# bjack205/rsLQR

Hardware: AMD Instinct MI355X
Metric: LQR solves/sec (nx=12,nu=4,N=256,batch=1024 per GPU) (higher is better)
Workload: dtype f64; 1 GPU; nx=12 nu=4 N=256 batch=1024 per GPU, fp64, factor+solve per step; parallelism=batch-sharded x1, no data-path collective, ranks_seen=1, flags=0, schedule=reduced-fused2

## Files before the change

### include/ndlqr_hip.h

```cpp
#ifndef NDLQR_HIP_H_
#define NDLQR_HIP_H_

#include <stddef.h>
#include <stdint.h>

#ifdef __cplusplus
extern "C" {
#endif

typedef struct NdlqrHipCtx NdlqrHipCtx;

int ndlqr_hip_device_count(void);
const char* ndlqr_hip_last_error(void);

NdlqrHipCtx* ndlqr_hip_create(int nstates, int ninputs, int nhorizon, int batch, int device);
#define NDLQR_CREATE_NO_PAD 1u
NdlqrHipCtx* ndlqr_hip_create_ex(int nstates, int ninputs, int nhorizon, int batch, int device, unsigned create_flags);
void ndlqr_hip_destroy(NdlqrHipCtx* ctx);
int ndlqr_hip_set_flags(NdlqrHipCtx* ctx, unsigned flags);
unsigned ndlqr_hip_get_flags(const NdlqrHipCtx* ctx);
int ndlqr_hip_set_stream(NdlqrHipCtx* ctx, void* hip_stream);
void* ndlqr_hip_get_stream(NdlqrHipCtx* ctx);

int ndlqr_hip_upload_inputs(NdlqrHipCtx* ctx, int p0, int count, const double* AB,
                            const double* QR, const double* rhs);
int ndlqr_hip_pack_flat_device(NdlqrHipCtx* ctx, const double* A, const double* B, const double* Q,
                               const double* R, const double* q, const double* r, const double* d,
                               const double* x0);
int ndlqr_hip_init_dense(NdlqrHipCtx* ctx, const double* A, const double* B, const double* Q, const double* H,
                         const double* R, const double* q, const double* r, const double* d, const double* x0);
int ndlqr_hip_cost_is_dense(const NdlqrHipCtx* ctx);
int ndlqr_hip_cost_phase_ms(NdlqrHipCtx* ctx, double* out3);
int ndlqr_hip_set_rhs_dense(NdlqrHipCtx* ctx, const double* q, const double* r, const double* d, const double* x0);
int ndlqr_hip_download_cost_reduction(NdlqrHipCtx* ctx, double* L, double* LR, double* G, double* At, double* Bt,
                                      double* qt, double* rt, double* dt, double* x0t);
int ndlqr_hip_init_constrained(NdlqrHipCtx* ctx, const double* A, const double* B, const double* Q, const double* H,
                               const double* R, const double* q, const double* r, const double* d, const double* x0, int p,
                               const double* C, const double* D, const double* lo, const double* hi, int shared);
int ndlqr_hip_is_constrained(const NdlqrHipCtx* ctx);
int ndlqr_hip_set_constraint_bounds(NdlqrHipCtx* ctx, const double* lo, const double* hi, int shared);
int ndlqr_hip_solve_constrained(NdlqrHipCtx* ctx, double rho, double alpha, double eps_abs, double eps_rel, int max_iter,
                                int check_every, int warm_start, int adapt_every, int* iters, int* status);
int ndlqr_hip_set_constraint_adaptation(NdlqrHipCtx* ctx, int every, double rho_min, double rho_max);
int ndlqr_hip_download_constraint_penalties(NdlqrHipCtx* ctx, double* rho);
int ndlqr_hip_set_constraint_infeasibility(NdlqrHipCtx* ctx, int every, double eps);
int ndlqr_hip_download_constraint_infeasibility_certificate(NdlqrHipCtx* ctx, double* dlam, double* dmu);
int ndlqr_hip_download_constraint_infeasibility_measures(NdlqrHipCtx* ctx, double* measures, int* iteration);
int ndlqr_hip_download_constraint_multipliers(NdlqrHipCtx* ctx, double* mu);
int ndlqr_hip_download_constraint_residuals(NdlqrHipCtx* ctx, double* resid);
int ndlqr_hip_download_constraint_reduction(NdlqrHipCtx* ctx, double* Qs, double* Hs, double* Rs, double* L, double* LR,
                                            double* G, double* At, double* Bt, double* qt, double* rt, double* dt, double* x0t,
                                            double* v, double* y);
int ndlqr_hip_solve_constrained_adjoint(NdlqrHipCtx* ctx, const double* g, double alpha, double eps_abs, double eps_rel,
                                        int max_iter, int check_every, int* iters, int* status);
int ndlqr_hip_constraint_gradients(NdlqrHipCtx* ctx, int summed, double* gC, double* gD, double* glo, double* ghi);
int ndlqr_hip_download_constraint_adjoint_multipliers(NdlqrHipCtx* ctx, double* nu);
int ndlqr_hip_download_constraint_adjoint_residuals(NdlqrHipCtx* ctx, double* resid);
int ndlqr_hip_download_constraint_codes(NdlqrHipCtx* ctx, unsigned char* codes, double* v);
int ndlqr_hip_device_pointers(NdlqrHipCtx* ctx, void** out5);

int ndlqr_hip_solve_async(NdlqrHipCtx* ctx);
int ndlqr_hip_synchronize(NdlqrHipCtx* ctx);
int ndlqr_hip_staged_io(NdlqrHipCtx* ctx, double** AB, double** QR, double** rhs, double** z);
int ndlqr_hip_solve_staged(NdlqrHipCtx* ctx);
int ndlqr_hip_set_pipeline_depth(NdlqrHipCtx* ctx, int depth);
int ndlqr_hip_pipeline_depth(const NdlqrHipCtx* ctx);
int ndlqr_hip_upload_rhs(NdlqrHipCtx* ctx, int p0, int count, const double* rhs);
int ndlqr_hip_solve_rhs_async(NdlqrHipCtx* ctx);
double ndlqr_hip_last_solve_ms(NdlqrHipCtx* ctx);
int ndlqr_hip_solve_adjoint(NdlqrHipCtx* ctx, const double* g);
int ndlqr_hip_download_adjoint(NdlqrHipCtx* ctx, double* w);
int ndlqr_hip_gradients(NdlqrHipCtx* ctx, unsigned sum_mask, double* gA, double* gB, double* gQ, double* gR, double* gq,
                        double* gr, double* gd, double* gx0);
int ndlqr_hip_refine(NdlqrHipCtx* ctx, int which, int max_steps, int* steps, double* eta_before, double* eta_after);
int ndlqr_hip_refine_phase_ms(NdlqrHipCtx* ctx, double* out3);
int ndlqr_hip_kkt_residual_vector(NdlqrHipCtx* ctx, double* r);
int ndlqr_hip_set_bounds(NdlqrHipCtx* ctx, int shared, const double* xlo, const double* xhi, const double* ulo,
                         const double* uhi);
int ndlqr_hip_solve_box(NdlqrHipCtx* ctx, double rho, double alpha, double eps_abs, double eps_rel, int max_iter,
                        int check_every, int warm_start, int* iters, int* status);
int ndlqr_hip_solve_box_ex(NdlqrHipCtx* ctx, double rho, double alpha, double eps_abs, double eps_rel, int max_iter,
                           int check_every, int warm_start, int* iters, int* status, int adapt_every, double rho_min,
                           double rho_max);
int ndlqr_hip_download_box_penalties(NdlqrHipCtx* ctx, double* rho);
int ndlqr_hip_download_box_residuals(NdlqrHipCtx* ctx, double* resid);
int ndlqr_hip_download_box_adjoint_residuals(NdlqrHipCtx* ctx, double* resid);
int ndlqr_hip_set_box_infeasibility(NdlqrHipCtx* ctx, int every, double eps);
int ndlqr_hip_download_infeasibility_certificate(NdlqrHipCtx* ctx, double* dlam, double* dmu_x, double* dmu_u);
int ndlqr_hip_download_infeasibility_measures(NdlqrHipCtx* ctx, double* measures, int* iteration);
int ndlqr_hip_set_box_acceleration(NdlqrHipCtx* ctx, int mem, double safeguard, double reg);
int ndlqr_hip_download_box_acceleration(NdlqrHipCtx* ctx, int* accepted, int* rejected, double* gamma, int* columns);
int ndlqr_hip_download_bound_multipliers(NdlqrHipCtx* ctx, double* mu_x, double* mu_u);
unsigned long long ndlqr_hip_factor_count(const NdlqrHipCtx* ctx);
int ndlqr_hip_solve_box_adjoint(NdlqrHipCtx* ctx, const double* g, double alpha, double eps_abs, double eps_rel, int max_iter,
                                int check_every, int* iters, int* status);
int ndlqr_hip_bound_gradients(NdlqrHipCtx* ctx, int summed, double* gxlo, double* gxhi, double* gulo, double* guhi);
int ndlqr_hip_polish_box(NdlqrHipCtx* ctx, double sigma, int max_steps, int max_rounds, int* steps, int* status);
int ndlqr_hip_solve_polished_adjoint(NdlqrHipCtx* ctx, const double* g, int max_steps, int* steps, int* status);
int ndlqr_hip_download_polish_codes(NdlqrHipCtx* ctx, unsigned char* codes);
int ndlqr_hip_solve_multi_rhs(NdlqrHipCtx* ctx, int nrhs, const double* q, const double* r, const double* d,
                              const double* x0, double* soln);
int ndlqr_hip_solve_multi_rhs_slices(NdlqrHipCtx* ctx, int nrhs, const double* q, const double* r, const double* d,
                                     const double* x0, int knot0, int nknots, unsigned blocks, double* out);

int ndlqr_hip_step_async(NdlqrHipCtx* ctx, const double* q, const double* r, const double* d, const double* x0,
                         double* soln);
int ndlqr_hip_synchronize_previous(NdlqrHipCtx* ctx);
int ndlqr_hip_set_step_selection(NdlqrHipCtx* ctx, int knot0, int nknots, unsigned blocks);
int ndlqr_hip_solve_slices_async(NdlqrHipCtx* ctx, int knot0, int nknots, unsigned blocks, double* out);
int ndlqr_hip_download_selection(NdlqrHipCtx* ctx, int knot0, int nknots, unsigned blocks, double* out);
int ndlqr_hip_time_shard_top_doubles(NdlqrHipCtx* ctx, int G);
int ndlqr_hip_time_shard_factor(NdlqrHipCtx* ctx, int g, int G);
int ndlqr_hip_time_shard_export(NdlqrHipCtx* ctx, int G, double* buf);
int ndlqr_hip_time_shard_import(NdlqrHipCtx* ctx, int G, const double* buf);
int ndlqr_hip_time_shard_finish(NdlqrHipCtx* ctx, int g, int G);
void* ndlqr_hip_host_alloc(size_t bytes);
void ndlqr_hip_host_free(void* p);
void* ndlqr_hip_device_alloc(size_t bytes);
void ndlqr_hip_device_free(void* p);
int ndlqr_hip_copy(void* dst, const void* src, size_t bytes);

int ndlqr_hip_download_solutions(NdlqrHipCtx* ctx, int p0, int count, double* soln);
int ndlqr_hip_download_rhs_blocks(NdlqrHipCtx* ctx, int p, double* z_full);
int ndlqr_hip_download_factors(NdlqrHipCtx* ctx, int p, double* fact);
int ndlqr_hip_factors_valid(const NdlqrHipCtx* ctx);
int ndlqr_hip_pack_solutions_device(NdlqrHipCtx* ctx, double* dst);
int ndlqr_hip_kkt_residual(NdlqrHipCtx* ctx, double* res, double* bnorm);
int ndlqr_hip_cholesky_failures(NdlqrHipCtx* ctx);
const char* ndlqr_hip_schedule(const NdlqrHipCtx* ctx);

int ndlqr_hip_profile_slots(NdlqrHipCtx* ctx);
int ndlqr_hip_profile_get(NdlqrHipCtx* ctx, int slot, char* name, int name_cap, double* total_ms,
                          int* launches);
int ndlqr_hip_profile_reset(NdlqrHipCtx* ctx);

int ndlqr_hip_gemm(int tA, int tB, int m, int n, int k, double alpha, const double* A, int lda,
                   const double* B, int ldb, double beta, double* C, int ldc);
int ndlqr_hip_potrf_lower(int n, double* A, int lda);
int ndlqr_hip_potrs_lower(int n, int nrhs, const double* L, int ldl, double* B, int ldb);
int ndlqr_hip_trsv_lower(int n, int nrhs, const double* L, int ldl, double* B, int ldb, int transposed);

#ifdef __cplusplus
}
#endif
#endif
```

### rslqr_amd/api.py

```python
import ctypes as C
import os
import re

import numpy as np

from . import build as _build

FLAG_STRICT_FP = 1
FLAG_GENERIC = 2
FLAG_PROFILE = 4
FLAG_KEEP_FACT = 8
FLAG_KEEP_RECORDS = 16
SOLN_LAMBDA, SOLN_STATE, SOLN_INPUT, SOLN_ONLY = 1, 2, 4, 8
GRAD_A, GRAD_B, GRAD_Q, GRAD_R, GRAD_q, GRAD_r, GRAD_d, GRAD_x0 = 1, 2, 4, 8, 16, 32, 64, 128
GRAD_NAMES = ("A", "B", "Q", "R", "q", "r", "d", "x0")

ERR_INVALID = -1
ERR_NO_DEVICE = -2
ERR_NOT_SPD = -3

dp = C.POINTER(C.c_double)


class Matrix(C.Structure):
# ... 132 lines not shown
    proto("ndlqr_NewLQRData", C.POINTER(LQRData), ci, ci)
    proto("ndlqr_FreeLQRData", ci, C.POINTER(LQRData))
    proto("ndlqr_InitializeLQRData", ci, C.POINTER(LQRData), dp, dp, dp, dp, cd, dp, dp, dp)
    proto("ndlqr_CopyLQRData", ci, C.POINTER(LQRData), C.POINTER(LQRData))
    proto("ndlqr_NewLQRProblem", pp, ci, ci, ci)
    proto("ndlqr_InitializeLQRProblem", ci, pp, dp, C.POINTER(C.POINTER(LQRData)))
    proto("ndlqr_FreeLQRProblem", ci, pp)
    proto("ndlqr_ReadLQRProblemJSONFile", pp, C.c_char_p)
    proto("ndlqr_ReadLQRDataJSONFile", C.POINTER(LQRData), C.c_char_p)
    proto("ReadMatrixJSONFile", Matrix, C.c_char_p, C.c_char_p)
    proto("FreeMatrix", ci, mp)
    proto("ReadFile", ci, C.c_char_p, C.POINTER(C.c_char_p), C.POINTER(ci))
    proto("ndlqr_NewSyntheticLQRProblem", pp, ci, ci, ci, cu64)
    proto("ndlqr_GenerateSyntheticFlat", ci, ci, ci, ci, cu64, dp, dp, dp, dp, dp, dp, dp, dp)
    proto("ndlqr_BuildTree", OrderedBinaryTree, ci)
    proto("ndlqr_FreeTree", ci, C.POINTER(OrderedBinaryTree))
    proto("ndlqr_GetIndexFromLeaf", ci, C.POINTER(OrderedBinaryTree), ci, ci)
    proto("ndlqr_GetIndexLevel", ci, C.POINTER(OrderedBinaryTree), ci)
    proto("ndlqr_GetIndexAtLevel", ci, C.POINTER(OrderedBinaryTree), ci, ci)
    proto("ndlqr_NewNdData", ndp, ci, ci, ci, ci)
    proto("ndlqr_FreeNdData", ci, ndp)
    proto("ndlqr_ResetNdData", None, ndp)
    proto("ndlqr_GetNdFactor", ci, ndp, ci, ci, C.POINTER(C.POINTER(NdFactor)))
    proto("ndlqr_NewCholeskyFactors", C.POINTER(NdLqrCholeskyFactors), ci, ci)
    proto("ndlqr_FreeCholeskyFactors", ci, C.POINTER(NdLqrCholeskyFactors))
    proto("ndlqr_GetSFactorization", ci, C.POINTER(NdLqrCholeskyFactors), ci, ci,
          C.POINTER(C.POINTER(CholeskyInfo)))
    proto("ndlqr_NewNdLqrSolver", sp, ci, ci, ci)
    proto("ndlqr_FreeNdLqrSolver", ci, sp)
    proto("ndlqr_InitializeWithLQRProblem", ci, pp, sp)
    proto("ndlqr_ResetSolver", None, sp)
    proto("ndlqr_GetNumVars", ci, sp)
    proto("ndlqr_SetNumThreads", ci, sp, ci)
    proto("ndlqr_GetNumThreads", ci, sp)
    proto("ndlqr_PrintSolveSummary", None, sp)
    proto("ndlqr_PrintSolveProfile", ci, sp)
    proto("ndlqr_GetProfile", NdLqrProfile, sp)
    proto("ndlqr_Solve", ci, sp)
    proto("ndlqr_GetSolution", Matrix, sp)
    proto("ndlqr_CopySolution", ci, sp, dp)
    proto("ndlqr_SyncFactorsToHost", ci, sp)
    proto("ndlqr_SetDeviceProfiling", ci, sp, ci)
    proto("ndlqr_SetDeviceFlags", ci, sp, C.c_uint)
    proto("ndlqr_SetFactorMirroring", ci, sp, ci)
    proto("ndlqr_SolveLeaf", ci, sp, ci)
    proto("ndlqr_SolveLeaves", ci, sp)
    proto("ndlqr_FactorInnerProduct", ci, ndp, ndp, ci, ci, ci)
    proto("ndlqr_SolveCholeskyFactor", ci, ndp, C.POINTER(CholeskyInfo), ci, ci, ci)
    proto("ndlqr_UpdateShurFactor", ci, ndp, ndp, ci, ci, ci, ci, C.c_bool)
    proto("ndlqr_ShouldCalcLambda", C.c_bool, C.POINTER(OrderedBinaryTree), ci, ci)
    proto("ndlqr_ComputeShurCompliment", ci, sp, ci, ci, ci)
    proto("MatrixMultiply", None, mp, mp, mp, C.c_bool, C.c_bool, cd, cd)
    proto("MatrixCholeskyFactorize", ci, mp)
    proto("MatrixCholeskySolve", ci, mp, mp)
    proto("MatrixSymmetricMultiply", None, mp, mp, mp, cd, cd)
    proto("MatrixAddition", ci, mp, mp, cd)
    proto("ndlqr_NewBatchSolver", vp, ci, ci, ci, ci, ci)
    proto("ndlqr_FreeBatchSolver", ci, vp)
    proto("ndlqr_BatchSetFlags", ci, vp, C.c_uint)
    proto("ndlqr_BatchGetFlags", C.c_uint, vp)
    proto("ndlqr_InitializeBatch", ci, vp, C.POINTER(pp), ci)
    proto("ndlqr_InitializeBatchFlat", ci, vp, dp, dp, dp, dp, dp, dp, dp, dp)
    proto("ndlqr_InitializeBatchSynthetic", ci, vp, cu64)
    proto("ndlqr_InitializeBatchFlatDense", ci, vp, dp, dp, dp, dp, dp, dp, dp, dp, dp)
    proto("ndlqr_BatchCostIsDense", ci, vp)
    proto("ndlqr_hip_download_cost_reduction", ci, vp, dp, dp, dp, dp, dp, dp, dp, dp, dp)
    proto("ndlqr_hip_cost_phase_ms", ci, vp, dp)
    proto("ndlqr_InitializeBatchFlatConstrained", ci, vp, dp, dp, dp, dp, dp, dp, dp, dp, dp, ci, dp, dp, dp, dp, C.c_uint)
    proto("ndlqr_BatchIsConstrained", ci, vp)
    proto("ndlqr_BatchSetConstraintBounds", ci, vp, dp, dp, C.c_uint)
    proto("ndlqr_SolveBatchLinConstrained", ci, vp, C.POINTER(NdLqrBoxSettingsFull), C.POINTER(ci), C.POINTER(ci))
    proto("ndlqr_BatchSetConstraintPenaltyAdaptation", ci, vp, ci, C.c_double, C.c_double)
    proto("ndlqr_CopyBatchConstraintPenalties", ci, vp, dp)
    proto("ndlqr_BatchSetConstraintInfeasibilityDetection", ci, vp, ci, cd)
    proto("ndlqr_CopyBatchConstraintInfeasibilityCertificate", ci, vp, dp, dp)
    proto("ndlqr_CopyBatchConstraintInfeasibilityMeasures", ci, vp, dp, C.POINTER(ci))
    proto("ndlqr_CopyBatchConstraintMultipliers", ci, vp, dp)
    proto("ndlqr_CopyBatchConstraintResiduals", ci, vp, dp)
    proto("ndlqr_hip_download_constraint_reduction", ci, vp, *([dp] * 14))
    proto("ndlqr_SolveBatchLinAdjoint", ci, vp, dp, C.POINTER(NdLqrBoxSettingsFull), C.POINTER(ci), C.POINTER(ci))
    proto("ndlqr_BatchConstraintGradients", ci, vp, dp, dp, dp, dp, C.c_uint)
    proto("ndlqr_CopyBatchConstraintAdjointMultipliers", ci, vp, dp)
    proto("ndlqr_CopyBatchConstraintAdjointResiduals", ci, vp, dp)
    proto("ndlqr_CopyBatchConstraintCodes", ci, vp, C.c_void_p)
    proto("ndlqr_hip_download_constraint_codes", ci, vp, C.c_void_p, dp)
    proto("ndlqr_InitializeBatchFlatDevice", ci, vp, vp, vp, vp, vp, vp, vp, vp, vp)
    proto("ndlqr_SolveBatch", ci, vp)
    proto("ndlqr_BatchSetRhsFlat", ci, vp, dp, dp, dp, dp)
    proto("ndlqr_SolveBatchRhsOnly", ci, vp)
    proto("ndlqr_SolveBatchMultiRhs", ci, vp, ci, dp, dp, dp, dp, dp)
    proto("ndlqr_SolveBatchMultiRhsSlices", ci, vp, ci, dp, dp, dp, dp, ci, ci, C.c_uint, dp)
    proto("ndlqr_SolveBatchAsync", ci, vp)
    proto("ndlqr_BatchStepAsync", ci, vp, dp, dp, dp, dp, dp)
    proto("ndlqr_BatchSynchronizePrevious", ci, vp)
    proto("ndlqr_BatchSetStepSelection", ci, vp, ci, ci, C.c_uint)
    proto("ndlqr_CopyBatchSolutionSlices", ci, vp, ci, ci, C.c_uint, dp)
    proto("ndlqr_SolveBatchSlicesAsync", ci, vp, ci, ci, C.c_uint, dp)
    proto("ndlqr_BatchTimeShardTopDoubles", ci, vp, ci)
    proto("ndlqr_BatchTimeShardFactor", ci, vp, ci, ci)
    proto("ndlqr_BatchTimeShardExportTop", ci, vp, ci, vp)
    proto("ndlqr_BatchTimeShardImportTop", ci, vp, ci, vp)
    proto("ndlqr_BatchTimeShardFinish", ci, vp, ci, ci)
    proto("ndlqr_HostAlloc", vp, C.c_size_t)
    proto("ndlqr_HostFree", None, vp)
    proto("ndlqr_DeviceAlloc", vp, C.c_size_t)
    proto("ndlqr_DeviceFree", None, vp)
    proto("ndlqr_DeviceCopy", ci, vp, vp, C.c_size_t)
    proto("ndlqr_BatchSynchronize", ci, vp)
    proto("ndlqr_BatchNumVars", ci, vp)
    proto("ndlqr_BatchSize", ci, vp)
    proto("ndlqr_CopyBatchSolution", ci, vp, ci, dp)
    proto("ndlqr_CopyBatchSolutions", ci, vp, dp)
    proto("ndlqr_CopyBatchSolutionsDevice", ci, vp, vp)
    proto("ndlqr_CopyBatchFactors", ci, vp, ci, dp)
    proto("ndlqr_BatchCholeskyFailures", ci, vp)
    proto("ndlqr_BatchKktResiduals", ci, vp, dp, dp)
    proto("ndlqr_BatchSolveTimeMs", cd, vp)
    proto("ndlqr_SolveBatchAdjoint", ci, vp, dp)
    proto("ndlqr_CopyBatchAdjoint", ci, vp, dp)
    proto("ndlqr_BatchGradients", ci, vp, C.c_uint, dp, dp, dp, dp, dp, dp, dp, dp)
    proto("ndlqr_RefineBatch", ci, vp, ci, C.POINTER(ci), dp, dp)
    proto("ndlqr_RefineBatchAdjoint", ci, vp, ci, C.POINTER(ci), dp, dp)
    proto("ndlqr_BatchKktResidualVector", ci, vp, dp)
    proto("ndlqr_hip_refine_phase_ms", ci, vp, dp)
    proto("ndlqr_BatchDeviceContext", vp, vp)
    proto("ndlqr_BatchSetBounds", ci, vp, C.c_uint, dp, dp, dp, dp)
    proto("ndlqr_SolveBatchBoxConstrained", ci, vp, C.POINTER(NdLqrBoxSettingsFull), C.POINTER(ci), C.POINTER(ci))
    proto("ndlqr_CopyBatchBoundMultipliers", ci, vp, dp, dp)
    proto("ndlqr_CopyBatchBoxPenalties", ci, vp, dp)
    proto("ndlqr_CopyBatchBoxResiduals", ci, vp, dp)
    proto("ndlqr_CopyBatchBoxAdjointResiduals", ci, vp, dp)
    proto("ndlqr_BatchSetInfeasibilityDetection", ci, vp, ci, cd)
    proto("ndlqr_CopyBatchInfeasibilityCertificate", ci, vp, dp, dp, dp)
    proto("ndlqr_CopyBatchInfeasibilityMeasures", ci, vp, dp, C.POINTER(ci))
    proto("ndlqr_BatchSetBoxAcceleration", ci, vp, ci, cd, cd)
    proto("ndlqr_CopyBatchBoxAcceleration", ci, vp, C.POINTER(ci), C.POINTER(ci), dp, C.POINTER(ci))
    proto("ndlqr_SolveBatchBoxAdjoint", ci, vp, dp, C.POINTER(NdLqrBoxSettingsFull), C.POINTER(ci), C.POINTER(ci))
    proto("ndlqr_BatchBoundGradients", ci, vp, C.c_uint, dp, dp, dp, dp)
    proto("ndlqr_PolishBatchBoxConstrained", ci, vp, C.POINTER(NdLqrPolishSettings), C.POINTER(ci), C.POINTER(ci))
    proto("ndlqr_hip_download_polish_codes", ci, vp, C.POINTER(C.c_ubyte))
    proto("ndlqr_SolveBatchPolishedAdjoint", ci, vp, dp, C.POINTER(NdLqrPolishSettings), C.POINTER(ci), C.POINTER(ci))
    proto("ndlqr_hip_factor_count", C.c_ulonglong, vp)
    proto("ndlqr_hip_set_stream", ci, vp, vp)
    proto("ndlqr_hip_get_stream", vp, vp)
    proto("ndlqr_hip_profile_slots", ci, vp)
    proto("ndlqr_hip_profile_get", ci, vp, ci, C.c_char_p, ci, dp, C.POINTER(ci))
    proto("ndlqr_hip_profile_reset", ci, vp)
    proto("ndlqr_hip_device_pointers", ci, vp, C.POINTER(vp))
    proto("ndlqr_hip_staged_io", ci, vp, C.POINTER(dp), C.POINTER(dp), C.POINTER(dp), C.POINTER(dp))
    proto("ndlqr_hip_download_rhs_blocks", ci, vp, ci, dp)
    proto("ndlqr_hip_upload_inputs", ci, vp, ci, ci, dp, dp, dp)
    proto("ndlqr_hip_factors_valid", ci, vp)
    proto("ndlqr_hip_schedule", C.c_char_p, vp)
    proto("ndlqr_hip_set_pipeline_depth", ci, vp, ci)
    proto("ndlqr_hip_pipeline_depth", ci, vp)
    proto("ndlqr_hip_pack_solutions_device", ci, vp, vp)
    proto("ndlqr_hip_gemm", ci, ci, ci, ci, ci, ci, cd, dp, ci, dp, ci, cd, dp, ci)
    proto("ndlqr_hip_potrf_lower", ci, ci, dp, ci)
    proto("ndlqr_hip_potrs_lower", ci, ci, ci, dp, ci, dp, ci)
    _LIB = L
    return L


def pinned_empty(shape):
    import weakref
    count = int(np.prod(shape))
    L = lib()
    ptr = L.ndlqr_HostAlloc(max(count, 1) * 8)
    if not ptr:
        raise MemoryError("ndlqr_HostAlloc(%d bytes) failed" % (count * 8))
    buf = (C.c_double * max(count, 1)).from_address(ptr)
    arr = np.ctypeslib.as_array(buf)[:count].reshape(shape)
    weakref.finalize(buf, L.ndlqr_HostFree, C.c_void_p(ptr))
    return arr


class DeviceArray:

    def __init__(self, shape):
        import weakref
        self.shape = tuple(int(s) for s in (shape if isinstance(shape, (tuple, list)) else (shape,)))
        self.size = int(np.prod(self.shape))
        L = lib()
        self.ptr = L.ndlqr_DeviceAlloc(max(self.size, 1) * 8)
        if not self.ptr:
            raise MemoryError("ndlqr_DeviceAlloc(%d bytes) failed" % (self.size * 8))
        weakref.finalize(self, L.ndlqr_DeviceFree, C.c_void_p(self.ptr))

    def set(self, arr):
        arr = np.ascontiguousarray(arr, dtype=np.float64)
        assert arr.size == self.size
        if lib().ndlqr_DeviceCopy(C.c_void_p(self.ptr), arr.ctypes.data_as(C.c_void_p), self.size * 8):
            raise RuntimeError("ndlqr_DeviceCopy failed")
        return self

    def get(self):
        out = np.empty(self.shape)
        if lib().ndlqr_DeviceCopy(out.ctypes.data_as(C.c_void_p), C.c_void_p(self.ptr), self.size * 8):
            raise RuntimeError("ndlqr_DeviceCopy failed")
        return out


def device_count():
    return lib().ndlqr_hip_device_count()


def _ptr(a):
    return a.ctypes.data_as(dp)


def _any_ptr(a, size):
    if hasattr(a, "ptr"):
        if a.size != size:
            raise ValueError("expected %d doubles, got %d" % (size, a.size))
        return C.cast(C.c_void_p(int(a.ptr)), dp)
    if not (isinstance(a, np.ndarray) and a.dtype == np.float64 and a.flags["C_CONTIGUOUS"] and a.size == size):
        raise ValueError("expected a C-contiguous float64 array of %d doubles" % size)
    return _ptr(a)


def generate_synthetic(n, m, N, seed):
    out = dict(A=np.zeros((N, n * n)), B=np.zeros((N, n * m)), Q=np.zeros((N, n)),
               R=np.zeros((N, m)), q=np.zeros((N, n)), r=np.zeros((N, m)), d=np.zeros((N, n)),
               x0=np.zeros(n))
    err = lib().ndlqr_GenerateSyntheticFlat(n, m, N, seed, *[_ptr(out[k]) for k in
                                                               ("A", "B", "Q", "R", "q", "r", "d", "x0")])
    if err:
        raise RuntimeError("ndlqr_GenerateSyntheticFlat failed: %d" % err)
    return out


class BatchSolver:

    def __init__(self, n, m, N, batch, device=-1, flags=0):
        self.L = lib()
        self.n, self.m, self.N, self.batch = n, m, N, batch
        self.h = self.L.ndlqr_NewBatchSolver(n, m, N, batch, device)
        if not self.h:
            raise RuntimeError("ndlqr_NewBatchSolver failed: %s" %
                               self.L.ndlqr_hip_last_error().decode())
        self.nvars = self.L.ndlqr_BatchNumVars(self.h)
        self._sel = None
        self._step_refs = []
        if flags:
            self.set_flags(flags)

    def close(self):
        if getattr(self, "h", None):
            self.L.ndlqr_FreeBatchSolver(self.h)
            self.h = None
        self._step_refs = []

    __del__ = close

    def set_flags(self, flags):
        self.L.ndlqr_BatchSetFlags(self.h, flags)

    @property
    def ctx(self):
        return self.L.ndlqr_BatchDeviceContext(self.h)

    def initialize_flat(self, A, B, Q, R, q, r, d, x0):
        n, m, N, bt = self.n, self.m, self.N, self.batch
        shapes = dict(A=(bt, N, n * n), B=(bt, N, n * m), Q=(bt, N, n), R=(bt, N, m),
                      q=(bt, N, n), r=(bt, N, m), d=(bt, N, n), x0=(bt, n))
        arrs = []
        for name, a in zip(("A", "B", "Q", "R", "q", "r", "d", "x0"), (A, B, Q, R, q, r, d, x0)):
            a = np.ascontiguousarray(a, dtype=np.float64)
            if a.size != int(np.prod(shapes[name])):
                raise ValueError("bad size for %s" % name)
            arrs.append(a)
        err = self.L.ndlqr_InitializeBatchFlat(self.h, *[_ptr(a) for a in arrs])
        if err:
            raise RuntimeError("ndlqr_InitializeBatchFlat failed: %d" % err)

    def initialize_flat_device(self, *device_ptrs):
        err = self.L.ndlqr_InitializeBatchFlatDevice(self.h, *[C.c_void_p(int(p)) for p in device_ptrs])
        if err:
            raise RuntimeError("ndlqr_InitializeBatchFlatDevice failed: %d" % err)

    def initialize_flat_dense(self, A, B, Q, H, R, q, r, d, x0):
        n, m, N, bt = self.n, self.m, self.N, self.batch
        sizes = dict(A=bt * N * n * n, B=bt * N * n * m, Q=bt * N * n * n, H=bt * N * n * m, R=bt * N * m * m,
                     q=bt * N * n, r=bt * N * m, d=bt * N * n, x0=bt * n)
        ptrs, keep = [], []
        for name, a in zip(("A", "B", "Q", "H", "R", "q", "r", "d", "x0"), (A, B, Q, H, R, q, r, d, x0)):
            if a is None:
                if name != "H":
                    raise ValueError("%s is missing (only H may be None)" % name)
                ptrs.append(None)
                continue
            if not hasattr(a, "ptr"):
                a = np.ascontiguousarray(a, dtype=np.float64)
                if a.size != sizes[name]:
                    raise ValueError("bad size for %s" % name)
                keep.append(a)
            ptrs.append(_any_ptr(a, sizes[name]))
        err = self.L.ndlqr_InitializeBatchFlatDense(self.h, *ptrs)
        if err:
            raise RuntimeError("ndlqr_InitializeBatchFlatDense failed: %d (%s)" % (err, self.L.ndlqr_hip_last_error().decode()))

    def cost_is_dense(self):
        return bool(self.L.ndlqr_BatchCostIsDense(self.h))

    def cost_phase_ms(self):
        out = np.zeros(3)
# ... 464 lines not shown

    def set_box_acceleration(self, mem=0, safeguard=0.0, reg=0.0):
        err = self.L.ndlqr_BatchSetBoxAcceleration(self.h, int(mem), float(safeguard), float(reg))
        if err:
            raise RuntimeError("ndlqr_BatchSetBoxAcceleration failed: %d (%s)" % (err, self.L.ndlqr_hip_last_error().decode()))
        self._accel_mem = int(mem)

    def box_acceleration(self):
        B, mem = self.batch, getattr(self, "_accel_mem", 0)
        ints = [np.zeros(B, dtype=np.int32) for _ in range(3)]
        gamma = np.zeros((B, max(mem, 1)))
        ip = [a.ctypes.data_as(C.POINTER(C.c_int)) for a in ints]
        err = self.L.ndlqr_CopyBatchBoxAcceleration(self.h, ip[0], ip[1], _ptr(gamma), ip[2])
        if err:
            raise RuntimeError("ndlqr_CopyBatchBoxAcceleration failed: %d (%s)"
                               % (err, self.L.ndlqr_hip_last_error().decode()))
        return ints[0], ints[1], gamma[:, :mem], ints[2]

    def box_penalties(self, rho=None):
        if rho is None:
            rho = np.zeros(self.batch)
        err = self.L.ndlqr_CopyBatchBoxPenalties(self.h, _any_ptr(rho, self.batch))
        if err:
            raise RuntimeError("ndlqr_CopyBatchBoxPenalties failed: %d (%s)" % (err, self.L.ndlqr_hip_last_error().decode()))
        return rho

    def _residuals(self, name, resid):
        if resid is None:
            resid = np.zeros((self.batch, 4))
        err = getattr(self.L, name)(self.h, _any_ptr(resid, 4 * self.batch))
        if err:
            raise RuntimeError("%s failed: %d (%s)" % (name, err, self.L.ndlqr_hip_last_error().decode()))
        return resid

    def box_residuals(self, resid=None):
        return self._residuals("ndlqr_CopyBatchBoxResiduals", resid)

    def box_adjoint_residuals(self, resid=None):
        return self._residuals("ndlqr_CopyBatchBoxAdjointResiduals", resid)

    def bound_multipliers(self, mu_x=None, mu_u=None):
        n, m, N, B = self.n, self.m, self.N, self.batch
        if mu_x is None:
            mu_x = np.zeros((B, N, n))
        if mu_u is None:
            mu_u = np.zeros((B, N, m))
        err = self.L.ndlqr_CopyBatchBoundMultipliers(self.h, _any_ptr(mu_x, B * N * n), _any_ptr(mu_u, B * N * m))
        if err:
            raise RuntimeError("ndlqr_CopyBatchBoundMultipliers failed: %d (%s)"
                               % (err, self.L.ndlqr_hip_last_error().decode()))
        return mu_x, mu_u

    def solve_box_adjoint(self, g, alpha=0.0, eps_abs=0.0, eps_rel=0.0, max_iter=0, check_every=0):
        if not hasattr(g, "ptr"):
            g = np.ascontiguousarray(g, dtype=np.float64)
        st = NdLqrBoxSettingsFull(0.0, alpha, eps_abs, eps_rel, int(max_iter), int(check_every), 0)
        iters = np.zeros(self.batch, dtype=np.int32)
        status = np.zeros(self.batch, dtype=np.int32)
        err = self.L.ndlqr_SolveBatchBoxAdjoint(self.h, _any_ptr(g, self.batch * self.nvars), C.byref(st),
                                                iters.ctypes.data_as(C.POINTER(C.c_int)),
                                                status.ctypes.data_as(C.POINTER(C.c_int)))
        if err:
            raise RuntimeError("ndlqr_SolveBatchBoxAdjoint failed: %d (%s)" % (err, self.L.ndlqr_hip_last_error().decode()))
        return iters, status

    def bound_gradients(self, summed=False, out=None):
        n, m, N, B = self.n, self.m, self.N, self.batch
        shape = {k: ((N, w) if summed else (B, N, w)) for k, w in (("xlo", n), ("xhi", n), ("ulo", m), ("uhi", m))}
        if out is None:
            out = {k: np.zeros(sh) for k, sh in shape.items()}
        unknown = set(out) - set(shape)
        if unknown:
            raise ValueError("unknown bound names: %s" % sorted(unknown))
        ptrs = [None if out.get(k) is None else _any_ptr(out[k], int(np.prod(shape[k]))) for k in ("xlo", "xhi", "ulo", "uhi")]
        err = self.L.ndlqr_BatchBoundGradients(self.h, BOUNDS_SHARED if summed else 0, *ptrs)
        if err:
            raise RuntimeError("ndlqr_BatchBoundGradients failed: %d (%s)" % (err, self.L.ndlqr_hip_last_error().decode()))
        return out

    def polish_box(self, sigma=0.0, max_steps=0, max_rounds=0, steps=None, status=None):
        st = NdLqrPolishSettings(sigma, int(max_steps), int(max_rounds))
        if steps is None:
            steps = np.zeros(self.batch, dtype=np.int32)
        if status is None:
            status = np.zeros(self.batch, dtype=np.int32)
        as_int = lambda a: C.cast(a.ptr, C.POINTER(C.c_int)) if hasattr(a, "ptr") else a.ctypes.data_as(C.POINTER(C.c_int))
        err = self.L.ndlqr_PolishBatchBoxConstrained(self.h, C.byref(st), as_int(steps), as_int(status))
        if err:
            raise RuntimeError("ndlqr_PolishBatchBoxConstrained failed: %d (%s)"
                               % (err, self.L.ndlqr_hip_last_error().decode()))
        return steps, status

    def solve_polished_adjoint(self, g, max_steps=0, steps=None, status=None):
        if not hasattr(g, "ptr"):
            g = np.ascontiguousarray(g, dtype=np.float64)
        st = NdLqrPolishSettings(0.0, int(max_steps), 0)
        if steps is None:
            steps = np.zeros(self.batch, dtype=np.int32)
        if status is None:
            status = np.zeros(self.batch, dtype=np.int32)
        as_int = lambda a: C.cast(a.ptr, C.POINTER(C.c_int)) if hasattr(a, "ptr") else a.ctypes.data_as(C.POINTER(C.c_int))
        err = self.L.ndlqr_SolveBatchPolishedAdjoint(self.h, _any_ptr(g, self.batch * self.nvars), C.byref(st), as_int(steps),
                                                     as_int(status))
        if err:
            raise RuntimeError("ndlqr_SolveBatchPolishedAdjoint failed: %d (%s)" % (err, self.L.ndlqr_hip_last_error().decode()))
        return steps, status

    def polish_codes(self):
        out = np.zeros((self.batch, self.N, self.n + self.m), dtype=np.uint8)
        err = self.L.ndlqr_hip_download_polish_codes(self.ctx, out.ctypes.data_as(C.POINTER(C.c_ubyte)))
        if err:
            raise RuntimeError("ndlqr_hip_download_polish_codes failed: %d (%s)" % (err, self.L.ndlqr_hip_last_error().decode()))
        return out

    def factor_count(self):
        return int(self.L.ndlqr_hip_factor_count(self.ctx))

    def solutions_to_device(self, device_ptr):
        got = self.L.ndlqr_CopyBatchSolutionsDevice(self.h, C.c_void_p(int(device_ptr)))
        if got != self.nvars:
            raise RuntimeError("ndlqr_CopyBatchSolutionsDevice failed: %d" % got)

    def upload_packed(self, AB, QR, rhs):
        err = self.L.ndlqr_hip_upload_inputs(self.ctx, 0, self.batch, _ptr(AB), _ptr(QR), _ptr(rhs))
        if err:
            raise RuntimeError("ndlqr_hip_upload_inputs failed: %d" % err)

    def factors(self, p):
        if self.N & (self.N - 1):
            raise RuntimeError("ndlqr_CopyBatchFactors: not available for a padded horizon (horizon %d is no power of two)"
                               % self.N)
        K = int(np.log2(self.N))
        out = np.zeros(self.N * K * (2 * self.n + self.m) * self.n)
        err = self.L.ndlqr_CopyBatchFactors(self.h, p, _ptr(out))
        if err:
            raise RuntimeError("ndlqr_CopyBatchFactors failed: %d" % err)
        return out

    def cholesky_failures(self):
        return self.L.ndlqr_BatchCholeskyFailures(self.h)

    def profile(self):
        out = {}
        for slot in range(self.L.ndlqr_hip_profile_slots(self.ctx)):
            name = C.create_string_buffer(64)
            ms, cnt = C.c_double(0), C.c_int(0)
            self.L.ndlqr_hip_profile_get(self.ctx, slot, name, 64, C.byref(ms), C.byref(cnt))
            out[name.value.decode()] = (ms.value, cnt.value)
        return out

    def schedule(self):
        return self.L.ndlqr_hip_schedule(self.ctx).decode()

    def set_pipeline_depth(self, depth):
        return self.L.ndlqr_hip_set_pipeline_depth(self.ctx, depth)

    def pipeline_depth(self):
        return self.L.ndlqr_hip_pipeline_depth(self.ctx)

    def profile_reset(self):
        self.L.ndlqr_hip_profile_reset(self.ctx)
```

### rslqr_amd/csrc/hip_context.hpp

```cpp
#pragma once
#include <hip/hip_runtime.h>

#include <cstdio>
#include <cstdlib>
#include <cstring>
#include <initializer_list>
#include <string>
#include <utility>
#include <vector>

#include "ndlqr.h"
#include "ndlqr_hip.h"

#include "kernels_common.hpp"

#pragma GCC visibility push(hidden)
int ndlqr_hip_fail(const char* what, hipError_t e);
struct NdlqrHipCtx;
int ndlqr_hip_ensure_F(NdlqrHipCtx* c);
#pragma GCC visibility pop
#define HIP_TRY(expr)                                                  \
  do {                                                                 \
    hipError_t e_ = (expr);                                            \
    if (e_ != hipSuccess) return ndlqr_hip_fail(#expr, e_);            \
  } while (0)

constexpr size_t kLdsMax = 160 * 1024;
constexpr size_t kLdsDefaultDynamic = 64 * 1024;
template <class Kernel>
static inline hipError_t allow_dynamic_lds(Kernel* kernel, size_t lds) {
  if (lds <= kLdsDefaultDynamic) return hipSuccess;
  return hipFuncSetAttribute(reinterpret_cast<const void*>(kernel), hipFuncAttributeMaxDynamicSharedMemorySize, (int)lds);
}


enum { SLOT_LEAF = 0, SLOT_SEP, SLOT_SCHUR, SLOT_BOUNDARY, SLOT_APPLY, SLOT_BOTTOM, SLOT_UPPER, SLOT_TOP, SLOT_COUNT };

struct PendingEvent {
  int slot;
  hipEvent_t start, stop;
};

enum class Family { None, Small, GenericReduced, GenericKnot };

struct KeptState {
  Family family = Family::None;
  bool time_shard = false;
  bool rec_complete = false;
  bool rec_compact = false;
  bool fact_valid = false;
  const char* schedule = "none";
  void forget_factorisation() { rec_complete = fact_valid = false; }
};

struct CapturedChain {
  hipGraphExec_t exec = nullptr;
  unsigned flags = 0;
  hipStream_t stream = nullptr;
  unsigned apply = 0;
  void reset() {
    if (exec) (void)hipGraphExecDestroy(exec);
    exec = nullptr;
  }
};

struct KnotSlice {
  int knot0 = 0, nknots = 0;
  unsigned blocks = 7u;
  bool valid(int N, unsigned allowed) const {
    return knot0 >= 0 && nknots > 0 && knot0 + nknots <= N && (blocks & 7u) && !(blocks & ~allowed);
  }
  size_t width(const ndlqr::Dims& u) const {
    return ((blocks & 1u) ? u.n : 0) + ((blocks & 2u) ? u.n : 0) + ((blocks & 4u) ? u.m : 0);
  }
  size_t doubles(const ndlqr::Dims& u) const { return nknots > 0 ? width(u) * nknots : (size_t)u.rows * u.N - u.m; }
};

#pragma GCC visibility push(hidden)

template <class T, bool PINNED>
class OwnedBuf {
  T* p_ = nullptr;
  size_t n_ = 0;

 public:
  OwnedBuf() = default;
  OwnedBuf(const OwnedBuf&) = delete;
  OwnedBuf& operator=(const OwnedBuf&) = delete;
  OwnedBuf(OwnedBuf&& o) noexcept : p_(o.p_), n_(o.n_) { o.p_ = nullptr; o.n_ = 0; }
  OwnedBuf& operator=(OwnedBuf&& o) noexcept { std::swap(p_, o.p_); std::swap(n_, o.n_); return *this; }
  ~OwnedBuf() { reset(); }
  T* get() const { return p_; }
  operator T*() const { return p_; }
  size_t count() const { return n_; }
  void reset() {
    if (p_) (void)(PINNED ? hipHostFree(p_) : hipFree(p_));
    p_ = nullptr; n_ = 0;
  }
  hipError_t ensure(size_t count) {
    if (p_) return hipSuccess;
    const hipError_t e = PINNED ? hipHostMalloc((void**)&p_, sizeof(T) * count, hipHostMallocDefault)
                                : hipMalloc((void**)&p_, sizeof(T) * count);
    if (e != hipSuccess) p_ = nullptr;
    else n_ = count;
    return e;
  }
  hipError_t ensure_zeroed(size_t count, hipStream_t st = nullptr) {
    if (p_) return hipSuccess;
    const hipError_t e = ensure(count);
    if (e != hipSuccess) return e;
    if (PINNED) { memset(p_, 0, sizeof(T) * count); return hipSuccess; }
    return hipMemsetAsync(p_, 0, sizeof(T) * count, st);
  }
  hipError_t grow(size_t count) {
    if (count <= n_) return hipSuccess;
    reset();
    return ensure(count);
  }
};
template <class T> using DevBuf = OwnedBuf<T, false>;
template <class T> using PinnedBuf = OwnedBuf<T, true>;

static inline size_t doubles_QR(const ndlqr::Dims& d) { return (size_t)d.batch * d.N * d.w; }
static inline size_t doubles_z(const ndlqr::Dims& d) { return (size_t)d.batch * d.N * d.rows; }
static inline size_t doubles_F(const ndlqr::Dims& d) { return (size_t)d.batch * d.K * d.N * d.fb; }
static inline hipError_t first_error(std::initializer_list<hipError_t> list) {
  for (const hipError_t e : list) if (e != hipSuccess) return e;
  return hipSuccess;
}

struct BufferSet {
  DevBuf<double> rec;
  DevBuf<double> red;
  DevBuf<double> ytop;
  DevBuf<double> z;
  DevBuf<double> rhs;
  DevBuf<double> xfer;
  DevBuf<int> tree_cnt;
  PinnedBuf<int> h_fail;
  hipStream_t stream = nullptr;
  hipEvent_t ev_start = nullptr, ev_stop = nullptr;
  unsigned long long rhs_gen[4] = {};
  CapturedChain graph;
  bool ready = false;
  hipError_t ensure_xfer(const ndlqr::Dims& u) { return xfer.ensure((size_t)u.batch * u.N * u.rows + (size_t)u.batch * u.n); }
};


struct DevKnobs {
  int rowbcast = -1;
  int tree = -1;
  int backsub_cols = -1;
  int fuse2 = -1;
  int pipeline = 2;
  bool no_top = false;
  int top_levels = 3;
  bool no_mfma = false;
  int sep_threads = 0;
  int mult_threads = 0;
  bool no_reduced_generic = false;
  bool no_pad = false;
  bool alt_priority_set = false;
  int alt_priority = 0;
};

struct AdjointState {
  DevBuf<double> rhs, z;
  DevBuf<double> save;
  unsigned long long gen = 0;
  hipError_t ensure_save(const ndlqr::Dims& d) { return save.ensure(2 * (size_t)d.batch * d.N * d.n); }
  hipError_t ensure(const ndlqr::Dims& d, hipStream_t st) {
    return first_error({rhs.ensure(doubles_z(d)), z.ensure_zeroed(doubles_z(d), st), ensure_save(d)});
  }
};

struct BoxState {
  DevBuf<double> lo, hi, v, y, z, qr_save, rhs[2], resid, rho;
  DevBuf<unsigned char> mask;
  DevBuf<int> status, iters, word;
  PinnedBuf<int> h_word;
  bool shared = false, have_bounds = false, have_vy = false;
  size_t bstride = 0;
  bool fact = false;
  bool rho_uniform = false;
  double rho_value = 0.0;
  unsigned flags = 0;
  KeptState kept;
  unsigned long long soln_gen = 0;
  hipError_t ensure(const ndlqr::Dims& d, hipStream_t st) {
    const size_t nz = doubles_z(d), nv = doubles_QR(d), nb = (size_t)d.batch;
    return first_error({mask.ensure_zeroed(nv, st), lo.ensure(nv), hi.ensure(nv), word.ensure(4), h_word.ensure(5),
                        z.ensure_zeroed(nz, st),
                        v.ensure(nv), y.ensure(nv), qr_save.ensure(nv), rhs[0].ensure(nz), rhs[1].ensure(nz),
                        resid.ensure(4 * nb), status.ensure(nb), iters.ensure(nb), rho.ensure(nb)});
  }
};

struct BoxInfeasState {
  DevBuf<double> z_prev, y_prev, rho_prev, cert_lam, cert_mu, measures;
  DevBuf<int> measured_at;
  int every = 0;
  double eps = 1e-4;
  unsigned long long gen = 0;
  hipError_t ensure(const ndlqr::Dims& d) {
    const size_t nv = doubles_QR(d);
    return first_error({z_prev.ensure(doubles_z(d)), y_prev.ensure(nv), rho_prev.ensure((size_t)d.batch),
                        cert_lam.ensure((size_t)d.batch * d.N * d.n), cert_mu.ensure(nv),
                        measures.ensure(4 * (size_t)d.batch), measured_at.ensure((size_t)d.batch)});
  }
};

struct BoxAccelState {
  DevBuf<double> ring_t, ring_g, pv, py, gram, gprev, gamma;
  DevBuf<int> meta;
  int mem = 0, mem_solved = 0;
  double safeguard = 1.0, reg = 1e-10;
  unsigned long long gen = 0;
  hipError_t ensure(const ndlqr::Dims& d) {
    const size_t nv = doubles_QR(d), nb = (size_t)d.batch;
    return first_error({ring_t.grow((size_t)(mem + 1) * nv), ring_g.grow((size_t)(mem + 1) * nv), pv.ensure(nv), py.ensure(nv),
                        gram.ensure(nb * 17 * 17), gprev.ensure(nb), gamma.ensure(nb * 16), meta.ensure(6 * nb)});
  }
};

struct BoxAdjointState {
  DevBuf<unsigned char> code;
  DevBuf<double> v, y, resid, rhs[2];
  DevBuf<int> status, iters, word;
  unsigned long long gen = 0;
  hipError_t ensure(const ndlqr::Dims& d) {
    const size_t nz = doubles_z(d), nv = doubles_QR(d), nb = (size_t)d.batch;
    return first_error({code.ensure(nv), v.ensure(nv), y.ensure(nv), rhs[0].ensure(nz), rhs[1].ensure(nz),
                        resid.ensure(4 * nb), status.ensure(nb), iters.ensure(nb), word.ensure(1)});
  }
};

constexpr int kRefineMaxSteps = 8;
struct RefineState {
  DevBuf<double> r, delta, eta;
  DevBuf<unsigned long long> norms;
  DevBuf<int> steps;
  double phase_ms[3] = {};
  static size_t norm_count(const ndlqr::Dims& d) { return 2 * (kRefineMaxSteps + 1) * (size_t)d.batch; }
  hipError_t ensure_r(const ndlqr::Dims& d) { return r.ensure(doubles_z(d)); }
  hipError_t ensure(const ndlqr::Dims& d, hipStream_t st) {
    return first_error({ensure_r(d), norms.ensure(norm_count(d)), steps.ensure((size_t)d.batch), eta.ensure(2 * (size_t)d.batch),
                        delta.ensure_zeroed(doubles_z(d), st)});
  }
};

constexpr int kPolishMaxSteps = 32;
struct PolishState {
  DevBuf<unsigned char> code;
  DevBuf<double> z, mu, bt, zc, muc, btc, z0, r, delta, sig;
  DevBuf<double> nu, abt, ones;
  DevBuf<int> astate, asteps, ahere;
  unsigned long long adj_gen = 0;
  DevBuf<unsigned long long> norms;
  DevBuf<int> state, steps, here, word;
  PinnedBuf<int> h_word;
  bool fact = false;
  unsigned flags = 0;
  KeptState kept;
  unsigned long long soln_gen = 0;
  static size_t norm_count(const ndlqr::Dims& d) { return 2 * (kPolishMaxSteps + 1) * (size_t)d.batch; }
  hipError_t ensure(const ndlqr::Dims& d, hipStream_t st) {
    const size_t nz = doubles_z(d), nv = doubles_QR(d), nb = (size_t)d.batch;
    return first_error({code.ensure(nv), z.ensure(nz), mu.ensure(nv), bt.ensure(nz), zc.ensure(nz), muc.ensure(nv),
                        btc.ensure(nz), z0.ensure(nz), r.ensure(nz),
                        delta.ensure_zeroed(nz, st),
                        sig.ensure(nb), norms.ensure(norm_count(d)), state.ensure(nb), steps.ensure(nb), here.ensure(nb),
                        word.ensure(2), h_word.ensure(2)});
  }
  hipError_t ensure_adjoint(const ndlqr::Dims& d) {
    const size_t nb = (size_t)d.batch;
    return first_error({nu.ensure(doubles_QR(d)), abt.ensure(doubles_z(d)), ones.ensure(nb), astate.ensure(nb), asteps.ensure(nb),
                        ahere.ensure(nb)});
  }
};

struct MultiRhsState {
  DevBuf<double> rhs, z, zsep, fsum, ytop, in, out;
  hipError_t ensure(const ndlqr::Dims& d, const ndlqr::Dims& u, size_t cap, hipStream_t st) {
    const size_t nz = cap * d.N * d.rows;
    if (rhs.count() >= nz) return hipSuccess;
    hipError_t e = first_error({rhs.grow(nz), z.grow(nz), zsep.grow(cap * d.N * d.n), fsum.grow(cap * (d.N / 8) * 2 * d.n),
                                ytop.grow(cap * (d.N / 8) * d.n), in.grow(cap * ((size_t)u.N * (2 * u.n + u.m) + u.n)),
                                out.grow(cap * ((size_t)u.rows * u.N - u.m))});
    if (e == hipSuccess) e = first_error({hipMemsetAsync(rhs, 0, sizeof(double) * nz, st), hipMemsetAsync(z, 0, sizeof(double) * nz, st)});
    if (e != hipSuccess)
      for (DevBuf<double>* b : {&rhs, &z, &zsep, &fsum, &ytop, &in, &out}) b->reset();
    return e;
  }
};

struct CostState {
  bool dense = false;
  unsigned long long mapped_gen = 0;
  DevBuf<double> rec, At, Bt, qt, rt, dt, x0t, ones, stage;
  bool mapped(unsigned long long gen) const { return mapped_gen != 0 && mapped_gen == gen; }
  double phase_ms[3] = {};
  static size_t record_doubles(const ndlqr::Dims& u) { return (size_t)u.n * u.n + (size_t)u.m * u.m + (size_t)u.m * u.n; }
  hipError_t ensure(const ndlqr::Dims& u) {
    const size_t kn = (size_t)u.batch * u.N;
    return first_error({rec.ensure(kn * record_doubles(u)), At.ensure(kn * u.n * u.n), Bt.ensure(kn * u.n * u.m),
                        qt.ensure(kn * u.n), rt.ensure(kn * u.m), dt.ensure(kn * u.n), x0t.ensure((size_t)u.batch * u.n),
// ... 176 lines not shown
```

### rslqr_amd/csrc/kernels_bottom_reduced.hpp

```cpp
#pragma once
#include "kernels_dpp.hpp"
#include "kernels_small.hpp"

namespace ndlqr {

typedef double acc4_t __attribute__((ext_vector_type(4)));

template <int NX>
struct McPitch {
  static constexpr int SP = 18, WP = 17;
};

template <int NX, class Hook>
__device__ __forceinline__ void factor_tail_mc(const int lane, const acc4_t& c, const double (&ra)[(NX + 3) / 4],
                                               const double (&rb)[(NX + 3) / 4], const double* Wm, acc4_t& X0,
                                               acc4_t& X1, Hook hook) {
  constexpr int KS = (NX + 3) / 4, WP = McPitch<NX>::WP;
  int lane_o = lane;
  asm volatile("" : "+v"(lane_o));
  const int li = lane_o & 15, lk = lane_o >> 4;
  double wt[KS], wa[KS], b0[KS];
#pragma unroll
  for (int q = 0; q < KS; ++q) {
    wt[q] = Wm[(4 * q + lk) * WP + li];
// ... 427 lines not shown
      if constexpr (TREE) {
        ts[it].x = __hip_atomic_load(sl + 2 * ec, __ATOMIC_RELAXED, __HIP_MEMORY_SCOPE_AGENT);
        ts[it].y = __hip_atomic_load(sl + 2 * ec + 1, __ATOMIC_RELAXED, __HIP_MEMORY_SCOPE_AGENT);
      } else {
        ts[it] = reinterpret_cast<const double2*>(sl)[ec];
      }
    }
#pragma unroll
    for (int it = 0; it < IA; ++it) { const int e = lane + 64 * it; ta[it] = abm[e < NA ? e : NA - 1]; }
#pragma unroll
    for (int it = 0; it < IQ; ++it) { const int e = lane + 64 * it; tq[it] = qr[e < NQ ? e : NQ - 1]; }
#pragma unroll
    for (int it = 0; it < IR; ++it) { const int e = lane + 64 * it; tr[it] = r0[e < NR ? e : NR - 1]; }
#pragma unroll
    for (int it = 0; it < (EXT ? 0 : IS); ++it) {
      const int e = lane + 64 * it, ec = e < NS ? e : NS - 1;
      reinterpret_cast<double2*>(lds.buf)[ec] = ts[it];
    }
#pragma unroll
    for (int it = 0; it < IA; ++it) {
      const int e = lane + 64 * it, ec = e < NA ? e : NA - 1, row = ec / W, c = ec - row * W;
      abs_[row * WP + c] = ta[it];
    }
#pragma unroll
    for (int it = 0; it < IQ; ++it) { const int e = lane + 64 * it, ec = e < NQ ? e : NQ - 1; rq[ec] = 1.0 / tq[it]; }
#pragma unroll
    for (int it = 0; it < IR; ++it) { const int e = lane + 64 * it, ec = e < NR ? e : NR - 1; zs[ec] = tr[it]; }
  }
  wave_lds_sync();
  constexpr int TRI = RedSlot<NX>::TRI;
  const double *DL = slot, *DR = slot + TRI, *CA = slot + 2 * TRI, *CB = slot + 2 * TRI + NN;
  const double *gL = slot + 2 * TRI + 2 * NN, *gR = slot + 2 * TRI + 2 * NN + NX;

  const acc4_t c0 = leaf_tile_mc<NX, NU, WP>(lane, false, abs_, rq, rq + W, zs, zs + NX + W, [&](int g) {
    const int i = lk + 4 * g, ic = i < NX ? i : NX - 1;
    const int tix = RedSlot<NX>::tri(ic, ri);
    const double dd = DL[tix] + DR[tix], gg = gL[ic] + gR[ic];
    return -(li == NX ? gg : dd);
  });
  double wcol[NX];
  {
    const int h = lane & 31;
    const bool is_a = h < NX, is_b = h > NX && h <= 2 * NX;
    const double* src = is_a ? CA + h : CB + (is_b ? h - NX - 1 : 0);
    const double sign = ((is_a && hasA) || (is_b && hasB)) ? -1.0 : 0.0;
#pragma unroll
    for (int k = 0; k < NX; ++k) wcol[k] = src[k * NX] * sign;
  }
  wave_lds_sync();
  SEG(9);

  acc4_t X0, X1, unused;
  if (chol_wy_mc<NX>(lane, c0, lds.buf, wcol, lstore_of<NX>(store_l, F, rec, d, b, l, s)) && lane == 0)
    flag_failure(info, d, b);
  SEG(31);
  tail_wy_mc<NX>(lane, lds.buf, X0, X1,
                 [&](const double (&R0)[KSN], const double (&R1)[KSN], const acc4_t& Z0, const acc4_t& Z1) {
                   acc4_t g00, g01, g11;
                   gram_mc<NX, true, true, false, true>(R0, R1, Z0, Z1, g00, g01, unused, g11);
                   const acc4_t zero = {0.0, 0.0, 0.0, 0.0};
                   if constexpr (TREE)
                     push_mc<NX>(lane, hasA, hasB, leftchild, sa, sb, g00, g01, g11, zero, zero, zero, AddAtomic(),
                                 StoreThrough());
                   else
                     push_mc<NX>(lane, hasA, hasB, leftchild, sa, sb, g00, g01, g11, zero, zero, zero, AddAtomic(),
                                 StorePlain());
                 });
  SEG(13);
  store_record_mc<NX>(rec + ((size_t)b * N + s) * (2 * NN + NX), lane, hasA, hasB, X0, X1);
#ifdef NDLQR_SEGTIME
  __builtin_amdgcn_s_waitcnt(0);
#endif
  SEG(12);
}

template <int NX, int NU>
__global__ __launch_bounds__(64) __attribute__((amdgpu_waves_per_eu(4))) void reduced_level_mc(
    Dims d, int l, const double* __restrict__ AB, const double* __restrict__ QR, const double* __restrict__ rhs,
    double* red, double* __restrict__ rec, double* F, int* __restrict__ info, const int store_l) {
  __shared__ ReducedLds<NX, NU, false> lds;
  reduced_separator_mc<NX, NU, false>(d, l, (blockIdx.x + d.xoff) * (2 << l), blockIdx.y, threadIdx.x, AB, QR, rhs, red, rec, F,
                                      info, store_l, lds);
}


template <int NX, int NU>
__device__ __forceinline__ void reduced_eliminate_pass_mc(const Dims& d, const int base, const int b, const int lane,
                                                          const acc4_t& c_leaf, const double* slot,
                                                          int* __restrict__ info, double* buf) {
  constexpr int NN = NX * NX, TRI = RedSlot<NX>::TRI;
  const int N = d.N, T = 8;
  const bool hasA = base > 0, hasB = base + T < N;
  const int li = lane & 15, lk = lane >> 4, ri = li < NX ? li : NX - 1;
  const double *DL = slot, *DR = slot + TRI, *CA = slot + 2 * TRI, *CB = slot + 2 * TRI + NN;
  const double *gL = slot + 2 * TRI + 2 * NN, *gR = slot + 2 * TRI + 2 * NN + NX;
  acc4_t c0;
#pragma unroll
  for (int g = 0; g < 4; ++g) {
    const int i = lk + 4 * g, ic = i < NX ? i : NX - 1;
    const int tix = RedSlot<NX>::tri(ic, ri);
    const double dd = DL[tix] + DR[tix], gg = gL[ic] + gR[ic];
    c0[g] = c_leaf[g] - (li == NX ? gg : dd);
  }
  double wcol[NX];
  {
    const int h = lane & 31;
    const bool is_a = h < NX, is_b = h > NX && h <= 2 * NX;
    const double* src = is_a ? CA + h : CB + (is_b ? h - NX - 1 : 0);
    const double sign = ((is_a && hasA) || (is_b && hasB)) ? -1.0 : 0.0;
#pragma unroll
    for (int k = 0; k < NX; ++k) wcol[k] = src[k * NX] * sign;
  }
  wave_lds_sync();
  if (chol_wy_mc<NX>(lane, c0, buf, wcol, nullptr) && lane == 0) flag_failure(info, d, b);
}
template <int NX, int NU>
__device__ __forceinline__ void reduced_eliminate_tail_mc(const Dims& d, const int base, const int b, const int lane,
                                                          const bool gram, double* red, double* __restrict__ rec,
                                                          const double* buf) {
  using P = McWyLayout<NX>;
  constexpr int NN = NX * NX, KS = P::KS;
  const int N = d.N, T = 8, s = base + 3;
  const bool hasA = base > 0, hasB = base + T < N, leftchild = (base & T) == 0;
  const int li = lane & 15, lk = lane >> 4;
  double y0[KS], y1[KS];
  acc4_t Z0 = {0.0, 0.0, 0.0, 0.0}, Z1 = {0.0, 0.0, 0.0, 0.0};
#pragma unroll
  for (int q = 0; q < KS; ++q) {
    y0[q] = buf[P::Y0 + (4 * q + lk) * P::YP + li];
    y1[q] = buf[P::Y1 + (4 * q + lk) * P::YP + li];
    Z0[q] = y0[q]; Z1[q] = y1[q];
  }
  if (gram) {
    const RedSlot<NX> sa = red_slot<NX>(red, d, b, hasA ? base - 1 : s);
    const RedSlot<NX> sb = red_slot<NX>(red, d, b, hasB ? base + T - 1 : s);
    acc4_t g00, g01, g11, unused;
    gram_mc<NX, true, true, false, true>(y0, y1, Z0, Z1, g00, g01, unused, g11);
    const acc4_t zero = {0.0, 0.0, 0.0, 0.0};
    push_mc<NX>(lane, hasA, hasB, leftchild, sa, sb, g00, g01, g11, zero, zero, zero, AddAtomic(), StorePlain());
  } else {
    double wt[KS];
#pragma unroll
    for (int q = 0; q < KS; ++q) wt[q] = buf[P::W + (4 * q + lk) * P::WP + li];
    acc4_t X0 = {0.0, 0.0, 0.0, 0.0}, X1 = {0.0, 0.0, 0.0, 0.0};
#pragma unroll
    for (int q = 0; q < KS; ++q) {
      X0 = __builtin_amdgcn_mfma_f64_16x16x4f64(wt[q], y0[q], X0, 0, 0, 0);
      X1 = __builtin_amdgcn_mfma_f64_16x16x4f64(wt[q], y1[q], X1, 0, 0, 0);
    }
    store_record_mc<NX>(rec + ((size_t)b * N + s) * (2 * NN + NX), lane, hasA, hasB, X0, X1);
  }
}

template <int NX, int NU, bool TREE, bool REDIRECT>
__device__ __forceinline__ void bottom_group_mc(const Dims& d, const int k0, const int b, const int lane,
                                                const double* __restrict__ AB, const double* __restrict__ QR,
                                                const double* __restrict__ rhs, double* red, double* __restrict__ rec,
                                                double* F, int* __restrict__ info, const int store_l, const int compact0,
                                                ReducedLds<NX, NU>& lds, double* slotA, double* slotB,
                                                const bool with_m = false, acc4_t* c_m = nullptr);
template <int NX, int NU>
__global__ __launch_bounds__(128) __attribute__((amdgpu_waves_per_eu(4))) void bottom8_reduced_mc(
    Dims d, const double* __restrict__ AB, const double* __restrict__ QR, const double* __restrict__ rhs, double* red,
    double* __restrict__ rec, int* __restrict__ info) {
  __shared__ ReducedLds<NX, NU> lds[2];
  __shared__ __attribute__((aligned(16))) double mslot[RedSlot<NX>::SIZE];
  const int wave = __builtin_amdgcn_readfirstlane(threadIdx.x >> 6), b = blockIdx.y;
  const int kw = (blockIdx.x + d.xoff) * 8;
  int lane = threadIdx.x & 63;
  for (int e = threadIdx.x; e < RedSlot<NX>::SIZE; e += 128) mslot[e] = 0.0;
  __syncthreads();
  acc4_t c_m = {0.0, 0.0, 0.0, 0.0};
  bottom_group_mc<NX, NU, false, true>(d, kw + 4 * wave, b, lane, AB, QR, rhs, red, rec, nullptr, info, 0, 1, lds[wave],
                                       wave == 1 ? mslot : nullptr, wave == 0 ? mslot : nullptr, wave == 0, &c_m);
  asm volatile("s_waitcnt vmcnt(0)" ::: "memory");
  __syncthreads();
  asm volatile("" : "+v"(lane));
  if (wave == 0) reduced_eliminate_pass_mc<NX, NU>(d, kw, b, lane, c_m, mslot, info, lds[0].buf);
  __syncthreads();
  reduced_eliminate_tail_mc<NX, NU>(d, kw, b, lane, wave == 0, red, rec, lds[0].buf);
}

template <int NX>
__device__ __forceinline__ void backsub_top_body(const Dims& d, const int b, const int t,
                                                 const double* __restrict__ recs, double* __restrict__ ytop,
                                                 double* ytop_lds, const int bp = -1, const double* zsep = nullptr);
template <int NX, int NU>
__global__ __launch_bounds__(256) __attribute__((amdgpu_waves_per_eu(4))) void reduced_top_mc(Dims d, const int l0, const double* __restrict__ AB,
                                                      const double* __restrict__ QR, const double* __restrict__ rhs,
                                                      double* red, double* __restrict__ rec, double* F,
                                                      int* __restrict__ info, const int store_l,
                                                      double* __restrict__ ytop) {
  __shared__ ReducedLds<NX, NU, false> lds[4];
  const int wave = __builtin_amdgcn_readfirstlane(threadIdx.x >> 6), b = blockIdx.x;
  for (int l = l0, s0 = 0; l < d.K;) {
    int lane = threadIdx.x & 63;
    asm volatile("" : "+v"(lane));
    const int cnt = d.N >> (l + 1);
    if (wave + s0 < cnt)
      reduced_separator_mc<NX, NU, true>(d, l, (wave + s0) * (2 << l), b, lane, AB, QR, rhs, red, rec, F, info, store_l,
                                         lds[wave]);
    s0 += 4;
    if (s0 < cnt) continue;
    s0 = 0;
    ++l;
    asm volatile("s_waitcnt vmcnt(0)" ::: "memory");
    __syncthreads();
  }
  if (ytop) backsub_top_body<NX>(d, b, threadIdx.x, rec, ytop, reinterpret_cast<double*>(&lds[0]), -1, nullptr);
}

template <int NX, int NU, bool TREE, bool REDIRECT>
__device__ __forceinline__ void bottom_group_mc(const Dims& d, const int k0, const int b, const int lane,
                                                const double* __restrict__ AB, const double* __restrict__ QR,
                                                const double* __restrict__ rhs, double* red, double* __restrict__ rec,
                                                double* F, int* __restrict__ info, const int store_l, const int compact0,
                                                ReducedLds<NX, NU>& lds, double* slotA, double* slotB,
                                                const bool with_m, acc4_t* c_m) {
  constexpr int W = NX + NU, ROWS = 2 * NX + NU, NN = NX * NX, KSN = (NX + 3) / 4;
  constexpr int REC = 2 * NN + NX;
  constexpr int WP = ReducedLds<NX, NU>::WP;
  double* abs_ = lds.buf;
  double* rq = lds.rq;
  double* rh = lds.rh;
  const int N = d.N;
  const int li = lane & 15, lk = lane >> 4;
  const int ri = li < NX ? li : NX - 1;
  const bool hasA = k0 > 0, hasB = k0 + 4 < N;
  SEG_INIT();

  {
    const double* abm = AB + ((size_t)b * N + k0) * NX * W;
    const double* q0 = QR + ((size_t)b * N + k0) * W;
    const double* r0 = rhs + ((size_t)b * N + k0) * ROWS;
    constexpr int NQ = 4 * W, IQ = (NQ + 63) / 64, NR = 4 * ROWS, IR = (NR + 63) / 64;
    double qv[IQ], rv[IR];
#pragma unroll
    for (int it = 0; it < IQ; ++it) { const int e = lane + 64 * it; qv[it] = q0[e < NQ ? e : NQ - 1]; }
#pragma unroll
    for (int it = 0; it < IR; ++it) { const int e = lane + 64 * it; rv[it] = r0[e < NR ? e : NR - 1]; }
    if constexpr (W % 2 == 0) {
      constexpr int NA = 4 * NX * W / 2, IA = (NA + 63) / 64;
      double2 t[IA];
#pragma unroll
      for (int it = 0; it < IA; ++it) {
        const int e = lane + 64 * it;
        t[it] = reinterpret_cast<const double2*>(abm)[e < NA ? e : NA - 1];
      }
#pragma unroll
      for (int it = 0; it < IA; ++it) {
        const int e = lane + 64 * it, ec = e < NA ? e : NA - 1, row = ec / (W / 2), c2 = ec - row * (W / 2);
        reinterpret_cast<double2*>(&abs_[row * WP])[c2] = t[it];
      }
    } else {
      constexpr int NA = 4 * NX * W, IA = (NA + 63) / 64;
      double t[IA];
#pragma unroll
      for (int it = 0; it < IA; ++it) { const int e = lane + 64 * it; t[it] = abm[e < NA ? e : NA - 1]; }
#pragma unroll
      for (int it = 0; it < IA; ++it) { const int e = lane + 64 * it; abs_[e < NA ? e : NA - 1] = t[it]; }
    }
#pragma unroll
    for (int it = 0; it < IQ; ++it) {
      const int e = lane + 64 * it, ec = e < NQ ? e : NQ - 1, kn = ec / W, c = ec - kn * W;
      rq[ec] = 1.0 / qv[it];
      if (e < NQ && !(qv[it] > 0.0) && !(k0 + kn == N - 1 && c >= NX)) flag_failure(info, d, b);
    }
#pragma unroll
    for (int it = 0; it < IR; ++it) { const int e = lane + 64 * it; rh[e < NR ? e : NR - 1] = rv[it]; }
  }
  wave_lds_sync();
  SEG(20);

  auto none = [](int) { return 0.0; };
  acc4_t c_s0;
  if (k0 == 0) c_s0 = leaf_tile_mc<NX, NU, WP>(lane, true, abs_, rq, rq + W, rh, rh + ROWS, none);
  else c_s0 = leaf_tile_mc<NX, NU, WP>(lane, false, abs_, rq, rq + W, rh, rh + ROWS, none);
  acc4_t c_t = leaf_tile_mc<NX, NU, WP>(lane, false, abs_ + NX * WP, rq + W, rq + 2 * W, rh + ROWS, rh + 2 * ROWS, none);
  acc4_t c_s2 = leaf_tile_mc<NX, NU, WP>(lane, false, abs_ + 2 * NX * WP, rq + 2 * W, rq + 3 * W, rh + 2 * ROWS,
                                         rh + 3 * ROWS, none);
  if constexpr (REDIRECT) {
    if (with_m) {
      const double* qn = QR + ((size_t)b * N + k0 + 4) * W;
      const double* rn = rhs + ((size_t)b * N + k0 + 4) * ROWS;
      const int e = lane < 3 * NX ? lane : 3 * NX - 1;
      const double raw = e < NX ? qn[e] : rn[e - NX];
      const double val = e < NX ? 1.0 / raw : raw;
      double nw[4], nl[4], nxv[4];
#pragma unroll
      for (int g = 0; g < 4; ++g) {
        const int i = lk + 4 * g, ic = i < NX ? i : NX - 1;
        nw[g] = __shfl(val, ic, 64); nl[g] = __shfl(val, NX + ic, 64); nxv[g] = __shfl(val, 2 * NX + ic, 64);
      }
      *c_m = leaf_tile_mc<NX, NU, WP, false>(lane, false, abs_ + 3 * NX * WP, rq + 3 * W, rq, rh + 3 * ROWS, rh, none);
#pragma unroll
      for (int g = 0; g < 4; ++g) {
        const int i = lk + 4 * g;
        (*c_m)[g] += li == NX ? -fma(nxv[g], nw[g], nl[g]) : (i == li ? nw[g] : 0.0);
      }
    }
  }
  acc4_t X0, X1, unused;
  double* myrec = rec + ((size_t)b * N + k0) * REC;
  acc4_t park_a, ca_t, park_b11, cb_t;
  auto hook_s0 = [&](const double (&R0)[KSN], const double (&R1)[KSN], const acc4_t& Z0, const acc4_t& Z1) {
    acc4_t g11;
    gram_mc<NX, true, false, true, true>(R0, R1, Z0, Z1, park_a, unused, ca_t, g11);
#pragma unroll
    for (int g = 0; g < 4; ++g) c_t[g] -= (li < NX) ? g11[g] : ca_t[g];
  };
  auto hook_s2 = [&](const double (&R0)[KSN], const double (&R1)[KSN], const acc4_t& Z0, const acc4_t& Z1) {
    acc4_t g00;
    gram_mc<NX, true, true, false, true>(R0, R1, Z0, Z1, g00, cb_t, unused, park_b11);
#pragma unroll
    for (int g = 0; g < 4; ++g) c_t[g] -= g00[g];
  };

  const bool compact_path = !TREE && compact0 != 0;
  if (!TREE && compact_path) {
    double wcol[NX];
    {
      const int h = lane & 31, x = lane >> 5;
      const bool is_a = h < NX, is_b = h > NX && h <= 2 * NX;
      const int ca = is_a ? h : 0, cb = is_b ? h - NX - 1 : 0;
      const double* src = abs_ + (2 * x) * NX * WP + (is_a ? ca : NX * WP + cb * WP);
      const double* scl = rq + (2 * x) * W + (is_a ? ca : W);
      const int sstr = is_a ? WP : 1, wstr = is_a ? 0 : 1;
      const bool on = (is_a && (x == 1 || hasA)) || (is_b && (x == 0 || hasB));
      const double sign = on ? -1.0 : 0.0;
#pragma unroll
      for (int k = 0; k < NX; ++k) wcol[k] = (src[k * sstr] * scl[k * wstr]) * sign;
    }
    wave_lds_sync();
    SEG(21);
    if (chol_pair_y_mc<NX>(lane, c_s0, c_s2, lds.buf, wcol, myrec, myrec + 2 * REC) && (lane == 0 || lane == 32))
      flag_failure(info, d, b);
    SEG(30);
    using PY = McPairYLayout<NX>;
#pragma unroll
    for (int x = 0; x < 2; ++x) {
      const double* Y0 = lds.buf + PY::tile(x, 0);
      const double* Y1 = lds.buf + PY::tile(x, 1);
      double y0[KSN], y1[KSN];
      acc4_t Z0 = {0.0, 0.0, 0.0, 0.0}, Z1 = {0.0, 0.0, 0.0, 0.0};
#pragma unroll
      for (int q = 0; q < KSN; ++q) {
        y0[q] = Y0[(4 * q + lk) * PY::YP + li];
        y1[q] = Y1[(4 * q + lk) * PY::YP + li];
        Z0[q] = y0[q]; Z1[q] = y1[q];
      }
      if (x == 0) hook_s0(y0, y1, Z0, Z1); else hook_s2(y0, y1, Z0, Z1);
    }
    SEG(35);
  } else {
  double ra0[KSN], rb0[KSN], ra2[KSN], rb2[KSN];
#pragma unroll
  for (int q = 0; q < KSN; ++q) {
    const int kq = 4 * q + lk, i = kq < NX ? kq : NX - 1;
    const double a0 = abs_[i * WP + ri], b0 = abs_[(NX + ri) * WP + i];
    const double a2 = abs_[(2 * NX + i) * WP + ri], b2 = abs_[(3 * NX + ri) * WP + i];
    const double s0 = rq[ri], s1 = rq[W + i], s2 = rq[2 * W + ri], s3 = rq[3 * W + i];
    ra0[q] = hasA ? -a0 * s0 : 0.0;
    rb0[q] = -b0 * s1;
    ra2[q] = -a2 * s2;
    rb2[q] = hasB ? -b2 * s3 : 0.0;
  }
  wave_lds_sync();
  SEG(21);

  using Pair = McPairLayout<NX>;
  if (chol_pair_mc<NX>(lane, c_s0, c_s2, lds.buf, store_l ? Fblk(F, d, b, 0, k0 + 1) : nullptr,
                       store_l ? Fblk(F, d, b, 0, k0 + 3) : nullptr) &&
      (lane == 0 || lane == 32))
    flag_failure(info, d, b);
  SEG(30);
  factor_tail_mc<NX>(lane, c_s0, ra0, rb0, lds.buf + Pair::W_A, X0, X1, hook_s0);
  store_record_mc<NX>(myrec, lane, hasA, true, X0, X1);
  factor_tail_mc<NX>(lane, c_s2, ra2, rb2, lds.buf + Pair::W_B, X0, X1, hook_s2);
  store_record_mc<NX>(myrec + 2 * REC, lane, true, hasB, X0, X1);
  SEG(35);
  }
  double wcol[NX];
  {
    constexpr int TP = 17;
    static_assert(2 * 16 * TP <= ReducedLds<NX, NU>::NBUF, "both coupling tiles fit the buffer");
    double* ta = lds.buf;
    double* tb = lds.buf + 16 * TP;
    wave_lds_sync();
#pragma unroll
    for (int g = 0; g < 4; ++g) {
      ta[(lk + 4 * g) * TP + li] = -ca_t[g];
      tb[(lk + 4 * g) * TP + li] = -cb_t[g];
    }
    wave_lds_sync();
    const int h = lane & 31;
    const bool is_a = h < NX, is_b = h > NX && h <= 2 * NX;
    const double* src = is_a ? ta + h : tb + (is_b ? h - NX - 1 : 0);
#pragma unroll
    for (int k = 0; k < NX; ++k) wcol[k] = src[k * TP];
    wave_lds_sync();
  }
  const bool leftchild = (k0 & 4) == 0;
  RedSlot<NX> sa = red_slot<NX>(red, d, b, hasA ? k0 - 1 : 3);
  RedSlot<NX> sb = red_slot<NX>(red, d, b, hasB ? k0 + 3 : 3);
  if constexpr (REDIRECT) {
    if (slotA) sa.p = slotA;
    if (slotB) sb.p = slotB;
  }
  if (chol_wy_mc<NX>(lane, c_t, lds.buf, wcol, lstore_of<NX>(store_l, F, rec, d, b, 1, k0 + 1)) && lane == 0)
    flag_failure(info, d, b);
  tail_wy_mc<NX>(lane, lds.buf, X0, X1,
                 [&](const double (&R0)[KSN], const double (&R1)[KSN], const acc4_t& Z0, const acc4_t& Z1) {
                   acc4_t g00, g01, g11;
                   gram_mc<NX, true, true, false, true>(R0, R1, Z0, Z1, g00, g01, unused, g11);
                   if constexpr (TREE)
                     push_mc<NX>(lane, hasA, hasB, leftchild, sa, sb, g00, g01, g11, park_a, cb_t, park_b11,
                                 StoreThrough(), StoreThrough());
                   else
                     push_mc<NX>(lane, hasA, hasB, leftchild, sa, sb, g00, g01, g11, park_a, cb_t, park_b11,
                                 StorePlain(), StorePlain());
                 });
  SEG(34);
  store_record_mc<NX>(myrec + REC, lane, hasA, hasB, X0, X1);
#ifdef NDLQR_SEGTIME
  __builtin_amdgcn_s_waitcnt(0);
#endif
  SEG(36);
}

template <int NX, int NU, bool TREE, bool COMPACT = false>
__global__ __launch_bounds__(64) __attribute__((amdgpu_waves_per_eu(4))) void bottom_reduced_mc(
    Dims d, const double* __restrict__ AB, const double* __restrict__ QR, const double* __restrict__ rhs,
    double* red, double* __restrict__ rec, double* F, int* __restrict__ info, const int store_l, int* cnt,
    const int compact0) {
  static_assert(!(TREE && COMPACT), "the tree schedule keeps full records");
  __shared__ ReducedLds<NX, NU> lds;
  const int lane = threadIdx.x, b = blockIdx.y, N = d.N, k0 = (blockIdx.x + d.xoff) * 4;
  bottom_group_mc<NX, NU, TREE, false>(d, k0, b, lane, AB, QR, rhs, red, rec, F, info, store_l, COMPACT ? 1 : compact0, lds,
                                       nullptr, nullptr);

  if constexpr (TREE) {
    int l = 1, base = k0;
    for (;;) {
      const int T = 2 << l;
      if (T >= N) {
        for (int e = lane; e < (N >> 2); e += 64) cnt[(size_t)b * (N >> 2) + e] = 0;
        break;
      }
      const bool left = (base & T) == 0;
      const int p = left ? base + T - 1 : base - 1;
      asm volatile("s_waitcnt vmcnt(0)" ::: "memory");
      int old = 0;
      if (lane == 0) old = atomicAdd(cnt + (size_t)b * (N >> 2) + (p >> 2), 1);
      old = __builtin_amdgcn_readfirstlane(old);
      if ((old & 1) == 0) break;
      asm volatile("" ::: "memory");
      l = l + 1;
      base = left ? base : base - T;
      wave_lds_sync();
      int lane_s = lane;
      asm volatile("" : "+v"(lane_s));
      reduced_separator_mc<NX, NU, true>(d, l, base, b, lane_s, AB, QR, rhs, red, rec, F, info, store_l, lds);
    }
  }
}

}
```

### rslqr_amd/csrc/kernels_rowbcast.hpp

```cpp
#pragma once
#include "kernels_dpp.hpp"
#include "kernels_small.hpp"

namespace ndlqr {

template <int K, bool NEG>
__device__ __forceinline__ void fmac_bc4(double& a0, double& a1, double& a2, double& a3, const double x0, const double x1,
                                         const double x2, const double x3, const double y) {
  if constexpr (NEG)
    asm volatile("v_fmac_f64_dpp %0, -%4, %8 row_newbcast:%9 row_mask:0xf bank_mask:0xf\n\t"
                 "v_fmac_f64_dpp %1, -%5, %8 row_newbcast:%9 row_mask:0xf bank_mask:0xf\n\t"
                 "v_fmac_f64_dpp %2, -%6, %8 row_newbcast:%9 row_mask:0xf bank_mask:0xf\n\t"
                 "v_fmac_f64_dpp %3, -%7, %8 row_newbcast:%9 row_mask:0xf bank_mask:0xf"
                 : "+v"(a0), "+v"(a1), "+v"(a2), "+v"(a3) : "v"(x0), "v"(x1), "v"(x2), "v"(x3), "v"(y), "n"(K));
  else
    asm volatile("v_fmac_f64_dpp %0, %4, %8 row_newbcast:%9 row_mask:0xf bank_mask:0xf\n\t"
                 "v_fmac_f64_dpp %1, %5, %8 row_newbcast:%9 row_mask:0xf bank_mask:0xf\n\t"
                 "v_fmac_f64_dpp %2, %6, %8 row_newbcast:%9 row_mask:0xf bank_mask:0xf\n\t"
                 "v_fmac_f64_dpp %3, %7, %8 row_newbcast:%9 row_mask:0xf bank_mask:0xf"
                 : "+v"(a0), "+v"(a1), "+v"(a2), "+v"(a3) : "v"(x0), "v"(x1), "v"(x2), "v"(x3), "v"(y), "n"(K));
}

template <int KD, int NC, bool INIT, bool NEG = false, int NA, int NB>
__device__ __forceinline__ void rb_mul(const double (&A)[NA], double (&B)[NB], double (&out)[NC]) {
// ... 475 lines not shown
        const int w_ = 2 * ((t & 31) + 32 * it), row = w_ / W, c = w_ - row * W;
        *reinterpret_cast<double2*>(&lds.ab[t >> 5][row * WP + c]) = ta[it];
      } else {
        const int e = t + 256 * it, ec = e < NA ? e : NA - 1;
#pragma unroll
        for (int h = 0; h < 2; ++h) {
          const int ed = 2 * ec + h, kn = ed / (NX * W), w_ = ed - kn * NX * W;
          const int row = w_ / W, c = w_ - row * W;
          lds.ab[kn][row * WP + c] = h ? ta[it].y : ta[it].x;
        }
      }
    }
#pragma unroll
    for (int it = 0; it < I0; ++it) {
      const int e = t + 256 * it, ec = e < N0 ? e : N0 - 1, j = ec / (R0 / G), w_ = ec - j * (R0 / G);
#pragma unroll
      for (int h = 0; h < G; ++h) lds.rec0[j][G * w_ + h] = t0[it][h];
    }
#pragma unroll
    for (int it = 0; it < I1; ++it) {
      const int e = t + 256 * it, ec = e < N1 ? e : N1 - 1, j = ec / (REC / G), w_ = ec - j * (REC / G);
#pragma unroll
      for (int h = 0; h < G; ++h) lds.rec1[j][G * w_ + h] = t1[it][h];
    }
    (&lds.qs[0][0])[t < NQ ? t : NQ - 1] = 1.0 / tq;
    (&lds.rs[0][0])[t < NR ? t : NR - 1] = tr;
    if (t < 2 * NX) lds.ys[t < NX ? 7 : 8][t < NX ? t : t - NX] = ty;
    if constexpr (MULTI) {
      __syncthreads();
      if (t < 3 * NX) lds.rec1[t / NX][2 * NN + t % NX] = tz;
    }
  }
  __syncthreads();

  const int q = t / NX, r = t - q * NX;
  const bool sep_thread = q < 7;
  const int s = first + (sep_thread ? q : 0), l = trailing_ones(s);
  const int sbase = s - ((1 << l) - 1);
  const bool hasA = sbase > 0, hasB = sbase + (2 << l) < N;
  const int slotA = hasA ? sep_slot(sbase - 1) : 0, slotB = hasB ? sep_slot(sbase + (2 << l) - 1) : 0;
  const int kn = t / ROWS, rr = t - kn * ROWS;
  const bool out_thread = kn < KPB;
  const int kc = out_thread ? kn : 0;
  const int i = first + kc;
  const bool lam = rr < NX;
  const int col = lam ? rr : rr - NX;
  const bool needs_ab = out_thread && i < N - 1 && (lam ? i == 0 : !(i == 0 && rr < 2 * NX));
  auto ab_dot = [&](const double* y) {
    const double* am = lds.ab[kc] + col;
    double a = 0.0;
#pragma unroll
    for (int c = 0; c < NX; ++c) a = fma(am[c * WP], y[c], a);
    return a;
  };

  for (int Lv = 2; Lv >= 1; --Lv) {
    if (sep_thread && l == Lv) {
      const double* rc = lds.rec1[q >> 1];
      double a = rc[2 * NN + r];
      if (hasA) {
#pragma unroll
        for (int c = 0; c < NX; ++c) a = fma(-rc[r * NX + c], lds.ys[slotA][c], a);
      }
      if (hasB) {
#pragma unroll
        for (int c = 0; c < NX; ++c) a = fma(-rc[NN + r * NX + c], lds.ys[slotB][c], a);
      }
      lds.ys[q][r] = a;
    }
    __syncthreads();
  }
  const bool odd_state = out_thread && (kn & 1) && rr >= NX && rr < 2 * NX;
  double dot = 0.0;
  if (odd_state) {
    if (needs_ab) dot = ab_dot(lds.ys[sep_slot(i)]);
    lds.dots[kn][rr - NX] = dot;
  }
  __syncthreads();
  if (sep_thread && l == 0) {
    const int k = s - first;
    const bool fst = s == 0;
    const double* arow = lds.ab[k] + r * WP;
    double v = 0.0;
#pragma unroll
    for (int c = 0; c < W; ++c) {
      const double wq = lds.qs[k][c];
      double zh;
      if (c < NX) zh = fst ? -lds.rs[k][c] : (lds.rs[k][NX + c] + (hasA ? lds.ys[slotA][c] : 0.0)) * wq;
      else zh = lds.rs[k][NX + c] * wq;
      v = fma(arow[c], zh, v);
    }
    const double q1 = lds.qs[k + 1][r];
    v -= lds.rs[k + 1][r] + (lds.rs[k + 1][NX + r] - lds.dots[k + 1][r]) * q1;
    lds.vs[k >> 1][r] = v;
  }
  __syncthreads();
  if (t < 64) {
    const int j = t >> 4, r15 = t & 15, rc = r15 < NX ? r15 : NX - 1;
    const double* Lp = lds.rec0[j];
    const double dinv = 1.0 / Lp[rc * (rc + 1) / 2 + rc];
    double lrow[NX], lcol[NX];
#pragma unroll
    for (int c = 0; c < NX; ++c) {
      const double lo = Lp[rc * (rc + 1) / 2 + (c < rc ? c : rc)];
      const double up = Lp[(c > rc ? c : rc) * ((c > rc ? c : rc) + 1) / 2 + rc];
      lrow[c] = (c < r15 && r15 < NX) ? lo : 0.0;
      lcol[c] = (c > r15 && r15 < NX) ? up : 0.0;
    }
    double x = lds.vs[j][rc];
    sfor<NX>([&](auto cc) {
      constexpr int c = decltype(cc)::value;
      double xs = x * dinv;
      dpp_fence(xs);
      x = fma(-lrow[c], row_bc<c>(xs), x);
    });
    x = x * dinv;
    sfor<NX>([&](auto cc) {
      constexpr int c = NX - 1 - decltype(cc)::value;
      double xs = x * dinv;
      dpp_fence(xs);
      x = fma(-lcol[c], row_bc<c>(xs), x);
    });
    if (r15 < NX) lds.ys[2 * j][r15] = x * dinv;
  }
  __syncthreads();

  if (!out_thread) return;
  const double rv = lds.rs[kn][rr];
  double out;
  const double* yi = lds.ys[sep_slot(i < N - 1 ? i : i - 1)];
  const double* yp = lds.ys[sep_slot(i > 0 ? i - 1 : 0)];
  if (needs_ab && !odd_state) dot = ab_dot(yi);
  if (lam) {
    out = (i == 0) ? fma(-QR[(size_t)bp * N * W + rr], rv, -lds.rs[0][NX + rr]) + dot : yp[rr];
  } else if (rr < 2 * NX) {
    out = (i == 0) ? -lds.rs[0][rr - NX] : (rv - dot + yp[rr - NX]) * lds.qs[kn][rr - NX];
  } else {
    out = (i == N - 1) ? rv : (rv - dot) * lds.qs[kn][rr - NX];
  }
  z[((size_t)b * N + i) * ROWS + rr] = out;
}

template <int NX>
__device__ __forceinline__ double rb_llt_solve(double x, const double (&lrow)[NX], const double (&lcol)[NX], const double dinv);

__device__ __forceinline__ double rb_rcp(const double x) {
  double y = __builtin_amdgcn_rcp(x);
  y = fma(fma(-x, y, 1.0), y, y);
  return fma(fma(-x, y, 1.0), y, y);
}

constexpr int kRbBacksubColsThreads = 128;

template <int NX, int NU>
struct alignas(16) RbBacksubColsLds {
  static constexpr int NN = NX * NX, REC = 2 * NN + NX, R0 = NX * (NX + 1) / 2;
  static constexpr int R0P = (R0 + 1) / 2 * 2, RECP = REC + (REC & 1);
  static constexpr int TS = 17;
  double rec0[4][R0P];
  union {
    double rec1[3][RECP];
    double prod[4][NX * TS];
  };
  double ys[9][NX];
  double wv[4][NX];
};

template <int SZ>
__device__ __forceinline__ int rec_of(const int e) { return (e >= SZ) + (e >= 2 * SZ) + (e >= 3 * SZ); }

template <int NX, int NU, bool MULTI>
__device__ __forceinline__ void rb_backsub_cols(const Dims& d, const double* __restrict__ AB, const double* __restrict__ QR,
                                                const double* __restrict__ rhs, const double* __restrict__ recs,
                                                const double* __restrict__ ytop, double* __restrict__ z,
                                                const int nprob, const double* __restrict__ zsep) {
  using Lds = RbBacksubColsLds<NX, NU>;
  constexpr int W = NX + NU, ROWS = 2 * NX + NU, NN = NX * NX, REC = 2 * NN + NX, KPB = 8, R0 = Lds::R0, TS = Lds::TS;
  constexpr int NT = kRbBacksubColsThreads;
  static_assert(W <= 16 && NT == 128 && 3 * NX <= NT, "thread roles fit the workgroup");
  __shared__ Lds lds;
  const int N = d.N, b = blockIdx.y, first = (blockIdx.x + d.xoff) * KPB;
  const int bp = MULTI ? b % nprob : b;
  const int t = threadIdx.x;
  const int odd = t >> 6, j = (t >> 4) & 3, c = t & 15;
  const int k = 2 * j + odd, i = first + k;
  const int cw = c < W ? c : W - 1, cx = c < NX ? c : NX - 1;

  double a[NX];
  const double* abk = AB + ((size_t)bp * N + i) * NX * W + cw;
#pragma unroll
  for (int r = 0; r < NX; ++r) a[r] = abk[r * W];
  const double tq = QR[((size_t)bp * N + i) * W + cw];
  const double* rk = rhs + ((size_t)b * N + i) * ROWS;
  const double tl = rk[cx], tg = rk[NX + cw];
  {
    const double* rc0 = recs + ((size_t)bp * N + first) * REC;
    constexpr bool WIDE = NX % 2 == 0 && R0 % 2 == 0;
    constexpr int G = WIDE ? 2 : 1;
    constexpr int N0 = 4 * R0 / G, I0 = (N0 + NT - 1) / NT, N1 = 3 * REC / G, I1 = (N1 + NT - 1) / NT;
    double t0[I0][G], t1[I1][G];
#pragma unroll
    for (int it = 0; it < I0; ++it) {
      const int e = t + NT * it, ec = e < N0 ? e : N0 - 1, q = rec_of<R0 / G>(ec), w_ = ec - q * (R0 / G);
      const double* src = rc0 + (size_t)(2 * q) * REC + G * w_;
      if constexpr (WIDE) { const double2 v = *reinterpret_cast<const double2*>(src); t0[it][0] = v.x; t0[it][1] = v.y; }
      else t0[it][0] = *src;
    }
#pragma unroll
    for (int it = 0; it < I1; ++it) {
      const int e = t + NT * it, ec = e < N1 ? e : N1 - 1, q = rec_of<REC / G>(ec), w_ = ec - q * (REC / G);
      const double* src = rc0 + (size_t)(2 * q + 1) * REC + G * w_;
      if constexpr (WIDE) { const double2 v = *reinterpret_cast<const double2*>(src); t1[it][0] = v.x; t1[it][1] = v.y; }
      else t1[it][0] = *src;
    }
    double tz = 0.0;
    if constexpr (MULTI) {
      const int e = t < 3 * NX ? t : 3 * NX - 1, q = e / NX;
      tz = zsep[((size_t)b * N + first + 2 * q + 1) * NX + (e - q * NX)];
    }
    double ty = 0.0;
    if (t < 2 * NX) {
      const int sx = t < NX ? first - 1 : first + 7;
      if (sx >= 0 && sx < N - 1) ty = ytop[((size_t)b * (N >> 3) + (sx >> 3)) * NX + (t < NX ? t : t - NX)];
    }
#pragma unroll
    for (int it = 0; it < I0; ++it) {
      const int e = t + NT * it, ec = e < N0 ? e : N0 - 1, q = rec_of<R0 / G>(ec), w_ = ec - q * (R0 / G);
#pragma unroll
      for (int h = 0; h < G; ++h) lds.rec0[q][G * w_ + h] = t0[it][h];
    }
#pragma unroll
    for (int it = 0; it < I1; ++it) {
      const int e = t + NT * it, ec = e < N1 ? e : N1 - 1, q = rec_of<REC / G>(ec), w_ = ec - q * (REC / G);
      if (!MULTI || G * w_ < 2 * NN) {
#pragma unroll
        for (int h = 0; h < G; ++h) lds.rec1[q][G * w_ + h] = t1[it][h];
      }
    }
    if (t < 2 * NX) lds.ys[t < NX ? 7 : 8][t < NX ? t : t - NX] = ty;
    if constexpr (MULTI) {
      if (t < 3 * NX) lds.rec1[t / NX][2 * NN + t % NX] = tz;
    }
  }
  const double qinv = rb_rcp(tq);
  __syncthreads();

  double dot = 0.0;
  auto ab_dot = [&](const double* y) {
    double s = 0.0;
#pragma unroll
    for (int r = 0; r < NX; ++r) s = fma(a[r], y[r], s);
    return s;
  };
  if (odd) {
    auto resolve = [&](const int q, const bool hasA, const int slotA, const bool hasB, const int slotB) {
      const double* rc = lds.rec1[q >> 1];
      double s = rc[2 * NN + c];
      if (hasA) {
#pragma unroll
        for (int e = 0; e < NX; ++e) s = fma(-rc[c * NX + e], lds.ys[slotA][e], s);
      }
      if (hasB) {
#pragma unroll
        for (int e = 0; e < NX; ++e) s = fma(-rc[NN + c * NX + e], lds.ys[slotB][e], s);
      }
      lds.ys[q][c] = s;
    };
    const bool left = first > 0, right = first + KPB < N;
    if (j == 1 && c < NX) resolve(3, left, 7, right, 8);
    wave_lds_sync();
    if (j == 0 && c < NX) resolve(1, left, 7, true, 3);
    if (j == 2 && c < NX) resolve(5, true, 3, right, 8);
    wave_lds_sync();
    if (i < N - 1) dot = ab_dot(lds.ys[k < 7 ? k : 8]);
    if (c < NX) lds.wv[j][c] = tl + (tg - dot) * qinv;
  }
  __syncthreads();
  if (!odd) {
    const double ya = (i > 0 && c < NX) ? lds.ys[k > 0 ? k - 1 : 7][cx] : 0.0;
    const double zh = (i == 0 && c < NX) ? -tl : (tg + ya) * qinv;
    if (c < W) {
#pragma unroll
      for (int r = 0; r < NX; ++r) lds.prod[j][r * TS + c] = a[r] * zh;
    }
    wave_lds_sync();
    const double* pr = lds.prod[j] + cx * TS;
    double v0 = 0.0, v1 = 0.0;
#pragma unroll
    for (int m = 0; m + 1 < W; m += 2) { v0 += pr[m]; v1 += pr[m + 1]; }
    if constexpr (W % 2) v0 += pr[W - 1];
    double x = (v0 + v1) - lds.wv[j][cx];
    const double* Lp = lds.rec0[j];
    const double dinv = rb_rcp(Lp[cx * (cx + 1) / 2 + cx]);
    double lrow[NX], lcol[NX];
#pragma unroll
    for (int e = 0; e < NX; ++e) {
      const double lo = Lp[cx * (cx + 1) / 2 + (e < cx ? e : cx)];
      const double up = Lp[(e > cx ? e : cx) * ((e > cx ? e : cx) + 1) / 2 + cx];
      lrow[e] = (e < c && c < NX) ? lo : 0.0;
      lcol[e] = (e > c && c < NX) ? up : 0.0;
    }
    x = rb_llt_solve<NX>(x, lrow, lcol, dinv);
    if (c < NX) lds.ys[2 * j][c] = x;
    wave_lds_sync();
    dot = ab_dot(lds.ys[k]);
  }
  __syncthreads();

  const double yp = (i > 0 && c < NX) ? lds.ys[k > 0 ? k - 1 : 7][cx] : 0.0;
  double* zi = z + ((size_t)b * N + i) * ROWS;
  if (c < NX) {
    zi[c] = (i == 0) ? fma(-tq, tl, -tg) + dot : yp;
    zi[NX + c] = (i == 0) ? -tl : (tg - dot + yp) * qinv;
  } else if (c < W) {
    zi[NX + c] = (i == N - 1) ? tg : (tg - dot) * qinv;
  }
}

template <int NX, int NU, bool MULTI = false, bool COLS = false>
__global__ __launch_bounds__(COLS ? kRbBacksubColsThreads : 256) void rb_backsub(
    Dims d, const double* __restrict__ AB, const double* __restrict__ QR, const double* __restrict__ rhs,
    const double* __restrict__ recs, const double* __restrict__ ytop, double* __restrict__ z, const int nprob = 0,
    const double* __restrict__ zsep = nullptr) {
  if constexpr (COLS) rb_backsub_cols<NX, NU, MULTI>(d, AB, QR, rhs, recs, ytop, z, nprob, zsep);
  else rb_backsub_staged<NX, NU, MULTI>(d, AB, QR, rhs, recs, ytop, z, nprob, zsep);
}

template <int NX>
__device__ __forceinline__ double rb_llt_solve(double x, const double (&lrow)[NX], const double (&lcol)[NX], const double dinv) {
  sfor<NX>([&](auto cc) {
    constexpr int c = decltype(cc)::value;
    double xs = x * dinv;
    dpp_fence(xs);
    x = fma(-lrow[c], row_bc<c>(xs), x);
  });
  x = x * dinv;
  sfor<NX>([&](auto cc) {
    constexpr int c = NX - 1 - decltype(cc)::value;
    double xs = x * dinv;
    dpp_fence(xs);
    x = fma(-lcol[c], row_bc<c>(xs), x);
  });
  return x * dinv;
}

template <int NX, int NU>
struct alignas(16) RbForwardLds {
  static constexpr int W = NX + NU, ROWS = 2 * NX + NU, NN = NX * NX, REC = 2 * NN + NX, R0 = NX * (NX + 1) / 2;
  static constexpr int R0P = (R0 + 1) / 2 * 2, WP = RbKnot<NX, NU>::WP;
  double ab[8][NX * WP];
  double rec0[4][R0P];
  double l1[3][NN];
  double f1[3][2 * NN];
  double qs[8][W];
  double rs[8][ROWS];
  double bt[7][NX];
  double zs[4][NX];
  double gl[7][NX], gr[7][NX];
  double outl[3][NX], outr[3][NX];
};

template <int NX, int NU, bool MULTI = false>
__global__ __launch_bounds__(256) void rb_forward(Dims d, const double* __restrict__ AB, const double* __restrict__ QR,
                                                  const double* __restrict__ rhs, double* __restrict__ recs,
                                                  double* __restrict__ fsum, const int nprob = 0,
                                                  double* __restrict__ zsep = nullptr) {
  using Lds = RbForwardLds<NX, NU>;
  constexpr int W = NX + NU, ROWS = 2 * NX + NU, NN = NX * NX, REC = 2 * NN + NX, KPB = 8, WP = Lds::WP, R0 = Lds::R0;
  static_assert(7 * NX <= 256 && KPB * ROWS <= 256 && KPB * W <= 256, "thread roles fit the workgroup");
  __shared__ Lds lds;
  const int N = d.N, b = blockIdx.y, first = blockIdx.x * KPB, t = threadIdx.x;
  const int bp = MULTI ? b % nprob : b;
  {
    const double* abm = AB + ((size_t)bp * N + first) * NX * W;
    const double* rc0 = recs + ((size_t)bp * N + first) * REC;
    constexpr bool WIDE = NX % 2 == 0 && R0 % 2 == 0 && (NX * W) % 2 == 0;
    constexpr int G = WIDE ? 2 : 1;
    constexpr int NA = KPB * NX * W / G, IA = (NA + 255) / 256;
    constexpr int N0 = 4 * R0 / G, I0 = (N0 + 255) / 256, NL = 3 * NN / G, IL = (NL + 255) / 256;
    constexpr int NF = 3 * 2 * NN / G, IF = (NF + 255) / 256;
    double ta[IA][G], t0[I0][G], tl[IL][G], tf[IF][G];
    auto ld = [](const double* src, double (&dst)[G]) {
      if constexpr (WIDE) { const double2 v = *reinterpret_cast<const double2*>(src); dst[0] = v.x; dst[1] = v.y; }
      else dst[0] = *src;
    };
#pragma unroll
    for (int it = 0; it < IA; ++it) { const int e = t + 256 * it, ec = e < NA ? e : NA - 1; ld(abm + G * ec, ta[it]); }
#pragma unroll
    for (int it = 0; it < I0; ++it) {
      const int e = t + 256 * it, ec = e < N0 ? e : N0 - 1, j = ec / (R0 / G), w_ = ec - j * (R0 / G);
      ld(rc0 + (size_t)(2 * j) * REC + G * w_, t0[it]);
    }
#pragma unroll
    for (int it = 0; it < IL; ++it) {
      const int e = t + 256 * it, ec = e < NL ? e : NL - 1, j = ec / (NN / G), w_ = ec - j * (NN / G);
      ld(rc0 + (size_t)(2 * j) * REC + rb_lrec_offset<NX>() + G * w_, tl[it]);
    }
#pragma unroll
    for (int it = 0; it < IF; ++it) {
      const int e = t + 256 * it, ec = e < NF ? e : NF - 1, j = ec / (2 * NN / G), w_ = ec - j * (2 * NN / G);
      ld(rc0 + (size_t)(2 * j + 1) * REC + G * w_, tf[it]);
    }
    const double tq = QR[((size_t)bp * N + first) * W + (t < KPB * W ? t : KPB * W - 1)];
    const double tr = rhs[((size_t)b * N + first) * ROWS + (t < KPB * ROWS ? t : KPB * ROWS - 1)];
#pragma unroll
    for (int it = 0; it < IA; ++it) {
      const int e = t + 256 * it, ec = e < NA ? e : NA - 1;
#pragma unroll
      for (int h = 0; h < G; ++h) {
        const int ed = G * ec + h, kn = ed / (NX * W), w_ = ed - kn * NX * W, row = w_ / W, c = w_ - row * W;
        lds.ab[kn][row * WP + c] = ta[it][h];
      }
    }
#pragma unroll
    for (int it = 0; it < I0; ++it) {
      const int e = t + 256 * it, ec = e < N0 ? e : N0 - 1, j = ec / (R0 / G), w_ = ec - j * (R0 / G);
#pragma unroll
      for (int h = 0; h < G; ++h) lds.rec0[j][G * w_ + h] = t0[it][h];
    }
#pragma unroll
    for (int it = 0; it < IL; ++it) {
      const int e = t + 256 * it, ec = e < NL ? e : NL - 1;
#pragma unroll
      for (int h = 0; h < G; ++h) (&lds.l1[0][0])[G * ec + h] = tl[it][h];
    }
#pragma unroll
    for (int it = 0; it < IF; ++it) {
      const int e = t + 256 * it, ec = e < NF ? e : NF - 1;
#pragma unroll
      for (int h = 0; h < G; ++h) (&lds.f1[0][0])[G * ec + h] = tf[it][h];
    }
    (&lds.qs[0][0])[t < KPB * W ? t : KPB * W - 1] = 1.0 / tq;
    (&lds.rs[0][0])[t < KPB * ROWS ? t : KPB * ROWS - 1] = tr;
  }
  __syncthreads();
  const int q = t / NX, r = t - q * NX;
  const bool sep_thread = q < 7;
  if (sep_thread) {
    const int s = first + q;
    const bool fst = s == 0;
    const double* arow = lds.ab[q] + r * WP;
    double v = 0.0;
#pragma unroll
    for (int c = 0; c < W; ++c) {
      const double wq = lds.qs[q][c];
      const double zh = (c < NX && fst) ? -lds.rs[q][c] : lds.rs[q][NX + c] * wq;
      v = fma(arow[c], zh, v);
    }
    v -= lds.rs[q + 1][r] + lds.rs[q + 1][NX + r] * lds.qs[q + 1][r];
    lds.bt[q][r] = v;
  }
  __syncthreads();
  auto solve_rows = [&](const int nrows, auto sel, const bool packed) {
    if (t < 64) {
      const int j = t >> 4, r15 = t & 15, rc = r15 < NX ? r15 : NX - 1;
      const int jj = j < nrows ? j : nrows - 1;
      const int sl = sel(jj);
      double lrow[NX], lcol[NX], dinv;
      if (packed) {
        const double* Lp = lds.rec0[sl >> 1];
        dinv = 1.0 / Lp[rc * (rc + 1) / 2 + rc];
#pragma unroll
        for (int c = 0; c < NX; ++c) {
          const double lo = Lp[rc * (rc + 1) / 2 + (c < rc ? c : rc)];
          const double up = Lp[(c > rc ? c : rc) * ((c > rc ? c : rc) + 1) / 2 + rc];
          lrow[c] = (c < r15 && r15 < NX) ? lo : 0.0;
          lcol[c] = (c > r15 && r15 < NX) ? up : 0.0;
        }
      } else {
        const double* Lf = lds.l1[sl >> 1];
        dinv = 1.0 / Lf[rc * NX + rc];
#pragma unroll
        for (int c = 0; c < NX; ++c) {
          lrow[c] = (c < r15 && r15 < NX) ? Lf[rc * NX + c] : 0.0;
          lcol[c] = (c > r15 && r15 < NX) ? Lf[c * NX + rc] : 0.0;
        }
      }
// ... 131 lines not shown
```

### rslqr_amd/csrc/launch_small.hpp

```cpp
#pragma once
#include "hip_context.hpp"
#include "kernels_leaf.hpp"
#include "kernels_small.hpp"
#include "kernels_bottom_reduced.hpp"
#include "kernels_rowbcast.hpp"

constexpr int kBottomLevels = 2;

struct SmallPlan {
  bool strict, keep;
  bool lean;
  int store_l;
  bool reduced;
  bool tree;
  bool compact;
  bool rowbcast;
  bool fuse2;
  int level0;
  int ltop;
  int top_l0;
  bool top_sweeps;
  size_t top_lds;
  const char* schedule;
  bool rec_complete, rec_compact;
  bool needs_F;
};

template <int NX, int NU>
constexpr bool kRbBacksubFits = 8 * (2 * NX + NU) <= 256;

static inline unsigned apply_grid(const NdlqrHipCtx* c, const ndlqr::Dims& d) {
  return (unsigned)(c->apply_nblk > 0 ? c->apply_nblk : d.N / 8);
}
static inline ndlqr::Dims apply_dims(const NdlqrHipCtx* c, const ndlqr::Dims& d) {
  ndlqr::Dims da = d;
  if (c->apply_nblk > 0) da.xoff += c->apply_blk0;
  return da;
}

template <int NX, int NU, bool MULTI, class... Args>
static void launch_rb_backsub(const NdlqrHipCtx* c, const dim3 grid, hipStream_t stream, const Args&... args) {
  if constexpr (NX + NU <= 16) {
    if (c->knobs.backsub_cols != 0) {
      hipLaunchKernelGGL((ndlqr::rb_backsub<NX, NU, MULTI, true>), grid, dim3(ndlqr::kRbBacksubColsThreads), 0, stream, args...);
      return;
    }
  }
  hipLaunchKernelGGL((ndlqr::rb_backsub<NX, NU, MULTI, false>), grid, dim3(256), 0, stream, args...);
}

template <int NX, int NU>
static SmallPlan plan_small(const NdlqrHipCtx* c, const bool strict, const bool keep) {
  const ndlqr::Dims& d = c->d;
  const BufferSet& s = c->set[0];
  SmallPlan p = {};
  p.strict = strict;
  p.keep = keep;
  p.lean = !strict && !keep && (d.K + 4) * NX <= 256;
  p.store_l = (c->flags & NDLQR_FLAG_KEEP_RECORDS) ? 1 : 0;
  p.rec_complete = !strict && (keep || (p.lean && p.store_l));
  p.level0 = p.ltop = p.top_l0 = d.K;
  p.schedule = p.lean ? "knot-lean" : (strict ? "knot-strict" : "knot-keep");
  if constexpr (ndlqr::P1OnMatrixCores<NX, NU>::value) {
    if (p.lean && s.red) {
      p.reduced = true;
      p.tree = s.tree_cnt && (c->knobs.tree == 1 || (c->knobs.tree < 0 && (size_t)d.batch * (d.N >> 2) <= 2048));
      p.top_lds = sizeof(double) * (size_t)(d.N >> 3) * NX;
      p.compact = !p.tree && d.N >= 16 && kRbBacksubFits<NX, NU> && p.top_lds * (p.store_l ? 4 : 1) <= kLdsMax;
      if (p.compact && p.store_l) p.store_l = 2;
      p.rec_compact = p.compact && p.store_l == 2;
      p.rowbcast = p.compact && !p.store_l && NX <= 16 && NX + NU <= 16 && (c->knobs.rowbcast == 1 || (c->knobs.rowbcast < 0 && NX <= 8));
      p.fuse2 = !p.rowbcast && p.compact && !p.store_l && (c->knobs.fuse2 > 0 || (c->knobs.fuse2 < 0 && NX == 12 && NU == 4));
      p.schedule = p.tree ? "reduced-tree"
                   : !p.compact ? "reduced-records"
                   : p.store_l ? "reduced-compact-records" : (p.fuse2 ? "reduced-fused2" : "reduced");
      if (!p.tree) {
        const int top_levels = d.K - c->knobs.top_levels >= 3 ? c->knobs.top_levels : 3;
        p.level0 = p.fuse2 ? 3 : 2;
        p.ltop = (d.K >= 5 && !c->knobs.no_top) ? d.K - top_levels : d.K;
        p.top_l0 = (p.fuse2 && p.ltop < 3) ? 3 : p.ltop;
        p.top_sweeps = p.ltop < d.K && p.compact && p.top_lds <= 4 * sizeof(ndlqr::ReducedLds<NX, NU, false>);
      }
    }
  }
  p.needs_F = !(p.reduced && p.store_l != 1);
  return p;
}

template <int NX, int NU, bool STRICT, bool KEEP>
static int launch_small(NdlqrHipCtx* c, const SmallPlan& plan) {
  const ndlqr::Dims& d = c->d;
  BufferSet& s = c->set[c->cur];
  using Sh = ndlqr::SchurShape<NX, NU>;
  constexpr int JB = kBottomLevels;
  const bool lean = plan.lean;
  const int store_l = plan.store_l;
  if constexpr (!STRICT && !KEEP && ndlqr::P1OnMatrixCores<NX, NU>::value) {
    if (plan.reduced) {
      {
        ScopedSlot t(c, SLOT_BOTTOM);
        if (plan.rowbcast) {
          if constexpr (NX <= 16 && NX + NU <= 16)
            hipLaunchKernelGGL((ndlqr::rb_bottom<NX, NU>), dim3(d.N >> 4, d.batch), dim3(64), 0, s.stream, d, c->AB,
                               c->QR, s.rhs, s.red, s.rec, c->info);
        } else if (plan.fuse2) {
          hipLaunchKernelGGL((ndlqr::bottom8_reduced_mc<NX, NU>), dim3(d.N >> 3, d.batch), dim3(128), 0, s.stream, d,
                             c->AB, c->QR, s.rhs, s.red, s.rec, c->info);
        } else if (plan.tree)
          hipLaunchKernelGGL((ndlqr::bottom_reduced_mc<NX, NU, true>), dim3(d.N >> 2, d.batch), dim3(64), 0, s.stream,
                             d, c->AB, c->QR, s.rhs, s.red, s.rec, c->F, c->info, store_l, s.tree_cnt, 0);
        else if (plan.compact)
          hipLaunchKernelGGL((ndlqr::bottom_reduced_mc<NX, NU, false, true>), dim3(d.N >> 2, d.batch), dim3(64), 0, s.stream,
                             d, c->AB, c->QR, s.rhs, s.red, s.rec, c->F, c->info, store_l, nullptr, 1);
        else
          hipLaunchKernelGGL((ndlqr::bottom_reduced_mc<NX, NU, false>), dim3(d.N >> 2, d.batch), dim3(64), 0, s.stream,
                             d, c->AB, c->QR, s.rhs, s.red, s.rec, c->F, c->info, store_l, nullptr, 0);
      }
      for (int l = plan.level0; l < plan.ltop; ++l) {
        ScopedSlot t(c, SLOT_UPPER);
        hipLaunchKernelGGL((ndlqr::reduced_level_mc<NX, NU>), dim3(d.N >> (l + 1), d.batch), dim3(64), 0, s.stream,
                           d, l, c->AB, c->QR, s.rhs, s.red, s.rec, c->F, c->info, store_l);
      }
      if (plan.ltop < d.K) {
        ScopedSlot t(c, SLOT_TOP);
        hipLaunchKernelGGL((ndlqr::reduced_top_mc<NX, NU>), dim3(d.batch), dim3(256), 0, s.stream, d, plan.top_l0, c->AB,
                           c->QR, s.rhs, s.red, s.rec, c->F, c->info, store_l, plan.top_sweeps ? s.ytop : (double*)nullptr);
      }
      ScopedSlot t(c, SLOT_APPLY);
      if (plan.compact) {
        if (!plan.top_sweeps) {
          (void)allow_dynamic_lds(&ndlqr::rb_backsub_top<NX>, plan.top_lds);
          hipLaunchKernelGGL((ndlqr::rb_backsub_top<NX>), dim3(d.batch), dim3(256), plan.top_lds, s.stream, d, s.rec, s.ytop);
        }
        launch_rb_backsub<NX, NU, false>(c, dim3(apply_grid(c, d), d.batch), s.stream,
                           apply_dims(c, d), c->AB, c->QR, s.rhs, s.rec, s.ytop, s.z);
      } else {
        hipLaunchKernelGGL((ndlqr::backsub_small<NX, NU>), dim3(apply_grid(c, d), d.batch), dim3(256), 0, s.stream, apply_dims(c, d), c->AB,
                           c->QR, s.rhs, s.rec, s.z);
      }
      return NDLQR_OK;
    }
  }
  {
    ScopedSlot t(c, SLOT_BOTTOM);
    hipLaunchKernelGGL((ndlqr::bottom_small<NX, NU, STRICT, KEEP, JB>), dim3(d.N >> JB, d.batch), dim3(32 << JB), 0,
                       s.stream, d, c->AB, c->QR, s.rhs, c->F, s.z, c->info, s.rec, lean ? 1 : 0,
                       ((lean || (KEEP && !STRICT)) ? 1 : 0) | (store_l ? 2 : 0));
  }
  for (int l = JB; l < d.K; ++l) {
    ScopedSlot t(c, SLOT_UPPER);
    hipLaunchKernelGGL((ndlqr::level_small<NX, NU, STRICT, KEEP>), dim3(d.N >> (l + 1), d.batch), dim3(64), 0,
                       s.stream, d, l, c->AB, c->F, s.z, s.rec, c->info, store_l);
  }
  ScopedSlot t(c, SLOT_APPLY);
  if (lean) {
    if constexpr (!STRICT && !KEEP)
      hipLaunchKernelGGL((ndlqr::backsub_small<NX, NU>), dim3(apply_grid(c, d), d.batch), dim3(256), 0, s.stream, apply_dims(c, d), c->AB,
                         c->QR, s.rhs, s.rec, s.z);
    return NDLQR_OK;
  }
  const size_t lds = sizeof(double) * (size_t)(d.K - JB) * Sh::REC;
  hipLaunchKernelGGL((ndlqr::apply_small<NX, NU, STRICT, KEEP>), dim3(d.N / Sh::KPB, d.batch), dim3(256), lds,
                     s.stream, d, JB, c->F, s.z, s.rec);
  return NDLQR_OK;
}

template <int NX, int NU>
static void launch_rhs_records(NdlqrHipCtx* c, const double* rhs, double* z) {
  const ndlqr::Dims& d = c->d;
  BufferSet& s = c->set[c->cur];
  if constexpr (ndlqr::P1OnMatrixCores<NX, NU>::value && kRbBacksubFits<NX, NU>) {
    if (c->kept.rec_compact) {
      {
        ScopedSlot t(c, SLOT_SEP);
        hipLaunchKernelGGL((ndlqr::rb_forward<NX, NU>), dim3(d.N / 8, d.batch), dim3(256), 0, s.stream, d, c->AB, c->QR,
                           rhs, s.rec, s.red);
      }
      {
        ScopedSlot t(c, SLOT_UPPER);
        const size_t lds = sizeof(double) * 4 * (size_t)(d.N >> 3) * NX;
        (void)allow_dynamic_lds(&ndlqr::rb_forward_top<NX, NU>, lds);
        hipLaunchKernelGGL((ndlqr::rb_forward_top<NX, NU>), dim3(d.batch), dim3(256), lds, s.stream, d, c->AB, c->QR,
                           rhs, s.rec, (const double*)s.red, s.ytop);
      }
      ScopedSlot t(c, SLOT_APPLY);
      launch_rb_backsub<NX, NU, false>(c, dim3(apply_grid(c, d), d.batch), s.stream,
                         apply_dims(c, d), c->AB, c->QR, rhs, s.rec, s.ytop, z);
      return;
    }
  }
  {
    ScopedSlot t(c, SLOT_SEP);
    hipLaunchKernelGGL((ndlqr::rhs_forward_small<NX, NU>), dim3(d.N / 8, d.batch), dim3(64), 0, s.stream, d, c->AB,
                       c->QR, rhs, c->F, s.rec, z);
  }
  if (d.K > 3) {
    ScopedSlot t(c, SLOT_UPPER);
    const size_t lds = sizeof(double) * (size_t)(d.N / 8) * NX;
    hipLaunchKernelGGL((ndlqr::rhs_forward_upper<NX, NU>), dim3(d.batch), dim3(512), lds, s.stream, d, c->AB, c->QR,
                       rhs, c->F, s.rec, z);
  }
  {
    ScopedSlot t(c, SLOT_APPLY);
    hipLaunchKernelGGL((ndlqr::backsub_small<NX, NU>), dim3(apply_grid(c, d), d.batch), dim3(256), 0, s.stream, apply_dims(c, d), c->AB,
                       c->QR, rhs, s.rec, z);
  }
}

template <int NX, int NU>
static bool launch_multi_rhs(NdlqrHipCtx* c, const int count, const double* rhs, double* zsep, double* fsum, double* ytop,
                             double* z) {
  if constexpr (ndlqr::P1OnMatrixCores<NX, NU>::value && kRbBacksubFits<NX, NU>) {
    const ndlqr::Dims& d = c->d;
    BufferSet& s = c->set[c->cur];
    const size_t lds = sizeof(double) * 4 * (size_t)(d.N >> 3) * NX;
    if (lds > kLdsMax) return false;
    (void)allow_dynamic_lds(&ndlqr::rb_forward_top<NX, NU, true>, lds);
    hipLaunchKernelGGL((ndlqr::rb_forward<NX, NU, true>), dim3(d.N / 8, count), dim3(256), 0, s.stream, d, c->AB, c->QR, rhs,
                       s.rec, fsum, d.batch, zsep);
    hipLaunchKernelGGL((ndlqr::rb_forward_top<NX, NU, true>), dim3(count), dim3(256), lds, s.stream, d, c->AB, c->QR, rhs,
                       s.rec, (const double*)fsum, ytop, d.batch, zsep);
    launch_rb_backsub<NX, NU, true>(c, dim3(apply_grid(c, d), count), s.stream,
                       apply_dims(c, d), c->AB, c->QR, rhs, (const double*)s.rec, (const double*)ytop, z, d.batch,
                       (const double*)zsep);
    return true;
  } else {
    return false;
  }
}

template <int NX, int NU>
static int launch_time_shard(NdlqrHipCtx* c, const int phase, const int g, const int G) {
  ndlqr::Dims d = c->d;
  BufferSet& bs = c->set[c->cur];
  int lg = 0;
  while ((1 << lg) < G) ++lg;
  if (G < 2 || (1 << lg) != G || g < 0 || g >= G) return NDLQR_ERR_INVALID;
  if constexpr (!ndlqr::P1OnMatrixCores<NX, NU>::value) {
    return NDLQR_ERR_INVALID;
  } else {
    const int ltop = d.K - lg;
    if (!bs.red || !bs.ytop || ltop < 4 || !kRbBacksubFits<NX, NU> || (c->flags & ~NDLQR_FLAG_PROFILE)) return NDLQR_ERR_INVALID;
    const size_t top_lds = sizeof(double) * (size_t)(d.N >> 3) * NX;
    if (top_lds > kLdsMax) return NDLQR_ERR_INVALID;
    (void)allow_dynamic_lds(&ndlqr::rb_backsub_top<NX>, top_lds);
    constexpr size_t SLOT = ndlqr::RedSlot<NX>::SIZE;
    if (phase == 0) {
      for (int j = 1; j < G; ++j) {
        const int s = j * (d.N / G) - 1;
        double* p = bs.red + (size_t)(s >> 2) * SLOT;
        if (hipMemset2DAsync(p, sizeof(double) * (size_t)(d.N >> 2) * SLOT, 0, sizeof(double) * SLOT, (size_t)d.batch,
                             bs.stream) != hipSuccess)
          return NDLQR_ERR_NO_DEVICE;
      }
      {
        ScopedSlot t(c, SLOT_BOTTOM);
        const int cnt = (d.N >> 2) / G;
        d.xoff = g * cnt;
        hipLaunchKernelGGL((ndlqr::bottom_reduced_mc<NX, NU, false, true>), dim3(cnt, d.batch), dim3(64), 0, bs.stream, d,
                           c->AB, c->QR, bs.rhs, bs.red, bs.rec, c->F, c->info, 0, nullptr, 1);
      }
      for (int l = 2; l < ltop; ++l) {
        ScopedSlot t(c, SLOT_UPPER);
        const int cnt = (d.N >> (l + 1)) / G;
        d.xoff = g * cnt;
        hipLaunchKernelGGL((ndlqr::reduced_level_mc<NX, NU>), dim3(cnt, d.batch), dim3(64), 0, bs.stream, d, l, c->AB,
                           c->QR, bs.rhs, bs.red, bs.rec, c->F, c->info, 0);
      }
    } else {
      d.xoff = 0;
      for (int l = ltop; l < d.K; ++l) {
        ScopedSlot t(c, SLOT_TOP);
        hipLaunchKernelGGL((ndlqr::reduced_level_mc<NX, NU>), dim3(d.N >> (l + 1), d.batch), dim3(64), 0, bs.stream, d,
                           l, c->AB, c->QR, bs.rhs, bs.red, bs.rec, c->F, c->info, 0);
      }
      ScopedSlot t(c, SLOT_APPLY);
      hipLaunchKernelGGL((ndlqr::rb_backsub_top<NX>), dim3(d.batch), dim3(256), top_lds, bs.stream, d, bs.rec, bs.ytop);
      const int cnt = (d.N >> 3) / G;
      d.xoff = g * cnt;
      launch_rb_backsub<NX, NU, false>(c, dim3(cnt, d.batch), bs.stream, d, c->AB, c->QR,
                         bs.rhs, bs.rec, bs.ytop, bs.z);
    }
    c->kept.schedule = "reduced-time-shard";
    c->kept.family = Family::Small;
    c->kept.time_shard = true;
    return NDLQR_OK;
  }
}

struct SmallInstance {
  int nx, nu;
  int kpb;
  int slot;
  SmallPlan (*plan)(const NdlqrHipCtx*, bool strict, bool keep);
  int (*solve)(NdlqrHipCtx*, const SmallPlan&);
  void (*rhs)(NdlqrHipCtx*, const double* rhs, double* z);
  int (*tshard)(NdlqrHipCtx*, int phase, int g, int G);
  bool (*multi)(NdlqrHipCtx*, int count, const double* rhs, double* zsep, double* fsum, double* ytop, double* z);
};

template <int NX, int NU>
static int solve_small(NdlqrHipCtx* c, const SmallPlan& p) {
  if (p.strict) return p.keep ? launch_small<NX, NU, true, true>(c, p) : launch_small<NX, NU, true, false>(c, p);
  return p.keep ? launch_small<NX, NU, false, true>(c, p) : launch_small<NX, NU, false, false>(c, p);
}

template <int NX, int NU>
static SmallInstance make_small_instance() {
  return {NX, NU, ndlqr::SchurShape<NX, NU>::KPB, (int)ndlqr::RedSlot<NX>::SIZE, plan_small<NX, NU>, solve_small<NX, NU>,
          launch_rhs_records<NX, NU>, launch_time_shard<NX, NU>, launch_multi_rhs<NX, NU>};
}
#define NDLQR_SMALL_NAME_(NX_, NU_) ndlqr_small_##NX_##_##NU_
#define NDLQR_SMALL_NAME(NX_, NU_) NDLQR_SMALL_NAME_(NX_, NU_)
```

### rslqr_amd/csrc/ndlqr_hip.hip

```cpp
#include "hip_host.hpp"
#include "kernels_generic.hpp"
#include "kernels_mfma.hpp"
#include "launch_reduced.hpp"
#include "kernels_reduced_solve.hpp"
#include "launch_small.hpp"


static thread_local std::string g_last_error = "";

const char* ndlqr_hip_last_error(void) { return g_last_error.c_str(); }

int ndlqr_hip_fail(const char* what, hipError_t e) {
  g_last_error = std::string(what) + ": " + hipGetErrorString(e);
  fprintf(stderr, "ndlqr_hip: %s\n", g_last_error.c_str());
  if (e == hipErrorInvalidConfiguration || e == hipErrorInvalidValue) return NDLQR_ERR_INVALID;
  return NDLQR_ERR_NO_DEVICE;
}
int fail(const char* what, hipError_t e) { return ndlqr_hip_fail(what, e); }
int refuse(const std::string& msg) {
  g_last_error = msg;
  fprintf(stderr, "ndlqr_hip: %s\n", g_last_error.c_str());
  return NDLQR_ERR_INVALID;
}

int need_unpadded_horizon(const NdlqrHipCtx* c, const char* who) {
  if (c->du.N == c->d.N) return NDLQR_OK;
  return refuse(std::string(who) + ": not available for a padded horizon (horizon " + std::to_string(c->du.N) +
                " runs as " + std::to_string(c->d.N) + " knots); use a power-of-two horizon");
}

int need_diagonal_cost(const NdlqrHipCtx* c, const char* who) {
  if (!c->cost.dense) return NDLQR_OK;
  return refuse(std::string(who) + ": not available in dense-cost mode (the resident problem is the unit-cost reduction "
                "ndlqr_InitializeBatchFlatDense left); use a diagonal initialiser");
}

Where where(const void* p, int device) {
  hipPointerAttribute_t a;
  if (hipPointerGetAttributes(&a, p) != hipSuccess) { (void)hipGetLastError(); return Where::Pageable; }
  if (a.type == hipMemoryTypeDevice) return a.device == device ? Where::OwnDevice : Where::OtherDevice;
  return a.type == hipMemoryTypeHost ? Where::Pinned : Where::Pageable;
}

int ndlqr_hip_device_count(void) {
  int count = 0;
  if (hipGetDeviceCount(&count) != hipSuccess) return 0;
  return count;
}

static const char* kSlotNames[SLOT_COUNT] = {"leaf", "separator", "schur", "schur_boundary", "apply", "bottom", "upper", "top"};

#ifdef NDLQR_SINGLE_TU
#define NDLQR_SMALL_INSTANCE(NX_, NU_) static const SmallInstance NDLQR_SMALL_NAME(NX_, NU_) = make_small_instance<NX_, NU_>();
#else
#define NDLQR_SMALL_INSTANCE(NX_, NU_) extern const SmallInstance NDLQR_SMALL_NAME(NX_, NU_);
#endif
#include "small_instances.def"
#undef NDLQR_SMALL_INSTANCE

static const SmallInstance* const kSmallInstances[] = {
#define NDLQR_SMALL_INSTANCE(NX_, NU_) &NDLQR_SMALL_NAME(NX_, NU_),
#include "small_instances.def"
#undef NDLQR_SMALL_INSTANCE
};

static bool has_small_instance(int nstates, int ninputs) {
  for (const SmallInstance* s : kSmallInstances)
    if (s->nx == nstates && s->nu == ninputs) return true;
  return false;
}

static void pick_pad_instance(int nstates, int ninputs, int* pn, int* pm) {
  long best = -1;
  for (const SmallInstance* si : kSmallInstances) {
    if (si->nx < nstates || si->nu < ninputs || si->nx < 6) continue;
    const long cost = (long)si->nx * si->nx * (si->nx + si->nu);
    if (best < 0 || cost < best) { best = cost; *pn = si->nx; *pm = si->nu; }
  }
}

static const SmallInstance* find_small(const ndlqr::Dims& d) {
  for (const SmallInstance* s : kSmallInstances)
    if (s->nx == d.n && s->nu == d.m) return s;
  return nullptr;
}

static size_t bytes_z(const ndlqr::Dims& d) { return sizeof(double) * doubles_z(d); }
static size_t bytes_F(const ndlqr::Dims& d) { return sizeof(double) * doubles_F(d); }

static DevKnobs read_knobs() {
  DevKnobs k;
  const auto num = [](const char* name, int* v) { if (getenv(name)) *v = atoi(getenv(name)); };
  const auto onoff = [](const char* name, int* v) { if (getenv(name)) *v = atoi(getenv(name)) != 0 ? 1 : 0; };
  num("NDLQR_PIPELINE", &k.pipeline);
  onoff("NDLQR_TREE", &k.tree);
  onoff("NDLQR_ROWBCAST", &k.rowbcast);
  onoff("NDLQR_FUSE2", &k.fuse2);
  onoff("NDLQR_BACKSUB_COLS", &k.backsub_cols);
  k.no_mfma = getenv("NDLQR_NO_MFMA") != nullptr;
  k.no_top = getenv("NDLQR_NO_TOP") != nullptr;
  num("NDLQR_TOP_LEVELS", &k.top_levels);
  if (k.top_levels < 3 || k.top_levels > 5) k.top_levels = 3;
  num("NDLQR_SEP_THREADS", &k.sep_threads);
  num("NDLQR_MULT_THREADS", &k.mult_threads);
  k.no_reduced_generic = getenv("NDLQR_DEV_NO_REDUCED_GENERIC") != nullptr;
  k.no_pad = getenv("NDLQR_NO_PAD") != nullptr;
  k.alt_priority_set = getenv("NDLQR_ALT_PRIORITY") != nullptr;
  num("NDLQR_ALT_PRIORITY", &k.alt_priority);
  return k;
}

static bool alloc_set(NdlqrHipCtx* c, BufferSet& s, bool slots) {
  const ndlqr::Dims& d = c->d;
  hipError_t e = first_error({hipEventCreate(&s.ev_start), hipEventCreate(&s.ev_stop), s.rec.ensure((size_t)d.batch * d.N * (2 * d.n * d.n + d.n)),
                              s.rhs.ensure(doubles_z(d)), s.h_fail.ensure_zeroed(1)});
  if (e == hipSuccess && slots) {
    const size_t slot_doubles = ((size_t)d.n * (d.n + 1) + 2 * (size_t)d.n * d.n + 2 * d.n + 15) / 16 * 16;
    e = first_error({s.red.ensure_zeroed((size_t)d.batch * (d.N / 4) * slot_doubles, s.stream),
                     s.ytop.ensure((size_t)d.batch * (d.N / 8) * d.n),
                     s.tree_cnt.ensure_zeroed((size_t)d.batch * (d.N / 4), s.stream)});
  }
  return e == hipSuccess && s.z.ensure_zeroed(doubles_z(d), s.stream) == hipSuccess;
}

NdlqrHipCtx* ndlqr_hip_create(int nstates, int ninputs, int nhorizon, int batch, int device) {
  return ndlqr_hip_create_ex(nstates, ninputs, nhorizon, batch, device, 0u);
}

NdlqrHipCtx* ndlqr_hip_create_ex(int nstates, int ninputs, int nhorizon, int batch, int device, unsigned create_flags) {
  if (nstates <= 0 || ninputs <= 0 || batch <= 0 || nhorizon < 2 || nhorizon > (1 << 24)) {
    g_last_error = "invalid dimensions";
    return nullptr;
  }
  if (batch > 65535) {
    g_last_error = "batch > 65535 problems per solver: split the batch over several solvers";
    fprintf(stderr, "ndlqr_hip: %s\n", g_last_error.c_str());
    return nullptr;
  }
  int count = 0;
  hipError_t e = hipGetDeviceCount(&count);
  if (e != hipSuccess || count <= 0) {
    g_last_error = std::string("no HIP device: ") + (e != hipSuccess ? hipGetErrorString(e) : "device count is 0");
    return nullptr;
  }
  if (device < 0) {
    if (hipGetDevice(&device) != hipSuccess) device = 0;
  }
  if (device >= count) {
    g_last_error = "device index out of range";
    return nullptr;
  }
  if ((e = hipSetDevice(device)) != hipSuccess) { fail("hipSetDevice", e); return nullptr; }

  NdlqrHipCtx* c = new NdlqrHipCtx();
  c->knobs = read_knobs();
  c->pipeline = c->knobs.pipeline;
  ndlqr::Dims& d = c->d;
  int phorizon = 1;
  while (phorizon < nhorizon) phorizon <<= 1;
  auto set_dims = [&](ndlqr::Dims& x, int n_, int m_, int N_) {
    x.n = n_; x.m = m_; x.N = N_; x.batch = batch;
    x.K = 0; while ((1 << x.K) < phorizon) ++x.K;
    x.rows = 2 * n_ + m_; x.w = n_ + m_; x.fb = x.rows * n_; x.xoff = 0;
  };
  set_dims(c->du, nstates, ninputs, nhorizon);
  nhorizon = phorizon;
  int pn = nstates, pm = ninputs;
  const bool may_pad = !c->knobs.no_pad && !(create_flags & NDLQR_CREATE_NO_PAD);
  if (!has_small_instance(nstates, ninputs) && nhorizon >= 8 && may_pad)
    pick_pad_instance(nstates, ninputs, &pn, &pm);
  if (nstates > 128 && (nstates % 16 != 0 || (nstates + ninputs) % 4 != 0) && may_pad) {
    pn = (nstates + 15) / 16 * 16;
    pm = ninputs + (4 - (pn + ninputs) % 4) % 4;
  }
  set_dims(d, pn, pm, phorizon);
  c->padded = pn != nstates || pm != ninputs || c->du.N != d.N;
  c->device = device;
  BufferSet& s = c->set[0];
  bool ok = hipStreamCreateWithFlags(&s.stream, hipStreamNonBlocking) == hipSuccess &&
            hipEventCreateWithFlags(&c->ev_inputs, hipEventDisableTiming) == hipSuccess &&
            hipEventCreateWithFlags(&c->ev_step[0], hipEventDisableTiming) == hipSuccess &&
            hipEventCreateWithFlags(&c->ev_step[1], hipEventDisableTiming) == hipSuccess &&
            c->AB.ensure((size_t)d.batch * d.N * d.n * d.w) == hipSuccess && c->QR.ensure(doubles_QR(d)) == hipSuccess &&
            alloc_set(c, s, nhorizon >= 8 && has_small_instance(d.n, d.m));
  if (ok && c->padded) {
    hipLaunchKernelGGL(ndlqr::pad_fill_generic, dim3(d.N, d.batch), dim3(128), 0, s.stream, d, c->AB, c->QR, s.rhs);
    ok = hipGetLastError() == hipSuccess;
  }
  ok = ok && c->info.ensure_zeroed((size_t)batch + 1, s.stream) == hipSuccess && hipStreamSynchronize(s.stream) == hipSuccess;
  if (!ok) {
    fail("device allocation", hipGetLastError());
    ndlqr_hip_destroy(c);
    return nullptr;
  }
  s.ready = true;
  return c;
}

static void free_set(NdlqrHipCtx* c, int i) {
  BufferSet& s = c->set[i];
  if (s.stream) (void)hipStreamSynchronize(s.stream);
  s.graph.reset();
  if (s.ev_start) (void)hipEventDestroy(s.ev_start);
  if (s.ev_stop) (void)hipEventDestroy(s.ev_stop);
  if (s.stream && (i == 1 || c->own_stream)) (void)hipStreamDestroy(s.stream);
  s = BufferSet();
}

void ndlqr_hip_destroy(NdlqrHipCtx* c) {
  if (!c) return;
  (void)hipSetDevice(c->device);
  for (int i = 1; i >= 0; --i) free_set(c, i);
  c->staged.reset();
  for (auto& p : c->pending) { (void)hipEventDestroy(p.start); (void)hipEventDestroy(p.stop); }
  for (auto& ev : c->event_pool) (void)hipEventDestroy(ev);
  if (c->ev_inputs) (void)hipEventDestroy(c->ev_inputs);
  for (hipEvent_t ev : c->ev_step) if (ev) (void)hipEventDestroy(ev);
  delete c;
}


void note_solution(NdlqrHipCtx* c) {
  ++c->soln_gen;
  c->latest = c->cur;
  c->z_partial = c->apply_nblk > 0;
  c->z_invalid = false;
  c->z_blk0 = c->apply_blk0;
  c->z_nblk = c->apply_nblk;
}
static void next_solve_on_current_set(NdlqrHipCtx* c) {
  if ((c->solve_count & 1u) != (unsigned)c->cur) ++c->solve_count;
}
int need_full_solution(const NdlqrHipCtx* c, const char* who) {
  if (c->z_invalid)
    return refuse(std::string(who) + ": the last constrained solve failed; there is no resident solution until the next solve");
  if (!c->z_partial) return NDLQR_OK;
  g_last_error = std::string(who) + ": the last step computed only knots " + std::to_string(8 * c->z_blk0) + " .. " +
                 std::to_string(8 * (c->z_blk0 + c->z_nblk) - 1) + " (NDLQR_SOLN_ONLY); run a solve or a step without it first";
  return NDLQR_ERR_INVALID;
}

static bool ensure_alt(NdlqrHipCtx* c) {
  BufferSet& a = c->set[1];
  if (a.ready) return true;
  const BufferSet& p = c->set[0];
  int prio_least = 0, prio_greatest = 0;
  (void)hipDeviceGetStreamPriorityRange(&prio_least, &prio_greatest);
  const int alt_prio = c->knobs.alt_priority_set ? c->knobs.alt_priority : prio_greatest;
  bool ok = hipStreamCreateWithPriority(&a.stream, hipStreamNonBlocking, alt_prio) == hipSuccess &&
            alloc_set(c, a, p.tree_cnt != nullptr);
  ok = ok && hipStreamSynchronize(p.stream) == hipSuccess &&
// ... 300 lines not shown
  const size_t lds = sizeof(double) * (2 * (size_t)d.w + d.n + 3 * (size_t)np + 256 + (size_t)d.n * (d.n + 1) / 2);
  for (int l = 0; l < d.K; ++l) {
    ScopedSlot t(c, SLOT_SEP);
    hipLaunchKernelGGL(ndlqr::rhs_reduced_generic, dim3(d.N >> (l + 1), d.batch), dim3(256), lds, s.stream, d, l, np,
                       c->AB, c->QR, rhs, s.red, s.rec);
  }
  launch_backsub_reduced_generic(c, rhs, z);
}

struct GenericSepPlan {
  bool mfma;
  bool scratch;
  size_t lds;
  int threads;
  int schur_nb;
};
static GenericSepPlan plan_generic_sep(const NdlqrHipCtx* c, const bool strict) {
  const ndlqr::Dims& d = c->d;
  GenericSepPlan p;
  p.schur_nb = (strict || d.n % 16 != 0 || c->knobs.no_mfma) ? -1 : (d.n > 64 ? 0 : (d.rows % 16 == 0 ? d.n / 16 : -1));
  p.mfma = !strict && d.n % 16 == 0 && d.w % 4 == 0 && !c->knobs.no_mfma;
  p.scratch = false;
  const int ctl = 2 * (d.n / 16) + 1, ctc = ctl < kSepChunkTiles ? ctl : kSepChunkTiles;
  const size_t lds_mfma = sizeof(double) * ((size_t)d.n * (d.n + 1) + (size_t)d.n * (16 * ctc + 1) + (size_t)d.n * 17);
  const size_t lds_generic = sizeof(double) * ((size_t)d.n * (d.n + 1) + (size_t)d.n * (2 * d.n + 1));
  p.threads = c->knobs.sep_threads > 0 ? c->knobs.sep_threads : (d.n >= 32 ? 512 : 256);
  if (p.mfma) {
    const int need = (d.n / 16) > ((d.n / 16) * ctc + 2) / 3 ? (d.n / 16) : ((d.n / 16) * ctc + 2) / 3;
    if (p.threads < 64 * need) p.threads = 64 * need;
    if (p.threads > 1024) p.mfma = false;
  }
  if (p.mfma) {
    const size_t lds_no_s = lds_mfma - sizeof(double) * (size_t)d.n * (d.n + 1);
    if (lds_mfma <= kLdsMax) { p.lds = lds_mfma; return p; }
    if (lds_no_s <= kLdsMax) { p.lds = lds_no_s; p.scratch = true; return p; }
    p.mfma = false;
  }
  p.scratch = lds_generic > kLdsMax;
  p.lds = p.scratch ? 0 : lds_generic;
  p.threads = p.scratch ? 1024 : 256;
  return p;
}

struct SolvePlan {
  Family family;
  const SmallInstance* inst;
  SmallPlan small;
  ReducedGenericPlan red;
  GenericSepPlan sep;
  bool strict, keep;
  bool lean;
  bool rec_as_factors;
  bool needs_F;
  size_t sep_scratch_bytes;
  bool needs_red_generic;
  bool may_pipeline;
  KeptState kept;
};

template <bool STRICT>
static int launch_generic(NdlqrHipCtx* c, const SolvePlan& plan) {
  const ndlqr::Dims& d = c->d;
  BufferSet& s = c->set[c->cur];
  const bool lean = plan.lean;
  double* rec = lean ? s.rec : nullptr;
  {
    ScopedSlot t(c, SLOT_LEAF);
    hipLaunchKernelGGL((ndlqr::leaf_generic<STRICT>), dim3(d.N, d.batch), dim3(128), 0, s.stream, d,
                       c->AB, c->QR, s.rhs, c->F, s.z, c->info, lean ? 1 : 0);
  }
  const GenericSepPlan& sp = plan.sep;
  const bool p1mfma = sp.mfma;
  const size_t lds = sp.lds;
  const int sep_threads = sp.threads;
  double* sep_scratch = sp.scratch ? c->sep_scratch : nullptr;
  for (int l = 0; l < d.K; ++l) {
    const int nsub = d.N >> (l + 1);
    {
      ScopedSlot t(c, SLOT_SEP);
      if (p1mfma)
        hipLaunchKernelGGL((ndlqr::separator_mfma<kSepChunkTiles>), dim3(nsub, d.batch), dim3(sep_threads), lds,
                           s.stream, d, l, c->AB, c->F, s.z, c->info, rec, sep_scratch,
                           (size_t)d.n * (d.n + 1) + (size_t)d.n * (2 * d.n + 1));
      else
        hipLaunchKernelGGL((ndlqr::separator_generic<STRICT>), dim3(nsub, d.batch), dim3(sep_threads), lds,
                           s.stream, d, l, c->AB, c->F, s.z, c->info, rec, sep_scratch);
    }
    if (lean && l == d.K - 1) break;
    {
      ScopedSlot t(c, lean ? SLOT_BOUNDARY : SLOT_SCHUR);
      const int bnd = lean ? 1 : 0;
      const unsigned gx = lean ? 2u * (unsigned)nsub : (unsigned)d.N;
      const size_t flds = sizeof(double) * (size_t)d.n * (d.n + 16);
      if (sp.schur_nb == 4)
        hipLaunchKernelGGL((ndlqr::schur_mfma<4>), dim3(gx, d.batch), dim3(256), flds, s.stream, d, l, c->F, s.z, bnd,
                           (const double*)rec);
      else if (sp.schur_nb == 3)
        hipLaunchKernelGGL((ndlqr::schur_mfma<3>), dim3(gx, d.batch), dim3(256), flds, s.stream, d, l, c->F, s.z, bnd,
                           (const double*)rec);
      else if (sp.schur_nb == 2)
        hipLaunchKernelGGL((ndlqr::schur_mfma<2>), dim3(gx, d.batch), dim3(256), flds, s.stream, d, l, c->F, s.z, bnd,
                           (const double*)rec);
      else if (sp.schur_nb == 1)
        hipLaunchKernelGGL((ndlqr::schur_mfma<1>), dim3(gx, d.batch), dim3(256), flds, s.stream, d, l, c->F, s.z, bnd,
                           (const double*)rec);
      else if (sp.schur_nb == 0)
        hipLaunchKernelGGL(ndlqr::schur_mfma_rt, dim3(gx, d.batch), dim3(256), 0, s.stream, d, l, c->F, s.z, bnd,
                           (const double*)rec);
      else {
        const long work = (long)gx * d.rows * d.n;
        hipLaunchKernelGGL((ndlqr::schur_generic<STRICT>), dim3((unsigned)((work + 255) / 256), d.batch),
                           dim3(256), 0, s.stream, d, l, c->F, s.z, bnd, (const double*)rec);
      }
    }
  }
  if (lean) {
    ScopedSlot t(c, SLOT_APPLY);
    for (int l = d.K - 1; l >= 0; --l) {
      hipLaunchKernelGGL(ndlqr::backsub_multipliers_generic, dim3(d.N >> (l + 1), d.batch), dim3(64), 0, s.stream,
                         d, l, s.rec, s.z);
    }
    const int work = d.N * d.rows;
    hipLaunchKernelGGL(ndlqr::backsub_states_generic, dim3((work + 255) / 256, d.batch), dim3(256), 0, s.stream, d,
                       c->AB, c->QR, s.rhs, s.z);
  }
  return NDLQR_OK;
}

static const SmallInstance* pick_small(const NdlqrHipCtx* c) {
  const ndlqr::Dims& d = c->d;
  if (c->flags & NDLQR_FLAG_GENERIC) return nullptr;
  const SmallInstance* inst = find_small(d);
  if (!inst || d.N < inst->kpb || d.K < 3) return nullptr;
  return inst;
}

static const SmallInstance* kept_instance(const NdlqrHipCtx* c) {
  return c->kept.family == Family::Small ? find_small(c->d) : nullptr;
}

static SolvePlan plan_solve(const NdlqrHipCtx* c) {
  const ndlqr::Dims& d = c->d;
  SolvePlan p = {};
  p.strict = (c->flags & NDLQR_FLAG_STRICT_FP) != 0;
  p.keep = (c->flags & NDLQR_FLAG_KEEP_FACT) != 0;
  p.inst = pick_small(c);
  if (p.inst) {
    p.family = Family::Small;
    p.small = p.inst->plan(c, p.strict, p.keep);
    p.needs_F = p.small.needs_F;
    p.kept.schedule = p.small.schedule;
    p.kept.rec_complete = p.small.rec_complete;
    p.kept.rec_compact = p.small.rec_compact;
  } else if ((p.red = plan_reduced_generic(c)).ok) {
    p.family = Family::GenericReduced;
    p.needs_red_generic = true;
    p.kept.schedule = p.red.keep ? "generic-reduced-records" : "generic-reduced";
    p.kept.rec_complete = p.red.keep;
  } else {
    p.family = Family::GenericKnot;
    p.rec_as_factors = (c->flags & NDLQR_FLAG_KEEP_RECORDS) && !p.strict;
    p.lean = !p.strict && !p.keep && !p.rec_as_factors;
    p.needs_F = true;
    p.sep = plan_generic_sep(c, p.strict);
    if (p.sep.scratch)
      p.sep_scratch_bytes = sizeof(double) * ((size_t)d.n * (d.n + 1) + (size_t)d.n * (2 * d.n + 1)) * (size_t)d.batch *
                            (d.N / 2 > 0 ? d.N / 2 : 1);
    p.kept.schedule = p.lean ? "generic-lean" : (p.strict ? "generic-strict" : "generic-keep");
  }
  p.kept.family = p.family;
  p.kept.fact_valid = p.keep || p.rec_as_factors || ((c->flags & NDLQR_FLAG_GENERIC) && p.strict);
  p.may_pipeline = !p.needs_F && !(c->flags & (NDLQR_FLAG_PROFILE | NDLQR_FLAG_KEEP_RECORDS | NDLQR_FLAG_KEEP_FACT));
  return p;
}

static int enqueue_solve(NdlqrHipCtx* c, const SolvePlan& plan) {
  BufferSet& s = c->set[c->cur];
  int err = NDLQR_OK;
  switch (plan.family) {
    case Family::Small: err = plan.inst->solve(c, plan.small); break;
    case Family::GenericReduced: err = launch_reduced_generic(c, plan.red); break;
    default: err = plan.strict ? launch_generic<true>(c, plan) : launch_generic<false>(c, plan); break;
  }
  if (!err) HIP_TRY(hipMemcpyAsync(s.h_fail, c->info + c->d.batch, sizeof(int), hipMemcpyDeviceToHost, s.stream));
  return err;
}

static int prepare_solve(NdlqrHipCtx* c, SolvePlan* plan) {
  HIP_TRY(hipSetDevice(c->device));
  *plan = plan_solve(c);
  if (plan->needs_F) {
    const int ferr = ndlqr_hip_ensure_F(c);
    if (ferr) return ferr;
  }
  if (plan->sep_scratch_bytes && c->sep_scratch.ensure(plan->sep_scratch_bytes / sizeof(double)) != hipSuccess) {
    (void)hipGetLastError();
    return refuse("global scratch of the large-block separator kernel does not fit on the device (" +
                  std::to_string(plan->sep_scratch_bytes >> 20) + " MiB): use a smaller batch");
  }
  if (c->state_dirty) {
    (void)sync_all(c);
    const hipStream_t st = c->set[c->cur].stream;
    for (const BufferSet& s : c->set)
      if (s.tree_cnt) HIP_TRY(hipMemsetAsync(s.tree_cnt, 0, sizeof(int) * (size_t)c->d.batch * (c->d.N / 4), st));
    HIP_TRY(hipMemsetAsync(c->info, 0, sizeof(int) * ((size_t)c->d.batch + 1), st));
    HIP_TRY(hipStreamSynchronize(st));
    for (const BufferSet& s : c->set)
      if (s.h_fail) *s.h_fail = 0;
    c->fail_base = 0;
    c->state_dirty = false;
  }
  const bool pipelined = c->pipeline >= 2 && c->own_stream && plan->may_pipeline;
  const bool want_alt = pipelined && (c->solve_count & 1u) && ensure_alt(c);
  if (!pipelined && c->set[1].stream) HIP_TRY(hipStreamSynchronize(c->set[1].stream));
  if (plan->needs_red_generic) {
    const int rerr = ensure_red_generic(c);
    if (rerr) return rerr;
  }
  c->cur = want_alt ? 1 : 0;
  ++c->solve_count;
  c->state_dirty = true;
  return NDLQR_OK;
}

static int replay_chain(NdlqrHipCtx* c, CapturedChain& g, const SolvePlan& plan, int (*enqueue)(NdlqrHipCtx*, const SolvePlan&)) {
  const hipStream_t st = c->set[c->cur].stream;
  const unsigned apply = ((unsigned)c->apply_blk0 << 16) | (unsigned)c->apply_nblk;
  if (!g.exec || g.flags != c->flags || g.stream != st || g.apply != apply) {
    g.reset();
    hipGraph_t graph = nullptr;
    HIP_TRY(hipStreamBeginCapture(st, hipStreamCaptureModeThreadLocal));
    const int err = enqueue(c, plan);
    hipError_t e = hipStreamEndCapture(st, &graph);
    if (err) { if (graph) (void)hipGraphDestroy(graph); return err; }
    if (e != hipSuccess) return fail("hipStreamEndCapture", e);
    e = hipGraphInstantiate(&g.exec, graph, nullptr, nullptr, 0);
    (void)hipGraphDestroy(graph);
    if (e != hipSuccess) { g.exec = nullptr; return fail("hipGraphInstantiate", e); }
    g.flags = c->flags;
    g.stream = st;
    g.apply = apply;
  }
  HIP_TRY(hipGraphLaunch(g.exec, st));
  return NDLQR_OK;
}

static int launch_solve(NdlqrHipCtx* c, const SolvePlan& plan) {
  c->kept.rec_complete = c->kept.rec_compact = false;
  const int err = (c->flags & NDLQR_FLAG_PROFILE) ? enqueue_solve(c, plan)
                                                  : replay_chain(c, c->set[c->cur].graph, plan, enqueue_solve);
  if (err) return err;
  HIP_TRY(hipGetLastError());
  note_solution(c);
  c->kept = plan.kept;
  c->inputs_replaced = false;
  c->forget_shifted();
  ++c->factor_count;
  return NDLQR_OK;
}

int ndlqr_hip_solve_async(NdlqrHipCtx* c) {
  if (!c) return NDLQR_ERR_INVALID;
  SolvePlan plan;
  int err = prepare_solve(c, &plan);
  if (err) return err;
  BufferSet& s = c->set[c->cur];
  err = rhs_make_current(c, 0xFu);
  if (err) return err;
  HIP_TRY(hipEventRecord(s.ev_start, s.stream));
  err = launch_solve(c, plan);
  if (err) return err;
  HIP_TRY(hipEventRecord(s.ev_stop, s.stream));
  c->timing_pending = true;
  c->state_dirty = false;
  return NDLQR_OK;
}

static size_t staged_doubles(const ndlqr::Dims& u, size_t* oAB, size_t* oQR, size_t* orhs, size_t* oz) {
  const size_t nAB = (size_t)u.batch * u.N * u.n * u.w, nQR = (size_t)u.batch * u.N * u.w, nz = (size_t)u.batch * u.N * u.rows;
  *oAB = 0; *oQR = nAB; *orhs = nAB + nQR; *oz = nAB + nQR + nz;
  return nAB + nQR + 2 * nz;
}

int ndlqr_hip_staged_io(NdlqrHipCtx* c, double** AB, double** QR, double** rhs, double** z) {
  if (!c || !AB || !QR || !rhs || !z) return NDLQR_ERR_INVALID;
  if (const int herr = need_unpadded_horizon(c, "ndlqr_hip_staged_io")) return herr;
  if (const int cerr = need_diagonal_cost(c, "ndlqr_hip_staged_io")) return cerr;
  HIP_TRY(hipSetDevice(c->device));
  size_t oAB, oQR, orhs, oz;
  const size_t total = staged_doubles(c->du, &oAB, &oQR, &orhs, &oz);
  if (!c->h_io) {
    HIP_TRY(c->h_io.ensure(total));
    if (c->padded) {
      HIP_TRY(c->grow_pad_stage(total));
    }
    const int perr = ndlqr_hip_set_pipeline_depth(c, 1);
    if (perr) return perr;
  }
  *AB = c->h_io + oAB; *QR = c->h_io + oQR; *rhs = c->h_io + orhs; *z = c->h_io + oz;
  return NDLQR_OK;
}

static int enqueue_staged(NdlqrHipCtx* c, const SolvePlan& plan) {
  const ndlqr::Dims& d = c->d;
  const ndlqr::Dims& u = c->du;
  BufferSet& s = c->set[c->cur];
// ... 520 lines not shown
  if (sets > (size_t)nrhs) sets = (size_t)nrhs;
  if (sets == 0) return NDLQR_ERR_INVALID;
  if (c->multi.ensure(d, u, sets * per_set, st.stream) != hipSuccess) {
    (void)hipGetLastError();
    g_last_error = "buffers of the multiple right-hand sides do not fit on the device";
    return NDLQR_ERR_INVALID;
  }
  double total_ms = 0.0;
  for (size_t s0 = 0; s0 < (size_t)nrhs; s0 += sets) {
    const size_t ns = (size_t)nrhs - s0 < sets ? (size_t)nrhs - s0 : sets, count = ns * per_set;
    ndlqr::Dims uc = u, dc = d;
    uc.batch = dc.batch = (int)count;
    const size_t nq = count * u.N * u.n, nr = count * u.N * u.m, nx = count * u.n;
    double* in = c->multi.in;
    HIP_TRY(hipMemcpyAsync(in, q + s0 * per_set * u.N * u.n, sizeof(double) * nq, hipMemcpyHostToDevice, st.stream));
    HIP_TRY(hipMemcpyAsync(in + nq, r + s0 * per_set * u.N * u.m, sizeof(double) * nr, hipMemcpyHostToDevice, st.stream));
    HIP_TRY(hipMemcpyAsync(in + nq + nr, dd + s0 * per_set * u.N * u.n, sizeof(double) * nq, hipMemcpyHostToDevice, st.stream));
    HIP_TRY(hipMemcpyAsync(in + 2 * nq + nr, x0 + s0 * per_set * u.n, sizeof(double) * nx, hipMemcpyHostToDevice, st.stream));
    hipLaunchKernelGGL(ndlqr::pack_rhs_stream_generic<false>, dim3(512), dim3(256), 0, st.stream, uc, dc, (const double*)in,
                       (const double*)(in + nq), (const double*)(in + nq + nr), (const double*)(in + 2 * nq + nr), c->multi.rhs);
    HIP_TRY(hipGetLastError());
    HIP_TRY(hipEventRecord(st.ev_start, st.stream));
    const ApplySlice apply_slice(c, sel);
    if (!inst->multi(c, (int)count, c->multi.rhs, c->multi.zsep, c->multi.fsum, c->multi.ytop, c->multi.z)) {
      g_last_error = "multiple right-hand sides: this shape / horizon has no such form";
      return NDLQR_ERR_INVALID;
    }
    HIP_TRY(hipGetLastError());
    HIP_TRY(hipEventRecord(st.ev_stop, st.stream));
    const int derr = deliver(uc, dc, sel, c->multi.z, soln + s0 * per_set * sel.doubles(u), false, c->multi.out,
                             hipMemcpyDeviceToHost, st.stream, (unsigned)count);
    if (derr) return derr;
    HIP_TRY(hipStreamSynchronize(st.stream));
    float ms = 0.0f;
    if (hipEventElapsedTime(&ms, st.ev_start, st.ev_stop) == hipSuccess) total_ms += ms;
  }
  c->last_ms = total_ms;
  c->timing_pending = false;
  return NDLQR_OK;
}
int ndlqr_hip_solve_multi_rhs(NdlqrHipCtx* c, int nrhs, const double* q, const double* r, const double* dd,
                              const double* x0, double* soln) {
  return solve_multi_rhs(c, nrhs, q, r, dd, x0, KnotSlice(), soln);
}
int ndlqr_hip_solve_multi_rhs_slices(NdlqrHipCtx* c, int nrhs, const double* q, const double* r, const double* dd,
                                     const double* x0, int knot0, int nknots, unsigned blocks, double* out) {
  if (nknots <= 0) return NDLQR_ERR_INVALID;
  return solve_multi_rhs(c, nrhs, q, r, dd, x0, KnotSlice{knot0, nknots, blocks}, out);
}

int ndlqr_hip_synchronize(NdlqrHipCtx* c) {
  if (!c) return NDLQR_ERR_INVALID;
  HIP_TRY(hipSetDevice(c->device));
  {
    const hipError_t se = sync_all(c);
    if (se != hipSuccess) { c->state_dirty = true; return fail("hipStreamSynchronize", se); }
  }
  if (c->timing_pending) {
    float ms = 0;
    HIP_TRY(hipEventElapsedTime(&ms, c->set[c->cur].ev_start, c->set[c->cur].ev_stop));
    c->last_ms = ms;
    c->timing_pending = false;
    int seen = 0;
    for (const BufferSet& s : c->set)
      if (s.h_fail && *s.h_fail > seen) seen = *s.h_fail;
    c->last_failures = seen - c->fail_base;
    c->fail_base = seen;
  }
  for (auto& p : c->pending) {
    float ms = 0;
    if (hipEventElapsedTime(&ms, p.start, p.stop) == hipSuccess) {
      c->slot_ms[p.slot] += ms;
      c->slot_launches[p.slot] += 1;
    }
    c->event_pool.push_back(p.start);
    c->event_pool.push_back(p.stop);
  }
  c->pending.clear();
  return NDLQR_OK;
}

double ndlqr_hip_last_solve_ms(NdlqrHipCtx* c) { return c ? c->last_ms : -1.0; }
int ndlqr_hip_cholesky_failures(NdlqrHipCtx* c) { return c ? c->last_failures : NDLQR_ERR_INVALID; }

int ndlqr_hip_profile_slots(NdlqrHipCtx* c) { return c ? (int)SLOT_COUNT : 0; }
int ndlqr_hip_profile_get(NdlqrHipCtx* c, int slot, char* name, int name_cap, double* total_ms, int* launches) {
  if (!c || slot < 0 || slot >= SLOT_COUNT) return NDLQR_ERR_INVALID;
  if (name && name_cap > 0) { strncpy(name, kSlotNames[slot], (size_t)name_cap - 1); name[name_cap - 1] = '\0'; }
  if (total_ms) *total_ms = c->slot_ms[slot];
  if (launches) *launches = c->slot_launches[slot];
  return NDLQR_OK;
}
int ndlqr_hip_profile_reset(NdlqrHipCtx* c) {
  if (!c) return NDLQR_ERR_INVALID;
  memset(c->slot_ms, 0, sizeof(c->slot_ms));
  memset(c->slot_launches, 0, sizeof(c->slot_launches));
  return NDLQR_OK;
}


int ndlqr_hip_download_solutions(NdlqrHipCtx* c, int p0, int count, double* soln) {
  if (!c || !soln || p0 < 0 || count <= 0 || p0 + count > c->d.batch) return NDLQR_ERR_INVALID;
  if (c->z_partial || c->z_invalid) return need_full_solution(c, "ndlqr_hip_download_solutions");
  return download_packed(c, c->set[c->latest].z, p0, count, soln);
}
int download_packed(NdlqrHipCtx* c, const double* zsrc, int p0, int count, double* soln) {
  const ndlqr::Dims& d = c->d;
  BufferSet& s = c->set[c->cur];
  HIP_TRY(hipSetDevice(c->device));
  HIP_TRY(sync_all(c));
  HIP_TRY(s.ensure_xfer(c->du));
  const size_t nvars = (size_t)c->du.rows * c->du.N - c->du.m, pitch = (size_t)d.rows * d.N;
  hipStream_t st = s.stream;
  HIP_TRY(launch_pack(c->du, d, KnotSlice(), zsrc + p0 * pitch, s.xfer, st, count));
  const bool in_callers = (zsrc == c->set[c->latest].z && c->cost.mapped(c->soln_gen)) || (zsrc == c->adj.z && c->lin_adjoint_resident());
  if (c->cost.dense && !in_callers) HIP_TRY(cost_map_back(c, s.xfer, p0, count, st));
  const size_t total = nvars * count;
  if (where(soln, c->device) == Where::Pinned) {
    HIP_TRY(hipMemcpyAsync(soln, s.xfer, sizeof(double) * total, hipMemcpyDeviceToHost, st));
    HIP_TRY(hipStreamSynchronize(st));
    return NDLQR_OK;
  }
  const size_t chunk = (8u << 20) / sizeof(double);
  if (total <= chunk / 8) {
    HIP_TRY(hipMemcpyAsync(soln, s.xfer, sizeof(double) * total, hipMemcpyDeviceToHost, st));
    HIP_TRY(hipStreamSynchronize(st));
    return NDLQR_OK;
  }
  for (int i = 0; i < 2; ++i)
    HIP_TRY(c->h_stage[i].ensure(chunk));
  hipEvent_t done[2] = {take_event(c), take_event(c)};
  const size_t nchunks = (total + chunk - 1) / chunk;
  hipError_t e = hipSuccess;
  for (size_t i = 0; i <= nchunks && e == hipSuccess; ++i) {
    if (i < nchunks) {
      const size_t off = i * chunk, len = total - off < chunk ? total - off : chunk;
      e = hipMemcpyAsync(c->h_stage[i & 1], s.xfer + off, sizeof(double) * len, hipMemcpyDeviceToHost, st);
      if (e == hipSuccess) e = hipEventRecord(done[i & 1], st);
    }
    if (i > 0 && e == hipSuccess) {
      const size_t off = (i - 1) * chunk, len = total - off < chunk ? total - off : chunk;
      e = hipEventSynchronize(done[(i - 1) & 1]);
      if (e == hipSuccess) memcpy(soln + off, c->h_stage[(i - 1) & 1], sizeof(double) * len);
    }
  }
  c->event_pool.push_back(done[0]);
  c->event_pool.push_back(done[1]);
  if (e != hipSuccess) return fail("ndlqr_hip_download_solutions", e);
  return NDLQR_OK;
}

const char* ndlqr_hip_schedule(const NdlqrHipCtx* c) { return c ? c->kept.schedule : "none"; }

int ndlqr_hip_factors_valid(const NdlqrHipCtx* c) { return c && c->kept.fact_valid ? 1 : 0; }

int ndlqr_hip_pack_solutions_device(NdlqrHipCtx* c, double* dst) {
  if (!c || !dst) return NDLQR_ERR_INVALID;
  if (c->z_partial || c->z_invalid) return need_full_solution(c, "ndlqr_hip_pack_solutions_device");
  const ndlqr::Dims& d = c->d;
  HIP_TRY(hipSetDevice(c->device));
  HIP_TRY(launch_pack(c->du, d, KnotSlice(), c->set[c->latest].z, dst, c->set[c->latest].stream, d.batch));
  if (c->cost.dense && !c->cost.mapped(c->soln_gen)) HIP_TRY(cost_map_back(c, dst, 0, d.batch, c->set[c->latest].stream));
  return NDLQR_OK;
}

int ndlqr_hip_kkt_residual(NdlqrHipCtx* c, double* res, double* bnorm) {
  if (!c || !res) return NDLQR_ERR_INVALID;
  if (const int cerr = need_diagonal_cost(c, "ndlqr_hip_kkt_residual")) return cerr;
  if (c->z_partial || c->z_invalid) return need_full_solution(c, "ndlqr_hip_kkt_residual");
  const ndlqr::Dims& d = c->d;
  BufferSet& s = c->set[c->cur];
  HIP_TRY(hipSetDevice(c->device));
  HIP_TRY(c->kkt_out.ensure(2 * (size_t)d.batch));
  double* out = c->kkt_out;
  HIP_TRY(sync_all(c));
  hipLaunchKernelGGL(ndlqr::kkt_residual_generic, dim3(d.batch), dim3(256), 0, s.stream, d, c->AB, c->QR, s.rhs,
                     c->set[c->latest].z, out);
  hipError_t e = hipGetLastError();
  if (e == hipSuccess) e = hipMemcpyAsync(res, out, sizeof(double) * d.batch, hipMemcpyDeviceToHost, s.stream);
  if (e == hipSuccess && bnorm)
    e = hipMemcpyAsync(bnorm, out + d.batch, sizeof(double) * d.batch, hipMemcpyDeviceToHost, s.stream);
  if (e == hipSuccess) e = hipStreamSynchronize(s.stream);
  if (e != hipSuccess) return fail("ndlqr_hip_kkt_residual", e);
  return NDLQR_OK;
}

int ndlqr_hip_download_rhs_blocks(NdlqrHipCtx* c, int p, double* z_full) {
  if (!c || !z_full || p < 0 || p >= c->d.batch) return NDLQR_ERR_INVALID;
  if (const int herr = need_unpadded_horizon(c, "ndlqr_hip_download_rhs_blocks")) return herr;
  if (const int cerr = need_diagonal_cost(c, "ndlqr_hip_download_rhs_blocks")) return cerr;
  if (c->z_partial || c->z_invalid) return need_full_solution(c, "ndlqr_hip_download_rhs_blocks");
  const ndlqr::Dims& d = c->d;
  BufferSet& s = c->set[c->cur];
  HIP_TRY(hipSetDevice(c->device));
  const size_t pitch = (size_t)d.rows * d.N;
  HIP_TRY(sync_all(c));
  const double* zp = c->set[c->latest].z + p * pitch;
  if (c->padded) {
    const size_t upitch = (size_t)c->du.rows * d.N;
    HIP_TRY(c->grow_pad_stage(upitch));
    hipLaunchKernelGGL(ndlqr::unpad_blocks_generic, dim3(d.N), dim3(64), 0, s.stream, c->du, d, zp, c->pad_stage);
    HIP_TRY(hipGetLastError());
    HIP_TRY(hipMemcpyAsync(z_full, c->pad_stage, sizeof(double) * upitch, hipMemcpyDeviceToHost, s.stream));
  } else {
    HIP_TRY(hipMemcpyAsync(z_full, zp, sizeof(double) * pitch, hipMemcpyDeviceToHost, s.stream));
  }
  HIP_TRY(hipStreamSynchronize(s.stream));
  return NDLQR_OK;
}

int ndlqr_hip_download_factors(NdlqrHipCtx* c, int p, double* fact) {
  if (!c || !fact || p < 0 || p >= c->d.batch) return NDLQR_ERR_INVALID;
  if (const int herr = need_unpadded_horizon(c, "ndlqr_hip_download_factors")) return herr;
  if (const int cerr = need_diagonal_cost(c, "ndlqr_hip_download_factors")) return cerr;
  if (!c->kept.fact_valid) return refuse("factor download needs NDLQR_FLAG_KEEP_FACT set before the solve");
  const ndlqr::Dims& d = c->d;
  BufferSet& s = c->set[c->cur];
  HIP_TRY(hipSetDevice(c->device));
  const size_t count = (size_t)d.K * d.N * d.fb;
  std::vector<double> tmp(count);
  HIP_TRY(hipMemcpyAsync(tmp.data(), c->F + p * count, sizeof(double) * count, hipMemcpyDeviceToHost, s.stream));
  HIP_TRY(hipStreamSynchronize(s.stream));
  const int n = c->du.n, m = c->du.m, np = d.n;
  const size_t ufb = c->du.fb;
  for (int lvl = 0; lvl < d.K; ++lvl)
    for (int k = 0; k < d.N; ++k) {
      const double* src = tmp.data() + ((size_t)lvl * d.N + k) * d.fb;
      double* dst = fact + ((size_t)k + (size_t)d.N * lvl) * ufb;
      for (int j = 0; j < n; ++j) {
        for (int i = 0; i < n; ++i) dst[i + n * j] = src[i * np + j];
        for (int i = 0; i < n; ++i) dst[n * n + i + n * j] = src[(np + i) * np + j];
        for (int i = 0; i < m; ++i) dst[2 * n * n + i + m * j] = src[(2 * np + i) * np + j];
      }
    }
  return NDLQR_OK;
}

extern "C" long ndlqr_hip_debug_download(NdlqrHipCtx* c, int which, double* host, long count) {
  if (!c || !host) return -1;
  const ndlqr::Dims& d = c->d;
  BufferSet& s = c->set[c->cur];
  const double* src = which == 0 ? s.rec : s.red;
  const size_t slot_doubles = ((size_t)d.n * (d.n + 1) + 2 * (size_t)d.n * d.n + 2 * d.n + 15) / 16 * 16;
  const size_t have = which == 0 ? (size_t)d.batch * d.N * (2 * d.n * d.n + d.n) : (size_t)d.batch * (d.N / 4) * slot_doubles;
  if (!src) return -1;
  const size_t n = (size_t)count < have ? (size_t)count : have;
  if (hipStreamSynchronize(s.stream) != hipSuccess) return -1;
  if (hipMemcpy(host, src, n * sizeof(double), hipMemcpyDeviceToHost) != hipSuccess) return -1;
  return (long)n;
}

#ifdef NDLQR_SEGTIME
extern "C" int ndlqr_hip_debug_segments(unsigned long long* out, int n, int reset) {
  unsigned long long host[128];
  if (hipMemcpyFromSymbol(host, HIP_SYMBOL(ndlqr::ndlqr_seg), sizeof(host)) != hipSuccess) return -1;
  for (int i = 0; i < n && i < 128; ++i) out[i] = host[i];
  if (reset) {
    for (int i = 0; i < 128; ++i) host[i] = 0;
    if (hipMemcpyToSymbol(HIP_SYMBOL(ndlqr::ndlqr_seg), host, sizeof(host)) != hipSuccess) return -1;
  }
  return 128;
}
#endif
```

### rslqr_amd/roofline.py

```python
import math

HBM_PEAK_GBS = 8000.0
FP64_PEAK_TFLOPS = 78.6


def record_doubles(n, level, compact_level0=False):
    if compact_level0 and level == 0:
        return n * (n + 1) // 2
    return 2 * n * n + n


def separator_flops(n, w):
    leaf = 2 * n * n * w + 2 * n * w
    chol = n ** 3 / 3.0
    solves = 2 * n * n * (2 * n + 1)
    schur = 4 * n ** 3 + 4 * n * n
    return leaf + chol + solves + schur


def backsub_flops(n, m, N):
    w = n + m
    return (N - 1) * 4 * n * n + N * (2 * n * w + 3 * (2 * n + m))


def inputs_doubles(n, m, N):
    return N * (n * (n + m) + (n + m) + (2 * n + m))


def compulsory_bytes(n, m, N):
    return 8 * (inputs_doubles(n, m, N) + N * (2 * n + m))


def reduced_model(n, m, N, compact_level0=False, fused2=False):
    K = int(math.log2(N))
    if fused2 and N >= 16:
        base = reduced_model(n, m, N, compact_level0, False)
        w, rows = n + m, 2 * n + m
        tri = n * (n + 1) // 2
        rec0, rec = record_doubles(n, 0, compact_level0), record_doubles(n, 1)
        fs = separator_flops(n, w)
        push = 2 * tri + n * n + 2 * n
        slot = 2 * tri + 2 * n * n + 2 * n
        per_sep = slot + n * w + w + n + rows + 2 * n + rec + push
        nsep2 = N // 8
        base["bottom"] = {"bytes": 8 * (inputs_doubles(n, m, N) + (N // 2) * rec0 + (N // 4 + nsep2) * rec +
                                       nsep2 * (4 * (tri + n) + n * n)),
                          "flops": (3 * N // 4 + nsep2) * fs, "launches": 1}
        if "upper" in base:
            left = base["upper"]["bytes"] // 8 // per_sep - nsep2
            if left > 0:
                base["upper"] = {"bytes": 8 * left * per_sep, "flops": left * fs, "launches": base["upper"]["launches"] - 1}
            else:
                del base["upper"]
        elif "top" in base and K == 5:
            sweep_b = (N // 8 - 1) * rec + (N // 8) * n
            base["top"] = {"bytes": 8 * (3 * per_sep + sweep_b), "flops": 3 * fs + (N // 8 - 1) * 4 * n * n, "launches": 1}
        return base
    w, rows = n + m, 2 * n + m
    tri = n * (n + 1) // 2
    push = 2 * tri + n * n + 2 * n
    slot = 2 * tri + 2 * n * n + 2 * n
    rec0 = record_doubles(n, 0, compact_level0)
    rec = record_doubles(n, 1)
    fs = separator_flops(n, w)
    nsep_upper = max(N // 4 - 1, 0)
    bottom_b = inputs_doubles(n, m, N) + (N // 2) * rec0 + (N // 4) * rec + (N // 4) * push
    upper_b = nsep_upper * (slot + n * w + w + n + rows + 2 * n + rec + push)
    recs_read = (N // 2) * rec0 + (N // 4) * rec + nsep_upper * rec
    apply_b = recs_read + inputs_doubles(n, m, N) + N * rows + ((N // 8) * n + (N // 8) * 2 * n if compact_level0 else 0)
    out = {
        "bottom": {"bytes": 8 * bottom_b, "flops": (3 * N // 4) * fs, "launches": 1},
        "apply": {"bytes": 8 * apply_b, "flops": backsub_flops(n, m, N), "launches": 1},
    }
    if K > 2:
        out["upper"] = {"bytes": 8 * upper_b, "flops": nsep_upper * fs, "launches": K - 2}
    if K >= 5 and compact_level0:
        per_sep = upper_b // nsep_upper
        sweep_b = (N // 8 - 1) * rec + (N // 8) * n
        sweep_f = (N // 8 - 1) * 4 * n * n
        out["top"] = {"bytes": 8 * (7 * per_sep + sweep_b), "flops": 7 * fs + sweep_f, "launches": 1}
        out["upper"] = {"bytes": 8 * (nsep_upper - 7) * per_sep, "flops": (nsep_upper - 7) * fs, "launches": K - 5}
        out["apply"] = {"bytes": out["apply"]["bytes"] - 8 * sweep_b, "flops": out["apply"]["flops"] - sweep_f,
                        "launches": 1}
        if nsep_upper == 7:
            del out["upper"]
    return out


def knot_lean_model(n, m, N):
    K = int(math.log2(N))
    w, rows = n + m, 2 * n + m
    fb = rows * n
    rec = 2 * n * n + n
    fs = separator_flops(n, w)
    bottom_b = inputs_doubles(n, m, N) + (3 * N // 4) * rec + (N // 2) * (2 * fb + rows)
    out = {"bottom": {"bytes": 8 * bottom_b, "flops": (3 * N // 4) * fs + N * 4 * fb * n, "launches": 1},
           "apply": {"bytes": 8 * ((N - 1) * rec + inputs_doubles(n, m, N) + N * rows),
                     "flops": backsub_flops(n, m, N), "launches": 1}}
    if K > 2:
        nsep = N // 4 - 1
        per = (2 * w * n + 2 * n * n + rows + 2 * n + n * w) + rec + 2 * (3 * fb + 2 * rows)
        out["upper"] = {"bytes": 8 * nsep * per, "flops": nsep * (fs + 2 * 4 * fb * n), "launches": K - 2}
    return out


def generic_lean_model(n, m, N):
    K = int(math.log2(N))
    w, rows = n + m, 2 * n + m
    fb_xu = w * n
    rec = 2 * n * n + n
    out = {
        "leaf": {"bytes": 8 * (inputs_doubles(n, m, N) + N * (2 * fb_xu + rows)),
                 "flops": N * (2 * w * n + 4 * rows), "launches": 1},
    }
    sep_b = sep_f = sch_b = sch_f = 0
    for l in range(K):
        L = N >> (l + 1)
        sep_b += L * (n * w + 2 * fb_xu + 2 * n * n + rows + 2 * n + rec)
        sep_f += L * (4 * n * n * w + n ** 3 / 3.0 + 2 * n * n * (2 * n + 1))
        if l < K - 1:
            sch_b += 2 * L * (fb_xu + 3 * fb_xu + 2 * rows) + L * 2 * n * n
            sch_f += 2 * L * (2 * 2 * fb_xu * n + 2 * w * n)
    out["separator"] = {"bytes": 8 * sep_b, "flops": sep_f, "launches": K}
    out["schur_boundary"] = {"bytes": 8 * sch_b, "flops": sch_f, "launches": K - 1}
    out["apply"] = {"bytes": 8 * ((N - 1) * rec + inputs_doubles(n, m, N) + N * rows),
                    "flops": backsub_flops(n, m, N), "launches": 1}
    return out


def generic_reduced_model(n, m, N):
    K = int(math.log2(N))
    w, rows = n + m, 2 * n + m
    rec0 = n * (n + 1) // 2 + n
    sym = min(n * n, n * (n + 16) // 2)
    slot = 2 * sym + 2 * n * n + 2 * n
    push = 2 * sym + n * n + 2 * n
    sep_b = 0
    for l in range(K):
        L = N >> (l + 1)
        own = n * w + (w + n) + (rows + 2 * n)
        if l == 0:
            sep_b += L * (own + n * n + rec0 + push)
        else:
            sep_b += L * (own + slot + rec0 + push + (2 * sym + 2 * n))
    return {
        "separator": {"bytes": 8 * sep_b, "flops": (N - 1) * separator_flops(n, w), "launches": K},
        "apply": {"bytes": 8 * ((N - 1) * rec0 + (N // 2 - 1) * 2 * n * n + inputs_doubles(n, m, N) + N * rows),
                  "flops": backsub_flops(n, m, N) + (N - 1) * 2 * n * n, "launches": 1},
    }


def model_for(schedule, n, m, N):
    if schedule == "reduced":
        return reduced_model(n, m, N, compact_level0=True)
    if schedule == "reduced-fused2":
        return reduced_model(n, m, N, compact_level0=True, fused2=True)
    if schedule in ("reduced-tree", "reduced-records"):
        return reduced_model(n, m, N)
    if schedule == "knot-lean":
        return knot_lean_model(n, m, N)
    if schedule == "generic-lean":
        return generic_lean_model(n, m, N)
    if schedule in ("generic-reduced", "generic-reduced-records"):
        return generic_reduced_model(n, m, N)
    return None


def model_b_bytes(n, m, N):
    K = int(math.log2(N))
    Fb = (2 * n + m) * n
    total = N * (4 * n * n + 3 * m * n + m * m + 5 * n + 3 * m)
    for l in range(K):
        L = 1 << (K - l - 1)
        P1 = L * (K - l) * (4 * n * n + 2 * m * n) + L * (n * n + n * m)
        P2 = 2 * L * n * n
        P3 = L * n * n + 2 * L * (K - l - 1) * n * n
        P4 = (N * Fb if l < K - 1 else 0) + L * (K - l - 1) * n * n + 2 * N * (K - l - 1) * Fb
        S = L * (2 * n * n + n * m + 8 * n + 2 * m) + N * (Fb + 5 * n + 2 * m)
        total += P1 + P2 + P3 + P4 + S
    return 8 * total


def model_b_flops(n, m, N):
    K = int(math.log2(N))
    Fb = (2 * n + m) * n
    fl = N * (n ** 3 / 3 + m ** 3 / 3 + 4 * n ** 3 + 2 * m * m * n)
    for l in range(K):
        L = 1 << (K - l - 1)
        fl += L * (K - l) * 4 * n * n * (n + m) + L * n ** 3 / 3 + L * (K - l - 1) * 2 * n ** 3
        fl += N * (K - l - 1) * 2 * Fb * n
        fl += L * (4 * n * (n + m) + 2 * n * n) + N * 2 * Fb
    return fl


def kernel_roofline(slot_model, batch, avg_launch_ms, launches=None):
    launches = launches or slot_model["launches"]
    b = slot_model["bytes"] * batch / launches
    f = slot_model["flops"] * batch / launches
    gbs = b / (avg_launch_ms * 1e-3) / 1e9
    tfl = f / (avg_launch_ms * 1e-3) / 1e12
    hbm_frac, fp_frac = gbs / HBM_PEAK_GBS, tfl / FP64_PEAK_TFLOPS
    if hbm_frac >= fp_frac:
        head = {"bound": "hbm", "achieved": gbs, "peak": HBM_PEAK_GBS, "unit": "GB/s", "frac": hbm_frac}
    else:
        head = {"bound": "mfma", "achieved": tfl, "peak": FP64_PEAK_TFLOPS, "unit": "TFLOP/s", "frac": fp_frac}
    head.update(avg_launch_ms=avg_launch_ms, algorithmic_bytes_per_launch=b, useful_flops_per_launch=f,
                hbm_gbs=gbs, hbm_frac=hbm_frac, fp64_tflops=tfl, fp64_frac=fp_frac)
    return head
```

Before: 1.910 million solves/s.

## Store compact triangular Cholesky records at level 1 and recompute in backsub

Adds a compact level-1 record mode in which the bottom reduced kernel stores only the triangular Cholesky factor for level-1 separators instead of the full 2n^2+n record. The column backsub kernel then loads six triangular factors and recomputes the level-1 separator values with extra triangular solves and LDS syncs. This is meant to cut HBM record traffic in the factor and apply phases, at the cost of extra recomputation and synchronisation in backsub. It is gated by the NDLQR_COMPACT1 environment knob and a compile-time fit check.

New measurement: 1.967 million solves/s, median of 6. 2.9% higher.

```diff
diff --git a/include/ndlqr_hip.h b/include/ndlqr_hip.h
--- a/include/ndlqr_hip.h
+++ b/include/ndlqr_hip.h
@@ -128,6 +128,7 @@
 int ndlqr_hip_kkt_residual(NdlqrHipCtx* ctx, double* res, double* bnorm);
 int ndlqr_hip_cholesky_failures(NdlqrHipCtx* ctx);
 const char* ndlqr_hip_schedule(const NdlqrHipCtx* ctx);
+int ndlqr_hip_compact_level1(const NdlqrHipCtx* ctx);
 
 int ndlqr_hip_profile_slots(NdlqrHipCtx* ctx);
 int ndlqr_hip_profile_get(NdlqrHipCtx* ctx, int slot, char* name, int name_cap, double* total_ms,
diff --git a/rslqr_amd/api.py b/rslqr_amd/api.py
--- a/rslqr_amd/api.py
+++ b/rslqr_amd/api.py
@@ -308,6 +308,8 @@
     proto("ndlqr_hip_upload_inputs", ci, vp, ci, ci, dp, dp, dp)
     proto("ndlqr_hip_factors_valid", ci, vp)
     proto("ndlqr_hip_schedule", C.c_char_p, vp)
+    if hasattr(L, "ndlqr_hip_compact_level1"):
+        proto("ndlqr_hip_compact_level1", C.c_int, vp)
     proto("ndlqr_hip_set_pipeline_depth", ci, vp, ci)
     proto("ndlqr_hip_pipeline_depth", ci, vp)
     proto("ndlqr_hip_pack_solutions_device", ci, vp, vp)
@@ -1078,6 +1080,9 @@
     def schedule(self):
         return self.L.ndlqr_hip_schedule(self.ctx).decode()
 
+    def compact_level1(self):
+        return hasattr(self.L, "ndlqr_hip_compact_level1") and bool(self.L.ndlqr_hip_compact_level1(self.ctx))
+
     def set_pipeline_depth(self, depth):
         return self.L.ndlqr_hip_set_pipeline_depth(self.ctx, depth)
 
diff --git a/rslqr_amd/csrc/hip_context.hpp b/rslqr_amd/csrc/hip_context.hpp
--- a/rslqr_amd/csrc/hip_context.hpp
+++ b/rslqr_amd/csrc/hip_context.hpp
@@ -50,6 +50,7 @@
   bool rec_compact = false;
   bool fact_valid = false;
   const char* schedule = "none";
+  bool rec1_compact = false;
   void forget_factorisation() { rec_complete = fact_valid = false; }
 };
 
@@ -152,6 +153,7 @@
   int tree = -1;
   int backsub_cols = -1;
   int fuse2 = -1;
+  int compact1 = -1;
   int pipeline = 2;
   bool no_top = false;
   int top_levels = 3;
diff --git a/rslqr_amd/csrc/kernels_bottom_reduced.hpp b/rslqr_amd/csrc/kernels_bottom_reduced.hpp
--- a/rslqr_amd/csrc/kernels_bottom_reduced.hpp
+++ b/rslqr_amd/csrc/kernels_bottom_reduced.hpp
@@ -603,14 +603,14 @@
   }
 }
 
-template <int NX, int NU, bool TREE, bool REDIRECT>
+template <int NX, int NU, bool TREE, bool REDIRECT, bool C1 = false>
 __device__ __forceinline__ void bottom_group_mc(const Dims& d, const int k0, const int b, const int lane,
                                                 const double* __restrict__ AB, const double* __restrict__ QR,
                                                 const double* __restrict__ rhs, double* red, double* __restrict__ rec,
                                                 double* F, int* __restrict__ info, const int store_l, const int compact0,
                                                 ReducedLds<NX, NU>& lds, double* slotA, double* slotB,
                                                 const bool with_m = false, acc4_t* c_m = nullptr);
-template <int NX, int NU>
+template <int NX, int NU, bool C1 = false>
 __global__ __launch_bounds__(128) __attribute__((amdgpu_waves_per_eu(4))) void bottom8_reduced_mc(
     Dims d, const double* __restrict__ AB, const double* __restrict__ QR, const double* __restrict__ rhs, double* red,
     double* __restrict__ rec, int* __restrict__ info) {
@@ -622,7 +622,7 @@
   for (int e = threadIdx.x; e < RedSlot<NX>::SIZE; e += 128) mslot[e] = 0.0;
   __syncthreads();
   acc4_t c_m = {0.0, 0.0, 0.0, 0.0};
-  bottom_group_mc<NX, NU, false, true>(d, kw + 4 * wave, b, lane, AB, QR, rhs, red, rec, nullptr, info, 0, 1, lds[wave],
+  bottom_group_mc<NX, NU, false, true, C1>(d, kw + 4 * wave, b, lane, AB, QR, rhs, red, rec, nullptr, info, 0, 1, lds[wave],
                                        wave == 1 ? mslot : nullptr, wave == 0 ? mslot : nullptr, wave == 0, &c_m);
   asm volatile("s_waitcnt vmcnt(0)" ::: "memory");
   __syncthreads();
@@ -661,7 +661,7 @@
   if (ytop) backsub_top_body<NX>(d, b, threadIdx.x, rec, ytop, reinterpret_cast<double*>(&lds[0]), -1, nullptr);
 }
 
-template <int NX, int NU, bool TREE, bool REDIRECT>
+template <int NX, int NU, bool TREE, bool REDIRECT, bool C1>
 __device__ __forceinline__ void bottom_group_mc(const Dims& d, const int k0, const int b, const int lane,
                                                 const double* __restrict__ AB, const double* __restrict__ QR,
                                                 const double* __restrict__ rhs, double* red, double* __restrict__ rec,
@@ -857,6 +857,25 @@
   if constexpr (REDIRECT) {
     if (slotA) sa.p = slotA;
     if (slotB) sb.p = slotB;
+  }
+  if constexpr (C1) {
+    static_assert(!TREE, "the tree schedule keeps full records");
+    if (chol_pair_y_mc<NX>(lane, c_t, c_t, lds.buf, wcol, myrec + REC, myrec + REC) && lane == 0) flag_failure(info, d, b);
+    SEG(34);
+    using PY = McPairYLayout<NX>;
+    double y0[KSN], y1[KSN];
+    acc4_t Z0 = {0.0, 0.0, 0.0, 0.0}, Z1 = {0.0, 0.0, 0.0, 0.0};
+#pragma unroll
+    for (int q = 0; q < KSN; ++q) {
+      y0[q] = lds.buf[PY::tile(0, 0) + (4 * q + lk) * PY::YP + li];
+      y1[q] = lds.buf[PY::tile(0, 1) + (4 * q + lk) * PY::YP + li];
+      Z0[q] = y0[q]; Z1[q] = y1[q];
+    }
+    acc4_t g00, g01, g11;
+    gram_mc<NX, true, true, false, true>(y0, y1, Z0, Z1, g00, g01, unused, g11);
+    push_mc<NX>(lane, hasA, hasB, leftchild, sa, sb, g00, g01, g11, park_a, cb_t, park_b11, StorePlain(), StorePlain());
+    SEG(36);
+    return;
   }
   if (chol_wy_mc<NX>(lane, c_t, lds.buf, wcol, lstore_of<NX>(store_l, F, rec, d, b, 1, k0 + 1)) && lane == 0)
     flag_failure(info, d, b);
@@ -879,15 +898,15 @@
   SEG(36);
 }
 
-template <int NX, int NU, bool TREE, bool COMPACT = false>
+template <int NX, int NU, bool TREE, bool COMPACT = false, bool C1 = false>
 __global__ __launch_bounds__(64) __attribute__((amdgpu_waves_per_eu(4))) void bottom_reduced_mc(
     Dims d, const double* __restrict__ AB, const double* __restrict__ QR, const double* __restrict__ rhs,
     double* red, double* __restrict__ rec, double* F, int* __restrict__ info, const int store_l, int* cnt,
     const int compact0) {
-  static_assert(!(TREE && COMPACT), "the tree schedule keeps full records");
+  static_assert(!(TREE && COMPACT) && (COMPACT || !C1), "the tree schedule keeps full records");
   __shared__ ReducedLds<NX, NU> lds;
   const int lane = threadIdx.x, b = blockIdx.y, N = d.N, k0 = (blockIdx.x + d.xoff) * 4;
-  bottom_group_mc<NX, NU, TREE, false>(d, k0, b, lane, AB, QR, rhs, red, rec, F, info, store_l, COMPACT ? 1 : compact0, lds,
+  bottom_group_mc<NX, NU, TREE, false, C1>(d, k0, b, lane, AB, QR, rhs, red, rec, F, info, store_l, COMPACT ? 1 : compact0, lds,
                                        nullptr, nullptr);
 
   if constexpr (TREE) {
diff --git a/rslqr_amd/csrc/kernels_rowbcast.hpp b/rslqr_amd/csrc/kernels_rowbcast.hpp
--- a/rslqr_amd/csrc/kernels_rowbcast.hpp
+++ b/rslqr_amd/csrc/kernels_rowbcast.hpp
@@ -651,32 +651,47 @@
 
 constexpr int kRbBacksubColsThreads = 128;
 
-template <int NX, int NU>
-struct alignas(16) RbBacksubColsLds {
+template <int NX, bool C1>
+struct RbBacksubColsC1 {};
+template <int NX>
+struct RbBacksubColsC1<NX, true> {
+  double wu[4][NX];
+};
+
+template <int NX, int NU, bool C1 = false>
+struct alignas(16) RbBacksubColsLds : RbBacksubColsC1<NX, C1> {
   static constexpr int NN = NX * NX, REC = 2 * NN + NX, R0 = NX * (NX + 1) / 2;
   static constexpr int R0P = (R0 + 1) / 2 * 2, RECP = REC + (REC & 1);
   static constexpr int TS = 17;
-  double rec0[4][R0P];
+  static constexpr int NL = C1 ? 6 : 4, NF = C1 ? 1 : 3;
+  double rec0[NL][R0P];
   union {
-    double rec1[3][RECP];
+    double rec1[NF][RECP];
     double prod[4][NX * TS];
   };
   double ys[9][NX];
   double wv[4][NX];
 };
 
-template <int SZ>
-__device__ __forceinline__ int rec_of(const int e) { return (e >= SZ) + (e >= 2 * SZ) + (e >= 3 * SZ); }
-
-template <int NX, int NU, bool MULTI>
+template <int SZ, int NR = 4>
+__device__ __forceinline__ int rec_of(const int e) {
+  int q = 0;
+#pragma unroll
+  for (int r = 1; r < NR; ++r) q += e >= r * SZ;
+  return q;
+}
+
+template <int NX, int NU, bool MULTI, bool C1 = false>
 __device__ __forceinline__ void rb_backsub_cols(const Dims& d, const double* __restrict__ AB, const double* __restrict__ QR,
                                                 const double* __restrict__ rhs, const double* __restrict__ recs,
                                                 const double* __restrict__ ytop, double* __restrict__ z,
                                                 const int nprob, const double* __restrict__ zsep) {
-  using Lds = RbBacksubColsLds<NX, NU>;
+  using Lds = RbBacksubColsLds<NX, NU, C1>;
   constexpr int W = NX + NU, ROWS = 2 * NX + NU, NN = NX * NX, REC = 2 * NN + NX, KPB = 8, R0 = Lds::R0, TS = Lds::TS;
   constexpr int NT = kRbBacksubColsThreads;
-  static_assert(W <= 16 && NT == 128 && 3 * NX <= NT, "thread roles fit the workgroup");
+  constexpr int NL = Lds::NL, NF = Lds::NF;
+  static_assert(W <= 16 && NT == 128 && 4 * NX <= NT, "thread roles fit the workgroup");
+  static_assert(!(C1 && MULTI), "the kept records (multi-rhs) are never compact at level 1");
   __shared__ Lds lds;
   const int N = d.N, b = blockIdx.y, first = (blockIdx.x + d.xoff) * KPB;
   const int bp = MULTI ? b % nprob : b;
@@ -696,19 +711,20 @@
     const double* rc0 = recs + ((size_t)bp * N + first) * REC;
     constexpr bool WIDE = NX % 2 == 0 && R0 % 2 == 0;
     constexpr int G = WIDE ? 2 : 1;
-    constexpr int N0 = 4 * R0 / G, I0 = (N0 + NT - 1) / NT, N1 = 3 * REC / G, I1 = (N1 + NT - 1) / NT;
+    constexpr int N0 = NL * R0 / G, I0 = (N0 + NT - 1) / NT, N1 = NF * REC / G, I1 = (N1 + NT - 1) / NT;
     double t0[I0][G], t1[I1][G];
 #pragma unroll
     for (int it = 0; it < I0; ++it) {
-      const int e = t + NT * it, ec = e < N0 ? e : N0 - 1, q = rec_of<R0 / G>(ec), w_ = ec - q * (R0 / G);
-      const double* src = rc0 + (size_t)(2 * q) * REC + G * w_;
+      const int e = t + NT * it, ec = e < N0 ? e : N0 - 1, q = rec_of<R0 / G, NL>(ec), w_ = ec - q * (R0 / G);
+      const int ko = (!C1 || q < 4) ? 2 * q : 4 * q - 15;
+      const double* src = rc0 + (size_t)ko * REC + G * w_;
       if constexpr (WIDE) { const double2 v = *reinterpret_cast<const double2*>(src); t0[it][0] = v.x; t0[it][1] = v.y; }
       else t0[it][0] = *src;
     }
 #pragma unroll
     for (int it = 0; it < I1; ++it) {
-      const int e = t + NT * it, ec = e < N1 ? e : N1 - 1, q = rec_of<REC / G>(ec), w_ = ec - q * (REC / G);
-      const double* src = rc0 + (size_t)(2 * q + 1) * REC + G * w_;
+      const int e = t + NT * it, ec = e < N1 ? e : N1 - 1, q = rec_of<REC / G, NF>(ec), w_ = ec - q * (REC / G);
+      const double* src = rc0 + (size_t)(C1 ? 3 : 2 * q + 1) * REC + G * w_;
       if constexpr (WIDE) { const double2 v = *reinterpret_cast<const double2*>(src); t1[it][0] = v.x; t1[it][1] = v.y; }
       else t1[it][0] = *src;
     }
@@ -724,19 +740,22 @@
     }
 #pragma unroll
     for (int it = 0; it < I0; ++it) {
-      const int e = t + NT * it, ec = e < N0 ? e : N0 - 1, q = rec_of<R0 / G>(ec), w_ = ec - q * (R0 / G);
+      const int e = t + NT * it, ec = e < N0 ? e : N0 - 1, q = rec_of<R0 / G, NL>(ec), w_ = ec - q * (R0 / G);
 #pragma unroll
       for (int h = 0; h < G; ++h) lds.rec0[q][G * w_ + h] = t0[it][h];
     }
 #pragma unroll
     for (int it = 0; it < I1; ++it) {
-      const int e = t + NT * it, ec = e < N1 ? e : N1 - 1, q = rec_of<REC / G>(ec), w_ = ec - q * (REC / G);
+      const int e = t + NT * it, ec = e < N1 ? e : N1 - 1, q = rec_of<REC / G, NF>(ec), w_ = ec - q * (REC / G);
       if (!MULTI || G * w_ < 2 * NN) {
 #pragma unroll
         for (int h = 0; h < G; ++h) lds.rec1[q][G * w_ + h] = t1[it][h];
       }
     }
     if (t < 2 * NX) lds.ys[t < NX ? 7 : 8][t < NX ? t : t - NX] = ty;
+    if constexpr (C1) {
+      if (t >= 2 * NX && t < 4 * NX) lds.ys[t < 3 * NX ? 1 : 5][t < 3 * NX ? t - 2 * NX : t - 3 * NX] = 0.0;
+    }
     if constexpr (MULTI) {
       if (t < 3 * NX) lds.rec1[t / NX][2 * NN + t % NX] = tz;
     }
@@ -751,6 +770,100 @@
     for (int r = 0; r < NX; ++r) s = fma(a[r], y[r], s);
     return s;
   };
+  if constexpr (C1) {
+    auto load_l = [&](const double* Lp, double (&lrow)[NX], double (&lcol)[NX]) {
+      const double* rowp = Lp + cx * (cx + 1) / 2;
+      double dinv = rb_rcp(rowp[cx]);
+      dpp_fence(dinv);
+      sfor<NX>([&](auto ec) {
+        constexpr int e = decltype(ec)::value;
+        const double de = row_bc<e>(dinv);
+        const double lo = rowp[e] * de;
+        const double up = Lp[e * (e + 1) / 2 + cx] * dinv;
+        lrow[e] = (e < c && c < NX) ? lo : 0.0;
+        lcol[e] = (e > c && c < NX) ? up : 0.0;
+      });
+      return dinv * dinv;
+    };
+    auto sep_step = [&](const double (&lrow)[NX], const double (&lcol)[NX], const double d2, const double* wvp) {
+      const double ya = (i > 0 && c < NX) ? lds.ys[k > 0 ? k - 1 : 7][cx] : 0.0;
+      const double zh = (i == 0 && c < NX) ? -tl : (tg + ya) * qinv;
+      if (c < W) {
+#pragma unroll
+        for (int r = 0; r < NX; ++r) lds.prod[j][r * TS + c] = a[r] * zh;
+      }
+      wave_lds_sync();
+      const double* pr = lds.prod[j] + cx * TS;
+      double v0 = 0.0, v1 = 0.0;
+#pragma unroll
+      for (int m = 0; m + 1 < W; m += 2) { v0 += pr[m]; v1 += pr[m + 1]; }
+      if constexpr (W % 2) v0 += pr[W - 1];
+      double x = (v0 + v1) - wvp[cx];
+      sfor<NX - 1>([&](auto cc) {
+        constexpr int e = decltype(cc)::value;
+        dpp_fence(x);
+        fnmac_bc<e>(x, x, lrow[e]);
+      });
+      x = x * d2;
+      sfor<NX - 1>([&](auto cc) {
+        constexpr int e = NX - 1 - decltype(cc)::value;
+        dpp_fence(x);
+        fnmac_bc<e>(x, x, lcol[e]);
+      });
+      return x;
+    };
+    double lrow[NX], lcol[NX];
+    double d2;
+    if (odd) {
+      const bool left = first > 0, right = first + KPB < N;
+      if (j == 1 && c < NX) {
+        const double* rc = lds.rec1[0];
+        double s = rc[2 * NN + c];
+        if (left) {
+#pragma unroll
+          for (int e = 0; e < NX; ++e) s = fma(-rc[c * NX + e], lds.ys[7][e], s);
+        }
+        if (right) {
+#pragma unroll
+          for (int e = 0; e < NX; ++e) s = fma(-rc[NN + c * NX + e], lds.ys[8][e], s);
+        }
+        lds.ys[3][c] = s;
+      }
+      wave_lds_sync();
+      if ((j & 1) && i < N - 1) dot = ab_dot(lds.ys[k < 7 ? k : 8]);
+      if (c < NX) lds.wv[j][c] = tl + (tg - dot) * qinv;
+      d2 = load_l(lds.rec0[4 + (j >> 1)], lrow, lcol);
+    } else {
+      d2 = load_l(lds.rec0[j], lrow, lcol);
+    }
+    __syncthreads();
+    if (!odd) {
+      const double x = sep_step(lrow, lcol, d2, lds.wv[j]);
+      if (c < NX) lds.ys[k][c] = x;
+      wave_lds_sync();
+      const double du = ab_dot(lds.ys[k]);
+      if (c < NX) lds.wu[j][c] = tl + (tg - du) * qinv;
+    }
+    __syncthreads();
+    if (odd) {
+      const double x = sep_step(lrow, lcol, d2, lds.wu[(j + 1) & 3]);
+      if ((j & 1) == 0) {
+        if (c < NX) lds.ys[k][c] = x;
+      }
+      wave_lds_sync();
+      if ((j & 1) == 0) {
+        dot = ab_dot(lds.ys[k]);
+        if (c < NX) lds.wv[j][c] = tl + (tg - dot) * qinv;
+      }
+    }
+    __syncthreads();
+    if (!odd) {
+      const double x = sep_step(lrow, lcol, d2, lds.wv[j]);
+      if (c < NX) lds.ys[k][c] = x;
+      wave_lds_sync();
+      dot = ab_dot(lds.ys[k]);
+    }
+  } else {
   if (odd) {
     auto resolve = [&](const int q, const bool hasA, const int slotA, const bool hasB, const int slotB) {
       const double* rc = lds.rec1[q >> 1];
@@ -804,6 +917,7 @@
     wave_lds_sync();
     dot = ab_dot(lds.ys[k]);
   }
+  }
   __syncthreads();
 
   const double yp = (i > 0 && c < NX) ? lds.ys[k > 0 ? k - 1 : 7][cx] : 0.0;
@@ -816,12 +930,13 @@
   }
 }
 
-template <int NX, int NU, bool MULTI = false, bool COLS = false>
+template <int NX, int NU, bool MULTI = false, bool COLS = false, bool C1 = false>
 __global__ __launch_bounds__(COLS ? kRbBacksubColsThreads : 256) void rb_backsub(
     Dims d, const double* __restrict__ AB, const double* __restrict__ QR, const double* __restrict__ rhs,
     const double* __restrict__ recs, const double* __restrict__ ytop, double* __restrict__ z, const int nprob = 0,
     const double* __restrict__ zsep = nullptr) {
-  if constexpr (COLS) rb_backsub_cols<NX, NU, MULTI>(d, AB, QR, rhs, recs, ytop, z, nprob, zsep);
+  static_assert(COLS || !C1, "the staged body reads full level-1 records");
+  if constexpr (COLS) rb_backsub_cols<NX, NU, MULTI, C1>(d, AB, QR, rhs, recs, ytop, z, nprob, zsep);
   else rb_backsub_staged<NX, NU, MULTI>(d, AB, QR, rhs, recs, ytop, z, nprob, zsep);
 }
 
diff --git a/rslqr_amd/csrc/launch_small.hpp b/rslqr_amd/csrc/launch_small.hpp
--- a/rslqr_amd/csrc/launch_small.hpp
+++ b/rslqr_amd/csrc/launch_small.hpp
@@ -16,6 +16,7 @@
   bool compact;
   bool rowbcast;
   bool fuse2;
+  bool compact1;
   int level0;
   int ltop;
   int top_l0;
@@ -38,9 +39,20 @@
   return da;
 }
 
+template <int NX, int NU>
+constexpr bool kCompact1Fits = ndlqr::P1OnMatrixCores<NX, NU>::value && NX >= 9 && NX + NU <= 16;
+
 template <int NX, int NU, bool MULTI, class... Args>
-static void launch_rb_backsub(const NdlqrHipCtx* c, const dim3 grid, hipStream_t stream, const Args&... args) {
+static void launch_rb_backsub(const NdlqrHipCtx* c, const dim3 grid, hipStream_t stream, const bool compact1,
+                              const Args&... args) {
   if constexpr (NX + NU <= 16) {
+    if constexpr (kCompact1Fits<NX, NU> && !MULTI) {
+      if (compact1) {
+        hipLaunchKernelGGL((ndlqr::rb_backsub<NX, NU, false, true, true>), grid, dim3(ndlqr::kRbBacksubColsThreads), 0, stream,
+                           args...);
+        return;
+      }
+    }
     if (c->knobs.backsub_cols != 0) {
       hipLaunchKernelGGL((ndlqr::rb_backsub<NX, NU, MULTI, true>), grid, dim3(ndlqr::kRbBacksubColsThreads), 0, stream, args...);
       return;
@@ -71,6 +83,9 @@
       p.rec_compact = p.compact && p.store_l == 2;
       p.rowbcast = p.compact && !p.store_l && NX <= 16 && NX + NU <= 16 && (c->knobs.rowbcast == 1 || (c->knobs.rowbcast < 0 && NX <= 8));
       p.fuse2 = !p.rowbcast && p.compact && !p.store_l && (c->knobs.fuse2 > 0 || (c->knobs.fuse2 < 0 && NX == 12 && NU == 4));
+      p.compact1 = kCompact1Fits<NX, NU> && p.compact && !p.store_l && !p.rowbcast && c->knobs.backsub_cols != 0 &&
+                   (c->knobs.compact1 > 0 ||
+                    (c->knobs.compact1 < 0 && ((NX == 12 && NU == 4 && p.fuse2) || (NX == 10 && NU == 4))));
       p.schedule = p.tree ? "reduced-tree"
                    : !p.compact ? "reduced-records"
                    : p.store_l ? "reduced-compact-records" : (p.fuse2 ? "reduced-fused2" : "reduced");
@@ -104,15 +119,33 @@
             hipLaunchKernelGGL((ndlqr::rb_bottom<NX, NU>), dim3(d.N >> 4, d.batch), dim3(64), 0, s.stream, d, c->AB,
                                c->QR, s.rhs, s.red, s.rec, c->info);
         } else if (plan.fuse2) {
-          hipLaunchKernelGGL((ndlqr::bottom8_reduced_mc<NX, NU>), dim3(d.N >> 3, d.batch), dim3(128), 0, s.stream, d,
-                             c->AB, c->QR, s.rhs, s.red, s.rec, c->info);
+          bool done = false;
+          if constexpr (kCompact1Fits<NX, NU>) {
+            if (plan.compact1) {
+              hipLaunchKernelGGL((ndlqr::bottom8_reduced_mc<NX, NU, true>), dim3(d.N >> 3, d.batch), dim3(128), 0, s.stream, d,
+                                 c->AB, c->QR, s.rhs, s.red, s.rec, c->info);
+              done = true;
+            }
+          }
+          if (!done)
+            hipLaunchKernelGGL((ndlqr::bottom8_reduced_mc<NX, NU>), dim3(d.N >> 3, d.batch), dim3(128), 0, s.stream, d,
+                               c->AB, c->QR, s.rhs, s.red, s.rec, c->info);
         } else if (plan.tree)
           hipLaunchKernelGGL((ndlqr::bottom_reduced_mc<NX, NU, true>), dim3(d.N >> 2, d.batch), dim3(64), 0, s.stream,
                              d, c->AB, c->QR, s.rhs, s.red, s.rec, c->F, c->info, store_l, s.tree_cnt, 0);
-        else if (plan.compact)
-          hipLaunchKernelGGL((ndlqr::bottom_reduced_mc<NX, NU, false, true>), dim3(d.N >> 2, d.batch), dim3(64), 0, s.stream,
-                             d, c->AB, c->QR, s.rhs, s.red, s.rec, c->F, c->info, store_l, nullptr, 1);
-        else
+        else if (plan.compact) {
+          bool done = false;
+          if constexpr (kCompact1Fits<NX, NU>) {
+            if (plan.compact1) {
+              hipLaunchKernelGGL((ndlqr::bottom_reduced_mc<NX, NU, false, true, true>), dim3(d.N >> 2, d.batch), dim3(64), 0,
+                                 s.stream, d, c->AB, c->QR, s.rhs, s.red, s.rec, c->F, c->info, store_l, nullptr, 1);
+              done = true;
+            }
+          }
+          if (!done)
+            hipLaunchKernelGGL((ndlqr::bottom_reduced_mc<NX, NU, false, true>), dim3(d.N >> 2, d.batch), dim3(64), 0, s.stream,
+                               d, c->AB, c->QR, s.rhs, s.red, s.rec, c->F, c->info, store_l, nullptr, 1);
+        } else
           hipLaunchKernelGGL((ndlqr::bottom_reduced_mc<NX, NU, false>), dim3(d.N >> 2, d.batch), dim3(64), 0, s.stream,
                              d, c->AB, c->QR, s.rhs, s.red, s.rec, c->F, c->info, store_l, nullptr, 0);
       }
@@ -132,7 +165,7 @@
           (void)allow_dynamic_lds(&ndlqr::rb_backsub_top<NX>, plan.top_lds);
           hipLaunchKernelGGL((ndlqr::rb_backsub_top<NX>), dim3(d.batch), dim3(256), plan.top_lds, s.stream, d, s.rec, s.ytop);
         }
-        launch_rb_backsub<NX, NU, false>(c, dim3(apply_grid(c, d), d.batch), s.stream,
+        launch_rb_backsub<NX, NU, false>(c, dim3(apply_grid(c, d), d.batch), s.stream, plan.compact1,
                            apply_dims(c, d), c->AB, c->QR, s.rhs, s.rec, s.ytop, s.z);
       } else {
         hipLaunchKernelGGL((ndlqr::backsub_small<NX, NU>), dim3(apply_grid(c, d), d.batch), dim3(256), 0, s.stream, apply_dims(c, d), c->AB,
@@ -184,7 +217,7 @@
                            rhs, s.rec, (const double*)s.red, s.ytop);
       }
       ScopedSlot t(c, SLOT_APPLY);
-      launch_rb_backsub<NX, NU, false>(c, dim3(apply_grid(c, d), d.batch), s.stream,
+      launch_rb_backsub<NX, NU, false>(c, dim3(apply_grid(c, d), d.batch), s.stream, false,
                          apply_dims(c, d), c->AB, c->QR, rhs, s.rec, s.ytop, z);
       return;
     }
@@ -220,7 +253,7 @@
                        s.rec, fsum, d.batch, zsep);
     hipLaunchKernelGGL((ndlqr::rb_forward_top<NX, NU, true>), dim3(count), dim3(256), lds, s.stream, d, c->AB, c->QR, rhs,
                        s.rec, (const double*)fsum, ytop, d.batch, zsep);
-    launch_rb_backsub<NX, NU, true>(c, dim3(apply_grid(c, d), count), s.stream,
+    launch_rb_backsub<NX, NU, true>(c, dim3(apply_grid(c, d), count), s.stream, false,
                        apply_dims(c, d), c->AB, c->QR, rhs, (const double*)s.rec, (const double*)ytop, z, d.batch,
                        (const double*)zsep);
     return true;
@@ -278,7 +311,7 @@
       hipLaunchKernelGGL((ndlqr::rb_backsub_top<NX>), dim3(d.batch), dim3(256), top_lds, bs.stream, d, bs.rec, bs.ytop);
       const int cnt = (d.N >> 3) / G;
       d.xoff = g * cnt;
-      launch_rb_backsub<NX, NU, false>(c, dim3(cnt, d.batch), bs.stream, d, c->AB, c->QR,
+      launch_rb_backsub<NX, NU, false>(c, dim3(cnt, d.batch), bs.stream, false, d, c->AB, c->QR,
                          bs.rhs, bs.rec, bs.ytop, bs.z);
     }
     c->kept.schedule = "reduced-time-shard";
diff --git a/rslqr_amd/csrc/ndlqr_hip.hip b/rslqr_amd/csrc/ndlqr_hip.hip
--- a/rslqr_amd/csrc/ndlqr_hip.hip
+++ b/rslqr_amd/csrc/ndlqr_hip.hip
@@ -97,6 +97,7 @@
   onoff("NDLQR_ROWBCAST", &k.rowbcast);
   onoff("NDLQR_FUSE2", &k.fuse2);
   onoff("NDLQR_BACKSUB_COLS", &k.backsub_cols);
+  onoff("NDLQR_COMPACT1", &k.compact1);
   k.no_mfma = getenv("NDLQR_NO_MFMA") != nullptr;
   k.no_top = getenv("NDLQR_NO_TOP") != nullptr;
   num("NDLQR_TOP_LEVELS", &k.top_levels);
@@ -703,6 +704,7 @@
     p.kept.schedule = p.small.schedule;
     p.kept.rec_complete = p.small.rec_complete;
     p.kept.rec_compact = p.small.rec_compact;
+    p.kept.rec1_compact = p.small.compact1;
   } else if ((p.red = plan_reduced_generic(c)).ok) {
     p.family = Family::GenericReduced;
     p.needs_red_generic = true;
@@ -1529,6 +1531,8 @@
 
 const char* ndlqr_hip_schedule(const NdlqrHipCtx* c) { return c ? c->kept.schedule : "none"; }
 
+int ndlqr_hip_compact_level1(const NdlqrHipCtx* c) { return c && c->kept.rec1_compact ? 1 : 0; }
+
 int ndlqr_hip_factors_valid(const NdlqrHipCtx* c) { return c && c->kept.fact_valid ? 1 : 0; }
 
 int ndlqr_hip_pack_solutions_device(NdlqrHipCtx* c, double* dst) {
diff --git a/rslqr_amd/roofline.py b/rslqr_amd/roofline.py
--- a/rslqr_amd/roofline.py
+++ b/rslqr_amd/roofline.py
@@ -4,8 +4,8 @@
 FP64_PEAK_TFLOPS = 78.6
 
 
-def record_doubles(n, level, compact_level0=False):
-    if compact_level0 and level == 0:
+def record_doubles(n, level, compact_level0=False, compact_level1=False):
+    if (compact_level0 and level == 0) or (compact_level1 and level == 1):
         return n * (n + 1) // 2
     return 2 * n * n + n
 
@@ -31,19 +31,20 @@
     return 8 * (inputs_doubles(n, m, N) + N * (2 * n + m))
 
 
-def reduced_model(n, m, N, compact_level0=False, fused2=False):
+def reduced_model(n, m, N, compact_level0=False, fused2=False, compact_level1=False):
     K = int(math.log2(N))
     if fused2 and N >= 16:
-        base = reduced_model(n, m, N, compact_level0, False)
+        base = reduced_model(n, m, N, compact_level0, False, compact_level1)
         w, rows = n + m, 2 * n + m
         tri = n * (n + 1) // 2
-        rec0, rec = record_doubles(n, 0, compact_level0), record_doubles(n, 1)
+        rec0, rec = record_doubles(n, 0, compact_level0), record_doubles(n, 2)
+        rec1 = record_doubles(n, 1, compact_level0, compact_level1)
         fs = separator_flops(n, w)
         push = 2 * tri + n * n + 2 * n
         slot = 2 * tri + 2 * n * n + 2 * n
         per_sep = slot + n * w + w + n + rows + 2 * n + rec + push
         nsep2 = N // 8
-        base["bottom"] = {"bytes": 8 * (inputs_doubles(n, m, N) + (N // 2) * rec0 + (N // 4 + nsep2) * rec +
+        base["bottom"] = {"bytes": 8 * (inputs_doubles(n, m, N) + (N // 2) * rec0 + (N // 4) * rec1 + nsep2 * rec +
                                        nsep2 * (4 * (tri + n) + n * n)),
                           "flops": (3 * N // 4 + nsep2) * fs, "launches": 1}
         if "upper" in base:
@@ -61,12 +62,13 @@
     push = 2 * tri + n * n + 2 * n
     slot = 2 * tri + 2 * n * n + 2 * n
     rec0 = record_doubles(n, 0, compact_level0)
-    rec = record_doubles(n, 1)
+    rec = record_doubles(n, 2)
+    rec1 = record_doubles(n, 1, compact_level0, compact_level1)
     fs = separator_flops(n, w)
     nsep_upper = max(N // 4 - 1, 0)
-    bottom_b = inputs_doubles(n, m, N) + (N // 2) * rec0 + (N // 4) * rec + (N // 4) * push
+    bottom_b = inputs_doubles(n, m, N) + (N // 2) * rec0 + (N // 4) * rec1 + (N // 4) * push
     upper_b = nsep_upper * (slot + n * w + w + n + rows + 2 * n + rec + push)
-    recs_read = (N // 2) * rec0 + (N // 4) * rec + nsep_upper * rec
+    recs_read = (N // 2) * rec0 + (N // 4) * rec1 + nsep_upper * rec
     apply_b = recs_read + inputs_doubles(n, m, N) + N * rows + ((N // 8) * n + (N // 8) * 2 * n if compact_level0 else 0)
     out = {
         "bottom": {"bytes": 8 * bottom_b, "flops": (3 * N // 4) * fs, "launches": 1},
@@ -150,11 +152,11 @@
     }
 
 
-def model_for(schedule, n, m, N):
+def model_for(schedule, n, m, N, compact1=False):
     if schedule == "reduced":
-        return reduced_model(n, m, N, compact_level0=True)
+        return reduced_model(n, m, N, compact_level0=True, compact_level1=compact1)
     if schedule == "reduced-fused2":
-        return reduced_model(n, m, N, compact_level0=True, fused2=True)
+        return reduced_model(n, m, N, compact_level0=True, fused2=True, compact_level1=compact1)
     if schedule in ("reduced-tree", "reduced-records"):
         return reduced_model(n, m, N)
     if schedule == "knot-lean":
```
